# BaeHann/feature_level_style_transfer_for_TSC

Measured on AMD Instinct MI355X. Metric: train-step samples/sec (univariate TS, len=512, batch=256) at 1/2/4/8 MI355X, higher is better.
Workload: dtype bf16x3

## Files before the change

### feature_level_style_transfer_for_tsc_amd/_lib.py

```python
from __future__ import annotations

import ctypes
import os
from ctypes import POINTER, Structure, c_char_p, c_float, c_int, c_int32, c_int64, c_void_p
from typing import Optional

import torch

ABI_VERSION = 26
_LIB_NAME = "libfst_hip.so"
_HERE = os.path.dirname(os.path.abspath(__file__))
LIB_PATH = os.environ.get("FST_HIP_LIB", os.path.join(_HERE, _LIB_NAME))


class FstLibraryError(RuntimeError):
    pass


class WSrc(Structure):
    _fields_ = [("w", c_void_p), ("off0", c_int64), ("sm", c_int64), ("sc", c_int64), ("st", c_int64)]


_P = c_void_p
_I32P = c_void_p
_SIGNATURES = {
    "fst_version": (c_int, []),
    "fst_last_error": (c_char_p, []),
    "fst_pack_weights": (c_int, [_I32P, _I32P, c_int, POINTER(WSrc), POINTER(WSrc), c_int, c_int, c_int, c_int, _P, c_void_p]),
    "fst_pack_weights_bf16x3": (c_int, [_I32P, _I32P, c_int, POINTER(WSrc), POINTER(WSrc), c_int, c_int, c_int, c_int, _P, c_void_p]),
    "fst_unpack_weights": (c_int, [_I32P, _I32P, c_int, _P, c_int, _P, c_int64, c_int64, c_int64, c_int64,
                                   _P, c_int64, c_int64, c_int64, c_int64, c_int, c_void_p]),
    "fst_mask_taps": (c_int, [_P, _I32P, _I32P, c_int, c_int, c_int, c_void_p]),
    "fst_conv_gemm": (c_int, [_P, c_int64, _P, c_int64, _P, _I32P, _I32P, c_int, _P, _P, c_int64, _P, c_int64,
                              _P, c_int64, c_int, c_int, c_int, c_int, c_int, c_int, c_int, c_int, c_void_p]),
    "fst_conv_wgrad": (c_int, [_P, c_int64, _P, c_int64, _P, c_int64, _P, c_int64, c_int, _P, _I32P, _I32P, c_int,
                               c_int, c_int, c_int, c_int, c_int, c_int64, c_void_p]),
    "fst_conv_last_route": (c_int, [POINTER(c_int32)]),
    "fst_row_sum": (c_int, [_P, c_int64, c_int, c_int, c_int, _P, c_void_p]),
    "fst_bn_stats": (c_int, [_P, c_int, c_int, c_int, _P, c_int64, c_void_p]),
    "fst_bn_finalize": (c_int, [_P, c_int, _P, _P, _P, _P, c_int, c_int, c_float, c_float, _P, c_void_p]),
    "fst_bn_apply": (c_int, [_P, _P, _P, _P, _P, c_int, c_int, c_int, c_int, c_int64, c_void_p]),
    "fst_bn_bwd_reduce": (c_int, [_P, _P, _P, _P, c_int, c_int, c_int, c_int, _P, c_int64, c_void_p]),
    "fst_bn_bwd_apply": (c_int, [_P, _P, _P, _P, _P, c_int, _P, _P, _P, c_int, c_int, c_int, c_int, c_int, c_int, c_int64, c_void_p]),
    "fst_bn_bwd_reduce_join": (c_int, [_P, _P, _P, _P, _P, c_int, c_int, c_int, _P, _P, c_int64, c_void_p]),
    "fst_bn_bwd_apply_join": (c_int, [_P, _P, _P, _P, _P, _P, _P, c_int, _P, _P, _P, _P, _P, _P, c_int, c_int, c_int, c_int, c_int,
                                      c_int64, c_void_p]),
    "fst_gate_fwd": (c_int, [_P, _P, c_int, c_int, c_int, c_int64, c_void_p]),
    "fst_gate_bwd": (c_int, [_P, _P, _P, c_int, c_int, c_int, c_int64, c_void_p]),
    "fst_coupling_sum_slots": (c_int64, [c_int, c_int, c_int]),
    "fst_coupling_fwd": (c_int, [_P, _P, _P, c_int, c_int, c_int, c_int64, _P, c_void_p]),
    "fst_coupling_bwd": (c_int, [_P, _P, _P, _P, _P, _P, _P, _P, c_int, c_int, c_int, c_int64, c_void_p]),
    "fst_coupling_inv_fwd": (c_int, [_P, _P, _P, c_int, c_int, c_int, c_int64, c_void_p]),
    "fst_coupling_inv_bwd": (c_int, [_P, _P, _P, _P, _P, c_int, c_int, c_int, c_int64, c_void_p]),
    "fst_rmsprop_multi": (c_int, [_P, _P, _P, _P, _P, c_int, c_float, c_float, c_void_p]),
    "fst_adam_multi": (c_int, [_P, _P, _P, _P, _P, c_int, _P, c_float, c_float, c_float, c_float, c_void_p]),
    "fst_rmsprop_multi_dev": (c_int, [_P, _P, _P, _P, _P, c_int, c_float, c_float, c_void_p]),
    "fst_adam_multi_dev": (c_int, [_P, _P, _P, _P, _P, c_int, _P, _P, c_float, c_float, c_float, c_void_p]),
    "fst_nonfinite_slots": (c_int64, [c_int]),
    "fst_nonfinite_multi": (c_int, [_P, _P, _I32P, c_int, c_int32, _I32P, c_int64, _I32P, _I32P, _P, _I32P, c_void_p]),
    "fst_rmsprop_multi_guard": (c_int, [_P, _P, _P, _P, _P, _P, c_int, c_float, c_float, _I32P, c_void_p]),
    "fst_adam_multi_guard": (c_int, [_P, _P, _P, _P, _P, c_int, _P, c_float, _P, c_float, c_float, c_float, _I32P, c_void_p]),
    "fst_guard_copy_multi": (c_int, [_P, _P, _P, c_int, _I32P, c_int, c_void_p]),
    "fst_sumsq_slots": (c_int64, [c_int]),
    "fst_sumsq_multi": (c_int, [_P, _P, _I32P, c_int, _P, c_int64, _P, _P, _P, c_void_p]),
    "fst_scale_multi": (c_int, [_P, _P, _I32P, c_int, _P, c_void_p]),
    "fst_ema_multi": (c_int, [_P, _P, _P, _I32P, c_int, c_int32, _P, _P, c_void_p]),
    "fst_swap_multi": (c_int, [_P, _P, _P, c_int, c_void_p]),
    "fst_accum_multi": (c_int, [_P, _P, _P, c_int, _P, c_int, c_void_p]),
    "fst_feed_batch": (c_int, [_P, _P, _P, _P, _P, _P, c_int, _P, _P, c_int, _P, c_void_p]),
    "fst_eval_fold": (c_int, [_P, c_int64, _P, c_int64, c_int, _P, _P, _P, _P, _P, _P, c_int64, _P, c_void_p]),
    "fst_eval_finish": (c_int, [_P, _P, c_int64, _P, c_int, c_void_p]),
    "fst_wn_stack_fwd_ok": (c_int, [c_int, c_int, c_int, c_int]),
    "fst_wn_stack_fwd": (c_int, [_P, _P, _P, c_int64, _P, _P, _P, c_int64, _P, c_int, c_int, c_int, c_int, c_int, c_int64, c_void_p]),
    "fst_wn_stack_infer": (c_int, [_P, _P, _P, c_int64, _P, _P, c_int64, _P, c_int, c_int, c_int, c_int, c_int, c_int64, c_void_p]),
    "fst_wn_stack_bwd_ok": (c_int, [c_int, c_int, c_int, c_int]),
    "fst_wn_stack_bwd": (c_int, [_P, _P, _P, _P, _P, _P, _P, _P, _P, c_int64, c_int, c_int, c_int, c_int, c_int, c_int64, c_void_p]),
    "fst_wn_stack_bwd_proj": (c_int, [_P, _P, _P, _P, _P, _P, _P, _P, c_int, c_int64, _P, c_int64, c_int, c_int, c_int, c_int, c_int,
                                      c_int64, c_void_p]),
    "fst_wn_wgrad_ok": (c_int, [c_int, c_int, c_int, c_int, c_int, c_int]),
    "fst_wn_wgrad_workspace_floats": (c_int64, [c_int, c_int, c_int, c_int, c_int, c_int]),
    "fst_wn_wgrad_in": (c_int, [_P, _P, _P, c_int, c_int64, _P, _P, _P, c_int64, c_int, c_int, c_int, c_int, c_int, c_int, c_int64,
                                c_void_p]),
    "fst_wn_wgrad_rs": (c_int, [_P, _P, _P, c_int, _P, _P, c_int64, c_int, c_int, c_int, c_int, c_int64, c_void_p]),
    "fst_wn_wgrad_in_slabs": (c_int, [_P, _P, _P, c_int, c_int64, _P, c_int64, c_int, c_int, c_int, c_int, c_int, c_int, c_int64,
                                      c_void_p]),
    "fst_wn_wgrad_rs_slabs": (c_int, [_P, _P, _P, c_int, _P, c_int64, c_int, c_int, c_int, c_int, c_int64, c_void_p]),
    "fst_wn_wgrad_reduce_many": (c_int, [_I32P, _I32P, _I32P, _P, _P, _P, _P, c_int, c_int, c_int, c_int, c_int, c_void_p]),
    "fst_nt_gemm_workspace_floats": (c_int64, [c_int, c_int, c_int]),
    "fst_nt_gemm": (c_int, [_P, _P, _P, _P, c_int64, c_int, c_int, c_int, _P, _P, c_int, c_float, _P, c_void_p]),
    "fst_tap_wgrad_ok": (c_int, [c_int, c_int, c_int, c_int, c_int, c_int, c_int]),
    "fst_tap_wgrad_workspace_floats": (c_int64, [c_int, c_int, c_int, c_int, c_int]),
    "fst_tap_wgrad": (c_int, [_P, _P, _P, _P, c_int64, c_int, c_int, c_int, c_int, c_int, c_int, c_int, c_int, c_int64, c_int64, c_void_p]),
    "fst_dense_tap_wgrad_ok": (c_int, [c_int, c_int, c_int, c_int, c_int, c_int]),
    "fst_dense_tap_wgrad_workspace_floats": (c_int64, [c_int, c_int, c_int, c_int, c_int]),
    "fst_dense_tap_wgrad": (c_int, [_P, _P, _P, _P, c_int64, c_int, c_int, c_int, c_int, c_int, c_int, c_int64, c_int64, c_void_p]),
    "fst_wn_last_route": (c_int, [POINTER(c_int32)]),
    "fst_relu_bwd": (c_int, [_P, _P, _P, c_int64, c_void_p]),
    "fst_gemm_workspace_floats": (c_int64, [c_int, c_int, c_int]),
    "fst_gemm": (c_int, [_P, c_int64, c_int, _P, c_int64, c_int, _P, c_int64, c_int, c_int, c_int, _P, c_int, c_float, _P, c_int64,
                         c_void_p]),
    "fst_gemm_f32_workspace_floats": (c_int64, [c_int, c_int, c_int]),
    "fst_gemm_f32": (c_int, [_P, c_int64, c_int, _P, c_int64, c_int, _P, c_int64, c_int, c_int, c_int, _P, c_int, c_float, _P, c_int64,
                             c_void_p]),
    "fst_act_bwd": (c_int, [_P, _P, _P, c_int64, c_float, c_void_p]),
    "fst_batch_sum": (c_int, [_P, _P, _P, c_int, c_int64, c_int, c_void_p]),
    "fst_noise_transfer_fwd": (c_int, [_P, c_int, c_int, _P, _P, c_float, c_float, _P, _P, _P, _P, _P, _P, _P, c_int, c_int, c_void_p]),
    "fst_bcast_add": (c_int, [_P, _P, _P, c_int, c_int64, c_void_p]),
    "fst_noise_transfer_bwd": (c_int, [_P, c_int, _P, _P, _P, _P, c_int, c_int, c_void_p]),
    "fst_noise_transfer_dw": (c_int, [_P, _P, _P, _P, c_int, c_int, c_void_p]),
    "fst_noise_transfer_bwd_apply": (c_int, [_P, _P, _P, _P, c_float, c_float, c_int, _P, _P, c_int64, c_void_p]),
    "fst_wn_fold_fwd": (c_int, [_P, c_int, _P, _P, c_void_p]),
    "fst_wn_fold_bwd": (c_int, [_P, c_int, _P, _P, _P, c_void_p]),
    "fst_logdet_inv": (c_int, [_P, c_int, _P, _P, c_void_p]),
    "fst_wn_image_bytes": (c_int64, [c_int, c_int]),
    "fst_wn_pack": (c_int, [_P, _P, _P, _P, _P, _P, c_int, c_int, c_int, c_int, _P, c_int64, c_void_p]),
    "fst_wn_pack_stack": (c_int, [_P, _P, _P, _P, _P, _P, c_int, c_int, c_int, c_int, _P, c_int64, c_void_p]),
    "fst_wn_layer_fwd": (c_int, [_P, c_int64, _P, c_int64, _P, c_int64, _P, _P, _P, _P, c_int, c_int, c_int, c_int, c_int, c_int,
                                 c_int, c_int64, c_void_p]),
    "fst_wn_layer_infer": (c_int, [_P, c_int64, _P, c_int64, _P, c_int64, _P, _P, c_int, c_int, c_int, c_int, c_int, c_int, c_int,
                                   c_int64, c_void_p]),
    "fst_wn_bwd_image_bytes": (c_int64, [c_int, c_int]),
    "fst_wn_pack_bwd": (c_int, [_P, c_int, c_int, c_int, _P, c_int64, c_void_p]),
    "fst_wn_pack_bwd_stack": (c_int, [_P, c_int, c_int, c_int, _P, c_int64, c_void_p]),
    "fst_wn_bwd_proj_image_bytes": (c_int64, [c_int, c_int, c_int]),
    "fst_wn_pack_bwd_proj_stack": (c_int, [_P, _P, c_int, c_int, c_int, _P, c_int64, c_void_p]),
    "fst_wn_layer_bwd": (c_int, [_P, _P, _P, _P, c_int64, _P, _P, c_int64, c_int, c_int, c_int, c_int, c_int64, c_void_p]),
    "fst_wn_dgrad_image_bytes": (c_int64, [c_int]),
    "fst_wn_pack_dgrad": (c_int, [_P, _P, c_int, c_int, c_int, _P, c_int64, c_void_p]),
    "fst_wn_pack_dgrad_stack": (c_int, [_P, _P, c_int, c_int, c_int, c_int, _P, c_int64, c_void_p]),
    "fst_wn_dgrad_fits": (c_int, [c_int, c_int, c_int]),
    "fst_wn_layer_dgrad": (c_int, [_P, _P, c_int64, _P, _P, _P, _P, c_int64, c_int, c_int, c_int, c_int, c_int, c_int64, c_int64,
                                   c_void_p]),
    "fst_gru_fwd": (c_int, [_P, _P, _P, _P, _P, _I32P, c_int, c_int, c_int, c_int, c_int64, c_void_p]),
    "fst_gru_bwd": (c_int, [_P, _P, _P, _P, _I32P, c_int, _P, _P, c_int, c_int, c_int, c_int64, c_void_p]),
    "fst_lstm2_fwd": (c_int, [_P, _P, _P, _P, c_int, c_int, c_int64, c_void_p]),
    "fst_lstm2_bwd": (c_int, [_P, _P, _P, _P, _P, c_int, c_int, c_int64, c_void_p]),
    "fst_axpy": (c_int, [_P, _P, c_float, c_int64, c_void_p]),
    "fst_add_slices": (c_int, [_P, c_int64, _P, c_int64, _P, c_int64, c_int, c_int, c_int, c_void_p]),
    "fst_cpc_workspace_floats": (c_int64, [c_int, c_int, c_int, c_int]),
    "fst_cpc_nce_slots": (c_int64, [c_int, c_int, c_int, c_int]),
    "fst_cpc_nce_fwd": (c_int, [_P, c_int64, c_int64, c_int64, _I32P, _P, c_int, c_int, c_int, c_int, c_int, _P, _P, _P, c_void_p]),
    "fst_cpc_nce_bwd": (c_int, [_P, c_int64, c_int64, c_int64, _I32P, _P, _P, c_int, c_int, c_int, c_int, c_int, _P, _P, _P,
                                c_void_p]),
}
EXPORTED_SYMBOLS = tuple(_SIGNATURES)

_lib: Optional[ctypes.CDLL] = None


def load(path: Optional[str] = None) -> ctypes.CDLL:
    global _lib
    if _lib is not None and path is None:
        return _lib
    p = path or LIB_PATH
    if not os.path.exists(p):
        raise FstLibraryError(
            f"{p} not found — build it with `python -c 'import __graft_entry__ as g; g.build()'` "
            "(hipcc --offload-arch=gfx950).  There is no CPU fallback.")
    try:
        lib = ctypes.CDLL(p)
    except OSError as e:
        raise FstLibraryError(f"cannot load {p}: {e}") from e
    for name, (res, args) in _SIGNATURES.items():
        try:
            fn = getattr(lib, name)
        except AttributeError as e:
            raise FstLibraryError(f"{p} does not export {name}; rebuild the library") from e
        fn.restype, fn.argtypes = res, args
    if lib.fst_version() != ABI_VERSION:
        raise FstLibraryError(f"{p}: ABI version {lib.fst_version()} != expected {ABI_VERSION}; rebuild")
    if path is None:
        _lib = lib
    return lib


def check(rc: int, what: str) -> None:
    if rc != 0:
        msg = load().fst_last_error()
        raise RuntimeError(f"{what} failed (rc={rc}): {msg.decode() if msg else '?'}")


def stream_ptr() -> int:
    return torch.cuda.current_stream().cuda_stream


def ptr(t: Optional[torch.Tensor]) -> Optional[int]:
    return None if t is None else t.data_ptr()


def require_gpu_tensor(t: torch.Tensor, name: str) -> None:
    if not t.is_cuda:
        raise FstLibraryError(f"{name} lives on {t.device}; the fst ops run on an MI355X only (no CPU fallback)")
    if t.dtype != torch.float32:
        raise TypeError(f"{name} must be float32, got {t.dtype}")
```

### feature_level_style_transfer_for_tsc_amd/csrc/wn_wgrad.hip

```cpp
#include <stdlib.h>
#include <type_traits>

#include "fst_device.h"

#define WW_TT 32
#define WW_MROWS 256
#define WW_ND 3
#define WW_NX 2
#define WW_MAX_NX 5

__device__ __attribute__((aligned(16))) float ww_zero16[4] = {0.f, 0.f, 0.f, 0.f};

#define WW_MAX_SETS 3
struct WwOut { int rows, out, out_off, out_sc, out_sm; };
struct WwSeg {
  const float* ptr[WW_MAX_SETS];
  long long bs;
  long long mul_off;
  int shift;
  WwOut o;
};

struct WwParams {
  WwSeg dy[2];
  WwSeg x[4];
  int n_dy, n_x, M, K, K_main, n_extra;
  int xr;
  int mul;
  int n_groups, ksplit, B, L, tiles_per_seq, n_tiles;
  const float* epi_p;
  const float* epi_r1;
  float* epi_raw;
  int epi_ncls;
  float epi_scale;
  int n_sets;
  int RX;
  int misaligned;
  int Kcols;
  float* slab;
  float* slab_extra;
  float* w[2];
};

__device__ __forceinline__ unsigned ww_lds_addr(const char* p) {
  return (unsigned)(uintptr_t)((__attribute__((address_space(3))) const char*)p);
}
template <int OFF = 0>
__device__ __forceinline__ f32x4 ww_lds_read16(unsigned addr) {
  f32x4 v;
  asm volatile("ds_read_b128 %0, %1 offset:%2" : "=v"(v) : "v"(addr), "n"(OFF) : "memory");
  return v;
}
template <int OFF = 0>
__device__ __forceinline__ float ww_lds_read4(unsigned addr) {
  float v;
  asm volatile("ds_read_b32 %0, %1 offset:%2" : "=v"(v) : "v"(addr), "n"(OFF) : "memory");
  return v;
}
template <int OFF = 0>
__device__ __forceinline__ void ww_lds_write16(unsigned addr, const u32x4& v) {
  asm volatile("ds_write_b128 %0, %1 offset:%2" ::"v"(addr), "v"(v), "n"(OFF) : "memory");
}
template <int OFF = 0>
__device__ __forceinline__ void ww_lds_zero4(unsigned addr) {
  asm volatile("ds_write_b32 %0, %1 offset:%2" ::"v"(addr), "v"(0.0f), "n"(OFF) : "memory");
}
__device__ __forceinline__ void ww_dma16(const char* gsrc, unsigned lds_addr) {
  unsigned saved_m0;
  asm volatile("s_mov_b32 %0, m0\n\ts_mov_b32 m0, %2\n\ts_nop 0\n\tglobal_load_lds_dwordx4 %1, off\n\ts_mov_b32 m0, %0"
               : "=&s"(saved_m0) : "v"(gsrc), "s"(lds_addr) : "memory");
}
__device__ __forceinline__ void ww_lds_wait() {
  asm volatile("s_waitcnt lgkmcnt(0)" ::: "memory");
  __builtin_amdgcn_sched_barrier(0);
}

template <class V4>
__device__ __forceinline__ void ww_split8u(const V4& v0, const V4& v1, u32x4& h, u32x4& l) {
  const float v[8] = {v0.x, v0.y, v0.z, v0.w, v1.x, v1.y, v1.z, v1.w};
  bf16x8 hi, lo;
  split_bf16x8(v, hi, lo);
  h = __builtin_bit_cast(u32x4, hi);
  l = __builtin_bit_cast(u32x4, lo);
}

__device__ __forceinline__ int ww_dma_row(int i, int lane) { return 8 * i + ((lane >> 3) ^ (i & 1)); }
__device__ __forceinline__ int ww_lds_off(int r, int q) { return ((r ^ ((r >> 3) & 1)) << 7) + (((q ^ r) & 7) << 4); }


struct WwDmaLane { int r, q; };
__device__ __forceinline__ WwDmaLane ww_dma_lane(int i, int lane) {
  const int r = ww_dma_row(i, lane);
  return {r, (lane ^ r) & 7};
}

struct WwFragLane { int row, piece[2][2]; };
__device__ __forceinline__ WwFragLane ww_frag_lane(int l31, int half) {
  WwFragLane f;
  f.row = (l31 ^ ((l31 >> 3) & 1)) << 7;
  const int sw = l31 & 7;
#pragma unroll
  for (int ks = 0; ks < 2; ++ks)
#pragma unroll
    for (int j = 0; j < 2; ++j) f.piece[ks][j] = (((4 * ks + 2 * half + j) ^ sw) & 7) << 4;
  return f;
}

__device__ __forceinline__ void ww_tile_range(int wg, int n_wgs, int n_tiles, int& begin, int& end) {
  begin = (int)(((long long)wg * n_tiles) / n_wgs);
  end = (int)(((long long)(wg + 1) * n_tiles) / n_wgs);
}

__device__ __forceinline__ void ww_store_tile(float* dst, int ld, const f32x16& acc) {
#pragma unroll
  for (int r = 0; r < 16; ++r) dst[(long long)((r & 3) + 8 * (r >> 2)) * ld] = acc[r];
}


__device__ __forceinline__ const WwOut& ww_out(const WwSeg& s) { return s.o; }
__device__ __forceinline__ const WwOut& ww_out(const WwOut& o) { return o; }
struct WwRow { int si, c; };
template <class S>
__device__ __forceinline__ WwRow ww_k_row(const S (&x)[4], int n_x, int kk) {
  WwRow r = {0, kk};
#pragma unroll
  for (int j = 0; j < 3; ++j)
    if (r.si == j && j + 1 < n_x && r.c >= ww_out(x[j]).rows) { r.c -= ww_out(x[j]).rows; ++r.si; }
  return r;
}
template <class S, class F>
__device__ __forceinline__ auto ww_pick(const S (&x)[4], int si, F f) {
  auto v = f(x[0]);
  if (si == 1) v = f(x[1]);
  if (si == 2) v = f(x[2]);
  if (si == 3) v = f(x[3]);
  return v;
}

struct WwSrc { const float* p; int bs, t; };

struct WwDyStage {
  WwSrc src[4];

  __device__ __forceinline__ void build(const WwParams& p, int set, int wave_s, int lane) {
    const float* const d0 = p.dy[0].ptr[set];
    const float* const d1 = p.dy[1].ptr[set];
#pragma unroll
    for (int k = 0; k < 4; ++k) {
      const WwDmaLane m = ww_dma_lane(wave_s + 8 * k, lane);
      const int r = m.r, q = m.q;
      src[k].p = nullptr; src[k].bs = 0; src[k].t = 4 * q;
      if (r < p.M) {
        if (p.n_dy > 1 && r >= p.dy[0].o.rows) {
          src[k].p = d1 + ((long long)(r - p.dy[0].o.rows) * p.L + 4 * q); src[k].bs = (int)p.dy[1].bs;
        } else {
          src[k].p = d0 + ((long long)r * p.L + 4 * q); src[k].bs = (int)p.dy[0].bs;
        }
      }
    }
  }
  __device__ __forceinline__ void issue1(int k, int b, int t0, int L, char* slot, int wave_s, const char* zero16) const {
    const bool ok = src[k].p != nullptr && t0 + src[k].t < L;
    const char* s = ok ? reinterpret_cast<const char*>(src[k].p + ((long long)b * src[k].bs + t0)) : zero16;
    ww_dma16(s, ww_lds_addr(slot + (wave_s + 8 * k) * 1024));
  }
};

struct WwXStage {
  WwSrc src[WW_MAX_NX];
  int my_nx;

  __device__ __forceinline__ void build(const WwParams& p, int set, int g, int wave_s, int lane) {
    const int NXI = p.RX >> 3;
    my_nx = (NXI - wave_s + 7) >> 3;
    const float* const xp[4] = {p.x[0].ptr[set], p.x[1].ptr[set], p.x[2].ptr[set], p.x[3].ptr[set]};
#pragma unroll
    for (int k = 0; k < WW_MAX_NX; ++k) {
      src[k].p = nullptr; src[k].bs = 0; src[k].t = 0;
      if (k >= my_nx) continue;
      const WwDmaLane m = ww_dma_lane(wave_s + 8 * k, lane);
      const int rr = m.r, q = m.q;
      int kk = -1;
      bool partner = false;
      if (rr < p.xr) kk = g * p.xr + rr;
      else if (p.mul && rr < 2 * p.xr) { kk = g * p.xr + rr - p.xr; partner = true; }
      else {
        const int e = rr - p.xr * (1 + p.mul);
        if (g == 0 && e < p.n_extra) kk = p.K_main + e;
      }
      if (kk >= 0 && kk < p.K && (kk < p.K_main || rr >= p.xr * (1 + p.mul))) {
        const WwRow row = ww_k_row(p.x, p.n_x, kk);
        const float* sp = ww_pick(xp, row.si, [](const float* x) { return x; });
        const long long sbs = ww_pick(p.x, row.si, [](const WwSeg& x) { return x.bs; });
        const long long smo = ww_pick(p.x, row.si, [](const WwSeg& x) { return x.mul_off; });
        const int ssh = ww_pick(p.x, row.si, [](const WwSeg& x) { return x.shift; });
        src[k].p = sp + ((long long)row.c * p.L + ssh + 4 * q) + (partner ? smo : 0);
        src[k].bs = (int)sbs;
        src[k].t = ssh + 4 * q;
      }
    }
  }
  __device__ __forceinline__ void issue1(int k, int b, int t0, int L, char* slot, int wave_s, const char* zero16) const {
    if (k >= my_nx) return;
    const int t = t0 + src[k].t;
    const bool ok = src[k].p != nullptr && t > -4 && t < L;
    const char* s = ok ? reinterpret_cast<const char*>(src[k].p + ((long long)b * src[k].bs + t0)) : zero16;
    ww_dma16(s, ww_lds_addr(slot + (wave_s + 8 * k) * 1024));
  }
};

__device__ __forceinline__ int ww_patch_shift(const WwParams& p, int g, int tid) {
  if (!(p.misaligned && tid < p.xr)) return 0;
  const int kk = g * p.xr + tid;
  const int sh = ww_pick(p.x, ww_k_row(p.x, p.n_x, kk).si, [](const WwSeg& x) { return x.shift; });
  return (kk < p.K_main && (sh & 3) != 0 && sh > -4 && sh < 4) ? sh : 0;
}

__device__ __forceinline__ void ww_patch_edges(char* xslot, int tid, int patch_sh, int t0, int L) {
  const bool at_start = t0 == 0, at_end = t0 + WW_TT >= L;
  if (at_start || at_end) {
    if (patch_sh != 0) {
      char* rowp = xslot + ((tid ^ ((tid >> 3) & 1)) << 7);
      if (at_start && patch_sh < 0)
        for (int j = 0; j < -patch_sh; ++j) ww_lds_zero4(ww_lds_addr(rowp + (((0 ^ tid) & 7) << 4) + 4 * j));
      if (at_end && patch_sh > 0)
        for (int j = 4 - patch_sh; j < 4; ++j) ww_lds_zero4(ww_lds_addr(rowp + (((7 ^ tid) & 7) << 4) + 4 * j));
    }
    asm volatile("s_waitcnt lgkmcnt(0)" ::: "memory");
    __builtin_amdgcn_s_barrier();
  }
}

template <bool MUL, int NE>
static __device__ void ww_split_pass(char* dw, char* xw, int tid, int xr, int e_off, float (&ev)[2]) {
  const int u = tid & 3, r0 = tid >> 2;
  f32x4 e0, e1;
  if constexpr (NE > 0) {
    e0 = ww_lds_read16(ww_lds_addr(xw + e_off + ((2 * u) << 4)));
    e1 = ww_lds_read16(ww_lds_addr(xw + e_off + ((2 * u + 1) << 4)));
  }
  f32x4 d[2][2], xq[2][2], xm[2][2];
  char* da[2][2]; char* xa[2][2];
  const int nxu = (xr * 4 > 512 + tid) ? 2 : 1;
#pragma unroll
  for (int i = 0; i < 2; ++i) {
    const int r = r0 + 128 * i;
    da[i][0] = dw + ww_lds_off(r, 2 * u); da[i][1] = dw + ww_lds_off(r, 2 * u + 1);
    d[i][0] = ww_lds_read16(ww_lds_addr(da[i][0])); d[i][1] = ww_lds_read16(ww_lds_addr(da[i][1]));
    xa[i][0] = xw + ww_lds_off(r, 2 * u); xa[i][1] = xw + ww_lds_off(r, 2 * u + 1);
    if (i < nxu && r < xr) {
      xq[i][0] = ww_lds_read16(ww_lds_addr(xa[i][0])); xq[i][1] = ww_lds_read16(ww_lds_addr(xa[i][1]));
      if constexpr (MUL) {
        xm[i][0] = ww_lds_read16(ww_lds_addr(xa[i][0] + (xr << 7))); xm[i][1] = ww_lds_read16(ww_lds_addr(xa[i][1] + (xr << 7)));
      }
    }
  }
  ww_lds_wait();
#pragma unroll
  for (int i = 0; i < 2; ++i) {
    const int r = r0 + 128 * i;
    if constexpr (NE > 0)
      ev[i] += (d[i][0].x * e0.x + d[i][0].y * e0.y) + (d[i][0].z * e0.z + d[i][0].w * e0.w) +
               (d[i][1].x * e1.x + d[i][1].y * e1.y) + (d[i][1].z * e1.z + d[i][1].w * e1.w);
    u32x4 h4, l4;
    ww_split8u(d[i][0], d[i][1], h4, l4);
    ww_lds_write16(ww_lds_addr(da[i][0]), h4); ww_lds_write16(ww_lds_addr(da[i][1]), l4);
    if (i < nxu && r < xr) {
      if constexpr (MUL) { xq[i][0] *= xm[i][0]; xq[i][1] *= xm[i][1]; }
      ww_split8u(xq[i][0], xq[i][1], h4, l4);
      ww_lds_write16(ww_lds_addr(xa[i][0]), h4); ww_lds_write16(ww_lds_addr(xa[i][1]), l4);
    }
  }
  asm volatile("s_waitcnt lgkmcnt(0)" ::: "memory");
}

template <int MT, int KT, bool FULL, class Issue>
__device__ __forceinline__ void ww_k_step(f32x16 (&acc)[MT][KT], const char* ap, const char* bp, const int (&piece)[2], int m_live,
                                          int k_live, Issue issue) {
  f32x4 araw[MT][2], braw[KT][2];
#pragma unroll
  for (int i = 0; i < MT; ++i) {
    araw[i][0] = ww_lds_read16(ww_lds_addr(ap + ((i * 32) << 7) + piece[0]));
    araw[i][1] = ww_lds_read16(ww_lds_addr(ap + ((i * 32) << 7) + piece[1]));
  }
#pragma unroll
  for (int j = 0; j < KT; ++j) {
    braw[j][0] = ww_lds_read16(ww_lds_addr(bp + ((j * 32) << 7) + piece[0]));
    braw[j][1] = ww_lds_read16(ww_lds_addr(bp + ((j * 32) << 7) + piece[1]));
  }
  ww_lds_wait();
  issue(0);
#pragma unroll
  for (int j = 0; j < KT; ++j) {
    if (FULL || j < k_live) {
      const bf16x8 bh = __builtin_bit_cast(bf16x8, braw[j][0]), bl = __builtin_bit_cast(bf16x8, braw[j][1]);
#pragma unroll
      for (int i = 0; i < MT; ++i) {
        if (!FULL && i >= m_live) break;
        const bf16x8 ah = __builtin_bit_cast(bf16x8, araw[i][0]), al = __builtin_bit_cast(bf16x8, araw[i][1]);
        mfma_bf3(acc[i][j], ah, al, bh, bl);
      }
    }
    issue(1 + j);
  }
  if constexpr (KT < 3) issue(3);
  issue(4);
}

template <int MT, int KT, bool FULL, bool MUL, int NE>
__global__ __launch_bounds__(512, 2) void wn_wgrad_kernel(WwParams p) {
  extern __shared__ __attribute__((aligned(16))) char ww_lds[];
  const int tid = threadIdx.x, lane = tid & 63, half = lane >> 5, l31 = lane & 31;
  const int wave_s = __builtin_amdgcn_readfirstlane(tid >> 6);
  const int wm = wave_s >> 1, wk = wave_s & 1;
  const int g = blockIdx.y, L = p.L;
  const int set = blockIdx.x % p.n_sets;
  const int dslot_bytes = WW_MROWS * 128, xslot_bytes = p.RX * 128;
  char* const xring = ww_lds + WW_ND * dslot_bytes;
  const char* const zero16 = reinterpret_cast<const char*>(ww_zero16);

  WwDyStage dys;
  dys.build(p, set, wave_s, lane);
  WwXStage xs;
  xs.build(p, set, g, wave_s, lane);
  const int patch_sh = ww_patch_shift(p, g, tid);
  __builtin_amdgcn_s_waitcnt(0x0F70);

  auto tile_bt = [&](int tile, int& b, int& t0) {
    b = tile / p.tiles_per_seq;
    t0 = (tile - b * p.tiles_per_seq) * WW_TT;
  };
  auto issue_dy = [&](int tile, int slot) {
    int b, t0;
    tile_bt(tile, b, t0);
#pragma unroll
    for (int k = 0; k < 4; ++k) dys.issue1(k, b, t0, L, ww_lds + slot * dslot_bytes, wave_s, zero16);
  };
  auto issue_x = [&](int tile, int slot) {
    int b, t0;
    tile_bt(tile, b, t0);
#pragma unroll
    for (int k = 0; k < WW_MAX_NX; ++k) xs.issue1(k, b, t0, L, xring + slot * xslot_bytes, wave_s, zero16);
  };

  f32x16 acc[MT][KT];
  zero_acc(acc);
  float ev[2] = {0.f, 0.f};

  const int wg_in_set = blockIdx.x / p.n_sets, wgs_of_set = (p.ksplit - set + p.n_sets - 1) / p.n_sets;
  int tile_begin, tile_end;
  ww_tile_range(wg_in_set, wgs_of_set, p.n_tiles, tile_begin, tile_end);
  const int m_blocks = (p.M + 31) >> 5;
  const int k_blocks_here = min(2 * KT, ((p.K_main + 31) >> 5) - g * 2 * KT);
  const int m_live = m_blocks - wm * MT, k_live = k_blocks_here - wk * KT;
  const bool do_extra = NE > 0 && g == 0;

  const WwFragLane fl = ww_frag_lane(l31, half);
  const int a_off = ((wm * MT * 32) << 7) + fl.row;
  const int x_off = ((wk * KT * 32) << 7) + fl.row;
  const int e_off = (p.xr * (1 + p.mul)) << 7;

  const int n_st = tile_end - tile_begin;
  if (n_st > 0) { issue_dy(tile_begin, 0); issue_x(tile_begin, 0); }
  if (n_st > 1) issue_dy(tile_begin + 1, 1);
  int dslot = 0, xslot = 0;
  for (int c = 0; c < n_st; ++c) {
    if (c + 1 < n_st) wait_vmcnt<4>(); else wait_vmcnt<0>();
    __builtin_amdgcn_s_barrier();
    const bool have_x = c + 1 < n_st, have_dy = c + 2 < n_st;
    int nb = 0, nt0 = 0, db = 0, dt0 = 0;
    if (have_x) tile_bt(tile_begin + c + 1, nb, nt0);
    if (have_dy) tile_bt(tile_begin + c + 2, db, dt0);
    const int x_next = xslot ^ 1, d_next = dslot >= 1 ? dslot - 1 : 2;
    auto issue_pos = [&](int pos) {
      if (pos < WW_MAX_NX) { if (have_x) xs.issue1(pos, nb, nt0, L, xring + x_next * xslot_bytes, wave_s, zero16); }
      else if (pos < WW_MAX_NX + 4) { if (have_dy) dys.issue1(pos - WW_MAX_NX, db, dt0, L, ww_lds + d_next * dslot_bytes, wave_s, zero16); }
    };
    char* const dsl = ww_lds + dslot * dslot_bytes;
    char* const xsl = xring + xslot * xslot_bytes;
    if (p.misaligned) {
      int bq, t0;
      tile_bt(tile_begin + c, bq, t0);
      ww_patch_edges(xsl, tid, patch_sh, t0, L);
    }
    ww_split_pass<MUL, NE>(dsl, xsl, tid, p.xr, e_off, ev);
    __builtin_amdgcn_s_barrier();
#pragma unroll
    for (int ks = 0; ks < 2; ++ks)
      ww_k_step<MT, KT, FULL>(acc, dsl + a_off, xsl + x_off, fl.piece[ks], m_live, k_live, [&](int pos) { issue_pos(5 * ks + pos); });
    dslot = dslot == WW_ND - 1 ? 0 : dslot + 1;
    xslot ^= 1;
  }

  float* const slab = p.slab + (long long)blockIdx.x * WW_MROWS * p.Kcols;
#pragma unroll
  for (int i = 0; i < MT; ++i) {
    if (i >= m_live) break;
#pragma unroll
    for (int j = 0; j < KT; ++j) {
      if (j >= k_live) break;
      ww_store_tile(slab + (long long)((wm * MT + i) * 32 + 4 * half) * p.Kcols + g * p.xr + (wk * KT + j) * 32 + l31, p.Kcols, acc[i][j]);
    }
  }
  if (do_extra) {
#pragma unroll
    for (int i = 0; i < 2; ++i) {
      float sv = ev[i];
      sv += __shfl_xor(sv, 1, 64);
      sv += __shfl_xor(sv, 2, 64);
      if ((tid & 3) == 0) p.slab_extra[((long long)blockIdx.x * WW_MROWS + (tid >> 2) + 128 * i) * 2] = sv;
    }
  }
}


__device__ __forceinline__ void ww_dst(const WwParams& p, int si, int& out, int& off, int& sc, int& sm) {
  out = p.x[0].o.out; off = p.x[0].o.out_off; sc = p.x[0].o.out_sc; sm = p.x[0].o.out_sm;
  if (si == 1) { out = p.x[1].o.out; off = p.x[1].o.out_off; sc = p.x[1].o.out_sc; sm = p.x[1].o.out_sm; }
  if (si == 2) { out = p.x[2].o.out; off = p.x[2].o.out_off; sc = p.x[2].o.out_sc; sm = p.x[2].o.out_sm; }
  if (si == 3) { out = p.x[3].o.out; off = p.x[3].o.out_off; sc = p.x[3].o.out_sc; sm = p.x[3].o.out_sm; }
}
template <class P, class Epi>
__device__ __forceinline__ void ww_scatter(const P& p, int m, int kk, float v, Epi epi) {
  const WwRow r = ww_k_row(p.x, p.n_x, kk);
  int out, off, sc, sm;
  ww_dst(p, r.si, out, off, sc, sm);
  float* dst = out == 0 ? p.w[0] : p.w[1];
  const long long at = (long long)m * sm + (long long)r.c * sc + off;
  dst[at] = epi(v, at, r.c, sm);
}

template <class Store>
__device__ __forceinline__ void ww_quad_sum(const float* q, long long st, int ksplit, bool live, float4 (&part)[4][64], Store store) {
  const int cx = threadIdx.x & 63, sg = threadIdx.x >> 6;
  float4 s = make_float4(0.f, 0.f, 0.f, 0.f);
  if (live) {
    int sl = sg;
    for (; sl + 28 < ksplit; sl += 32) {
      float4 v[8];
#pragma unroll
      for (int u = 0; u < 8; ++u) v[u] = *reinterpret_cast<const float4*>(q + (sl + 4 * u) * st);
#pragma unroll
      for (int u = 0; u < 8; ++u) { s.x += v[u].x; s.y += v[u].y; s.z += v[u].z; s.w += v[u].w; }
    }
    for (; sl < ksplit; sl += 4) {
      const float4 v = *reinterpret_cast<const float4*>(q + sl * st);
      s.x += v.x; s.y += v.y; s.z += v.z; s.w += v.w;
    }
  }
  part[sg][cx] = s;
  __syncthreads();
  if (sg == 0 && live) {
    float4 t = part[0][cx];
#pragma unroll
    for (int g2 = 1; g2 < 4; ++g2) { const float4 o = part[g2][cx]; t.x += o.x; t.y += o.y; t.z += o.z; t.w += o.w; }
    const float tv[4] = {t.x, t.y, t.z, t.w};
    store(tv);
  }
}

__device__ __forceinline__ float ww_extra_sum(const float* q, int ksplit) {
  float s = 0.f;
  int sl = 0;
  for (; sl + 8 <= ksplit; sl += 8) {
    float v[8];
#pragma unroll
    for (int u = 0; u < 8; ++u) v[u] = q[(long long)(sl + u) * WW_MROWS * 2];
#pragma unroll
    for (int u = 0; u < 8; ++u) s += v[u];
  }
  for (; sl < ksplit; ++sl) s += q[(long long)sl * WW_MROWS * 2];
  return s;
}

__global__ __launch_bounds__(256) void wn_wgrad_reduce_kernel(WwParams p) {
  __shared__ float4 part[4][64];
  const int m = blockIdx.y, cx = threadIdx.x & 63, sg = threadIdx.x >> 6;
  const int kk0 = blockIdx.x * 256 + cx * 4;
  auto epi = [&](float v, long long at, int c, int sm) {
    if (p.epi_p) {
      float sd = 0.f;
      for (int j = 0; j < p.epi_ncls; ++j) sd += p.epi_p[m * p.epi_ncls + j] * p.epi_r1[(long long)j * sm + c];
      if (p.epi_raw) p.epi_raw[at] = v;
      v = v * p.epi_scale * sd;
    }
    return v;
  };
  ww_quad_sum(p.slab + (long long)m * p.Kcols + kk0, (long long)WW_MROWS * p.Kcols, p.ksplit, kk0 < p.Kcols, part, [&](const float (&tv)[4]) {
#pragma unroll
    for (int j = 0; j < 4; ++j)
      if (kk0 + j < p.K_main) ww_scatter(p, m, kk0 + j, tv[j], epi);
  });
  if (blockIdx.x == gridDim.x - 1 && sg == 1 && cx < p.n_extra && p.K_main < p.K)
    ww_scatter(p, m, p.K_main + cx, ww_extra_sum(p.slab_extra + (long long)m * 2 + cx, p.ksplit), epi);
}

#define WW_MAX_RED 16
struct WwRedEntry {
  const float* slab;
  const float* slab_extra;
  float* w[2];
  int ksplit, Kcols, K_main, K, n_extra, M, n_x;
  int quad_blocks;
  WwOut x[4];
};
struct WwRedParams { WwRedEntry e[WW_MAX_RED]; };
__device__ __forceinline__ void ww_dst(const WwRedEntry& e, int si, int& out, int& off, int& sc, int& sm) {
  auto field = [&](int WwOut::*f) { return ww_pick(e.x, si, [f](const WwOut& o) { return o.*f; }); };
  out = field(&WwOut::out); off = field(&WwOut::out_off); sc = field(&WwOut::out_sc); sm = field(&WwOut::out_sm);
}

__global__ __launch_bounds__(256) void wn_wgrad_reduce_many_kernel(WwRedParams p) {
  __shared__ float4 part[4][64];
  const WwRedEntry& e = p.e[blockIdx.z];
  const int bx = blockIdx.x;
  auto plain = [](float v, long long, int, int) { return v; };
  if (bx >= e.quad_blocks) {
    const int it = (bx - e.quad_blocks) * 256 + threadIdx.x;
    if (e.K_main < e.K && it < e.M * e.n_extra) {
      const int m = it / e.n_extra, j = it - m * e.n_extra;
      ww_scatter(e, m, e.K_main + j, ww_extra_sum(e.slab_extra + (long long)m * 2 + j, e.ksplit), plain);
    }
    return;
  }
  const int qpr = e.Kcols >> 2;
  const int quad = bx * 64 + (threadIdx.x & 63);
  ww_quad_sum(e.slab + (long long)quad * 4, (long long)WW_MROWS * e.Kcols, e.ksplit, quad < e.M * qpr, part, [&](const float (&tv)[4]) {
    const int m = quad / qpr, kk0 = (quad - m * qpr) * 4;
#pragma unroll
    for (int j = 0; j < 4; ++j)
      if (kk0 + j < e.K_main) ww_scatter(e, m, kk0 + j, tv[j], plain);
  });
}


static thread_local int32_t g_wn_route[FST_WN_ROUTE_LEN] = {0};

void fst_wn_set_route(int family, int t1, int t2, int t3, int t4, int gx, int gy, int gz, int a8, int a9, int a10, int lds) {
  const int32_t r[FST_WN_ROUTE_LEN] = {family, t1, t2, t3, t4, gx, gy, gz, a8, a9, a10, lds};
  for (int i = 0; i < FST_WN_ROUTE_LEN; ++i) g_wn_route[i] = r[i];
}

extern "C" int fst_wn_last_route(int32_t out[FST_WN_ROUTE_LEN]) {
  FST_REQUIRE(out != nullptr, "fst_wn_last_route: null output");
  for (int i = 0; i < FST_WN_ROUTE_LEN; ++i) out[i] = g_wn_route[i];
  return g_wn_route[0] != 0 ? 0 : -1;
}

static int ww_ksplit(int n_groups, int clamp, int floor) {
  int ks = fst_cu_count_or(256) / n_groups;
  if (ks > clamp) ks = clamp;
  if (ks < floor) ks = floor;
  return ks;
}

static void ww_tiles_and_split(WwParams* p, int B, int L, int n_sets) {
  p->RX = p->xr * (1 + p->mul) + (p->n_extra ? 8 : 0);
  p->Kcols = p->n_groups * p->xr;
  p->B = B; p->L = L;
  p->tiles_per_seq = L / WW_TT;
  p->n_tiles = B * p->tiles_per_seq;
  p->ksplit = ww_ksplit(p->n_groups, p->n_tiles * n_sets, n_sets);
  p->n_sets = n_sets;
}

static int64_t ww_slab_floats(const WwParams& p) { return (int64_t)p.ksplit * WW_MROWS * (p.Kcols + 2); }

static int ww_bind_workspace(WwParams& p, float* workspace, int64_t workspace_floats, const char* who) {
  FST_REQUIRE(workspace_floats >= ww_slab_floats(p), "%s: workspace of %lld floats is too small", who, (long long)workspace_floats);
  p.slab = workspace;
  p.slab_extra = workspace + (long long)p.ksplit * WW_MROWS * p.Kcols;
  return 0;
}

static int ww_geometry(int kind, int B, int L, int n, int h, int last, int n_sets, WwParams* p) {
  const int KT = kind == 0 ? 3 : 2;
  p->M = kind == 0 ? 2 * n : (last ? n : 2 * n);
  p->K = kind == 0 ? 3 * n + h : n;
  const int rem = p->K & 31;
  p->n_extra = (kind == 0 && rem == 1) ? 1 : 0;
  p->K_main = p->n_extra ? p->K - rem : p->K;
  p->xr = 32 * 2 * KT;
  const int kb = (p->K_main + 31) / 32;
  p->n_groups = (kb + 2 * KT - 1) / (2 * KT);
  p->mul = kind == 1;
  ww_tiles_and_split(p, B, L, n_sets);
  return KT;
}

extern "C" int fst_wn_wgrad_ok(int kind, int B, int L, int n, int h, int dil) {
  if (!(B > 0 && L > 0 && L % WW_TT == 0 && n > 0 && n < 128)) return 0;
  if (kind == 0) {
    if (!(h > 0 && h <= 32 && dil > 0 && (3 * n + h + 31) / 32 <= 18)) return 0;
    return dil % 4 == 0 ? 1 : (dil < 4 ? 2 : 0);
  }
  return kind == 1;
}

extern "C" int64_t fst_wn_wgrad_workspace_floats(int kind, int B, int L, int n, int h, int last) {
  if (!fst_wn_wgrad_ok(kind, B, L, n, h, 4)) return -1;
  WwParams p;
  ww_geometry(kind, B, L, n, h, last, WW_MAX_SETS, &p);
  return ww_slab_floats(p);
}

static int ww_launch(WwParams& p, int KT, void* stream, bool reduce = true) {
  const size_t lds = (size_t)WW_ND * WW_MROWS * 128 + (size_t)WW_NX * p.RX * 128;
  FST_REQUIRE(lds <= 160 * 1024 && (p.RX >> 3) <= 8 * WW_MAX_NX, "fst_wn_wgrad: %d staged k-rows per stage do not fit (LDS %zu B)", p.RX, lds);
  const bool full = (p.M + 31) / 32 == 8 && ((p.K_main + 31) / 32) % (2 * KT) == 0;
  void (*fn)(WwParams);
  if (KT == 3) {
    if (p.n_extra) fn = full ? wn_wgrad_kernel<2, 3, true, false, 1> : wn_wgrad_kernel<2, 3, false, false, 1>;
    else fn = full ? wn_wgrad_kernel<2, 3, true, false, 0> : wn_wgrad_kernel<2, 3, false, false, 0>;
  } else if (p.mul) {
    fn = full ? wn_wgrad_kernel<2, 2, true, true, 0> : wn_wgrad_kernel<2, 2, false, true, 0>;
  } else {
    fn = full ? wn_wgrad_kernel<2, 2, true, false, 0> : wn_wgrad_kernel<2, 2, false, false, 0>;
  }
  if (int rc = fst_allow_full_lds((const void*)fn, "fst_wn_wgrad")) return rc;
  fst_wn_set_route(FST_WN_ROUTE_WGRAD, KT, (int)full, p.mul, p.n_extra, p.ksplit, p.n_groups, 1, p.n_sets, p.misaligned, (int)reduce, (int)lds);
  hipLaunchKernelGGL(fn, dim3((unsigned)p.ksplit, (unsigned)p.n_groups), dim3(512), lds, (hipStream_t)stream, p);
  FST_LAUNCH_CHECK();
  if (!reduce) return 0;
  hipLaunchKernelGGL(wn_wgrad_reduce_kernel, dim3((unsigned)((p.Kcols + 255) / 256), (unsigned)p.M), dim3(256), 0, (hipStream_t)stream, p);
  FST_LAUNCH_CHECK();
  return 0;
}

static void ww_in_segments(WwParams& p, int n, int h, int L, int dil, long long u0_bs) {
  p.n_dy = 1;
  p.dy[0] = {{}, (long long)2 * n * L, 0, 0, {2 * n, 0, 0, 0, 0}};
  p.n_x = 4;
  for (int tap = 0; tap < 3; ++tap) p.x[tap] = {{}, (long long)n * L, 0, (tap - 1) * dil, {n, 0, tap, 3, 3 * n}};
  p.x[3] = {{}, u0_bs, 0, 0, {h, 1, 0, 1, h}};
}

static void ww_rs_segments(WwParams& p, int n, int L, int last) {
  p.n_dy = last ? 1 : 2;
  p.dy[0] = {{}, (long long)n * L, 0, 0, {n, 0, 0, 0, 0}};
  p.dy[1] = {{}, (long long)n * L, 0, 0, {n, 0, 0, 0, 0}};
  p.n_x = 1;
  p.x[0] = {{}, (long long)2 * n * L, (long long)n * L, 0, {n, 0, 0, 1, n}};
}

static int ww_prologue(const char* who, int kind, const float* const* const* ops, int n_ops, int n_sets, float* workspace,
                       int64_t workspace_floats, int B, int L, int n, int h, int last, WwParams& p, int& KT) {
  FST_REQUIRE(n_sets >= 1 && n_sets <= WW_MAX_SETS, "%s: %d operand sets (1..%d)", who, n_sets, WW_MAX_SETS);
  FST_REQUIRE(fst_aligned16(workspace), "%s: operands must be 16-byte aligned", who);
  KT = ww_geometry(kind, B, L, n, h, last, n_sets, &p);
  if (int rc = ww_bind_workspace(p, workspace, workspace_floats, who)) return rc;
  for (int s = 0; s < n_sets; ++s)
    for (int k = 0; k < n_ops; ++k) {
      FST_REQUIRE(ops[k][s], "%s: null operand in set %d", who, s);
      FST_REQUIRE(fst_aligned16(ops[k][s]), "%s: operands must be 16-byte aligned", who);
    }
  return 0;
}

static int ww_in(const float* const* dg, const float* const* a, const float* const* u0, int n_sets, int64_t u0_bs, float* dw_in,
                 float* dw_cond, float* workspace, int64_t workspace_floats, int B, int L, int n, int h, int dil, int a_slack,
                 int64_t numel_a, void* stream, bool reduce) {
  fst_wn_clear_route();
  FST_REQUIRE(dg && a && u0 && workspace && (!reduce || (dw_in && dw_cond)), "fst_wn_wgrad_in: null operand");
  const int served = fst_wn_wgrad_ok(0, B, L, n, h, dil);
  FST_REQUIRE(served == 1 || (served == 2 && a_slack), "fst_wn_wgrad_in: unsupported shape B=%d L=%d n=%d h=%d dil=%d (needs L %% 32 == 0, "
              "n < 128, h <= 32, and dil %% 4 == 0 or — with 16 readable bytes either side of a — dil < 4)", B, L, n, h, dil);
  FST_REQUIRE((long long)B * n * L == (long long)numel_a, "fst_wn_wgrad_in: B*n*L does not match the element count %lld of a", (long long)numel_a);
  FST_REQUIRE(B == 1 || u0_bs >= (int64_t)h * L, "fst_wn_wgrad_in: u0 batch stride %lld < h*L", (long long)u0_bs);
  FST_REQUIRE(u0_bs % 4 == 0, "fst_wn_wgrad_in: operands must be 16-byte aligned");
  WwParams p = {};
  int KT;
  const float* const* const ops[3] = {dg, a, u0};
  if (int rc = ww_prologue("fst_wn_wgrad_in", 0, ops, 3, n_sets, workspace, workspace_floats, B, L, n, h, 0, p, KT)) return rc;
  ww_in_segments(p, n, h, L, dil, (long long)u0_bs);
  for (int s = 0; s < n_sets; ++s) {
    p.dy[0].ptr[s] = dg[s];
    for (int tap = 0; tap < 3; ++tap) p.x[tap].ptr[s] = a[s];
    p.x[3].ptr[s] = u0[s];
  }
  p.misaligned = dil % 4 != 0;
  p.w[0] = dw_in; p.w[1] = dw_cond;
  return ww_launch(p, KT, stream, reduce);
}

extern "C" int fst_wn_wgrad_in(const float* const* dg, const float* const* a, const float* const* u0, int n_sets, int64_t u0_bs,
                               float* dw_in, float* dw_cond, float* workspace, int64_t workspace_floats, int B, int L, int n, int h,
                               int dil, int a_slack, int64_t numel_a, void* stream) {
  return ww_in(dg, a, u0, n_sets, u0_bs, dw_in, dw_cond, workspace, workspace_floats, B, L, n, h, dil, a_slack, numel_a, stream, true);
}

extern "C" int fst_wn_wgrad_in_slabs(const float* const* dg, const float* const* a, const float* const* u0, int n_sets, int64_t u0_bs,
                                     float* workspace, int64_t workspace_floats, int B, int L, int n, int h, int dil, int a_slack,
                                     int64_t numel_a, void* stream) {
  return ww_in(dg, a, u0, n_sets, u0_bs, nullptr, nullptr, workspace, workspace_floats, B, L, n, h, dil, a_slack, numel_a, stream, false);
}

static int ww_rs(const float* const* d_a, const float* const* d_out, const float* const* ts, int n_sets, float* dw_rs, float* workspace,
                 int64_t workspace_floats, int last, int B, int L, int n, int64_t numel_a, void* stream, bool reduce) {
  fst_wn_clear_route();
  FST_REQUIRE(d_out && ts && (dw_rs || !reduce) && workspace && (last || d_a), "fst_wn_wgrad_rs: null operand");
  FST_REQUIRE(fst_wn_wgrad_ok(1, B, L, n, 0, 4), "fst_wn_wgrad_rs: unsupported shape B=%d L=%d n=%d (needs L %% 32 == 0, n < 128)", B, L, n);
  FST_REQUIRE((long long)B * n * L == (long long)numel_a, "fst_wn_wgrad_rs: B*n*L does not match the element count %lld", (long long)numel_a);
  WwParams p = {};
  int KT;
  const float* const* const ops[3] = {d_out, ts, d_a};
  if (int rc = ww_prologue("fst_wn_wgrad_rs", 1, ops, last ? 2 : 3, n_sets, workspace, workspace_floats, B, L, n, 0, last, p, KT)) return rc;
  ww_rs_segments(p, n, L, last);
  for (int s = 0; s < n_sets; ++s) {
    if (last) p.dy[0].ptr[s] = d_out[s];
    else { p.dy[0].ptr[s] = d_a[s]; p.dy[1].ptr[s] = d_out[s]; }
    p.x[0].ptr[s] = ts[s];
  }
  p.w[0] = dw_rs; p.w[1] = nullptr;
  return ww_launch(p, KT, stream, reduce);
}

extern "C" int fst_wn_wgrad_rs(const float* const* d_a, const float* const* d_out, const float* const* ts, int n_sets, float* dw_rs,
                               float* workspace, int64_t workspace_floats, int last, int B, int L, int n, int64_t numel_a,
                               void* stream) {
  return ww_rs(d_a, d_out, ts, n_sets, dw_rs, workspace, workspace_floats, last, B, L, n, numel_a, stream, true);
}

extern "C" int fst_wn_wgrad_rs_slabs(const float* const* d_a, const float* const* d_out, const float* const* ts, int n_sets,
                                     float* workspace, int64_t workspace_floats, int last, int B, int L, int n, int64_t numel_a,
                                     void* stream) {
  return ww_rs(d_a, d_out, ts, n_sets, nullptr, workspace, workspace_floats, last, B, L, n, numel_a, stream, false);
}

static WwRedEntry ww_red_entry(const WwParams& p) {
  WwRedEntry e = {p.slab, p.slab_extra, {p.w[0], p.w[1]}, p.ksplit, p.Kcols, p.K_main, p.K, p.n_extra, p.M, p.n_x,
                  (p.M * (p.Kcols / 4) + 63) / 64, {}};
  for (int i = 0; i < p.n_x; ++i) e.x[i] = p.x[i].o;
  return e;
}

extern "C" int fst_wn_wgrad_reduce_many(const int32_t* kind, const int32_t* last, const int32_t* n_sets, float* const* workspace,
                                        const int64_t* workspace_floats, float* const* dw0, float* const* dw1, int n_entries, int B,
                                        int L, int n, int h, void* stream) {
  fst_wn_clear_route();
  FST_REQUIRE(kind && last && n_sets && workspace && workspace_floats && dw0 && dw1, "fst_wn_wgrad_reduce_many: null table");
  FST_REQUIRE(n_entries >= 1 && n_entries <= WW_MAX_RED, "fst_wn_wgrad_reduce_many: %d entries (1..%d)", n_entries, WW_MAX_RED);
  WwRedParams rp = {};
  unsigned gx = 1;
  for (int j = 0; j < n_entries; ++j) {
    FST_REQUIRE(kind[j] == 0 || kind[j] == 1, "fst_wn_wgrad_reduce_many: entry %d has kind %d (0 or 1)", j, (int)kind[j]);
    FST_REQUIRE(fst_wn_wgrad_ok(kind[j], B, L, n, h, 4), "fst_wn_wgrad_reduce_many: unsupported shape B=%d L=%d n=%d h=%d", B, L, n, h);
    FST_REQUIRE(n_sets[j] >= 1 && n_sets[j] <= WW_MAX_SETS, "fst_wn_wgrad_reduce_many: entry %d has %d operand sets (1..%d)", j,
                (int)n_sets[j], WW_MAX_SETS);
    FST_REQUIRE(workspace[j] && dw0[j] && (kind[j] == 1 || dw1[j]), "fst_wn_wgrad_reduce_many: null operand in entry %d", j);
    FST_REQUIRE(fst_aligned16(workspace[j]), "fst_wn_wgrad_reduce_many: workspaces must be 16-byte aligned");
    WwParams p = {};
    const int lastj = kind[j] == 1 && last[j];
    ww_geometry(kind[j], B, L, n, h, lastj, n_sets[j], &p);
    char who[48];
    snprintf(who, sizeof who, "fst_wn_wgrad_reduce_many: entry %d", j);
    if (int rc = ww_bind_workspace(p, workspace[j], workspace_floats[j], who)) return rc;
    if (kind[j] == 0) ww_in_segments(p, n, h, L, 4, 0);
    else ww_rs_segments(p, n, L, lastj);
    p.w[0] = dw0[j]; p.w[1] = kind[j] == 0 ? dw1[j] : nullptr;
    const WwRedEntry& e = rp.e[j] = ww_red_entry(p);
    const unsigned blocks = (unsigned)e.quad_blocks + (unsigned)((p.K_main < p.K ? p.M * p.n_extra : 0) + 255) / 256;
    if (blocks > gx) gx = blocks;
  }
  hipLaunchKernelGGL(wn_wgrad_reduce_many_kernel, dim3(gx, 1, (unsigned)n_entries), dim3(256), 0, (hipStream_t)stream, rp);
  FST_LAUNCH_CHECK();
  return 0;
}

static void nt_geometry(int M, int N, int K, WwParams* p) {
  p->M = M; p->K = N; p->K_main = N; p->n_extra = 0;
  p->xr = 128;
  p->n_groups = ((N + 31) / 32 + 3) / 4;
  p->mul = 0;
  ww_tiles_and_split(p, 1, K, 1);
}

extern "C" int64_t fst_nt_gemm_workspace_floats(int M, int N, int K) {
  if (!(M > 0 && M <= WW_MROWS && N > 0 && K > 0 && K % WW_TT == 0)) return -1;
  WwParams p = {};
  nt_geometry(M, N, K, &p);
  return ww_slab_floats(p);
}

extern "C" int fst_nt_gemm(const float* A, const float* Bm, float* C, float* workspace, int64_t workspace_floats, int M, int N, int K,
                           const float* epi_p, const float* epi_r1, int epi_ncls, float epi_scale, float* epi_raw, void* stream) {
  fst_wn_clear_route();
  FST_REQUIRE(A && Bm && C && workspace, "fst_nt_gemm: null operand");
  FST_REQUIRE(M > 0 && M <= WW_MROWS && N > 0 && K > 0 && K % WW_TT == 0, "fst_nt_gemm: M=%d N=%d K=%d (needs M <= 256, K %% 32 == 0)", M, N, K);
  FST_REQUIRE((long long)N * K < (1LL << 31) * 4 && (long long)M * N < (1LL << 31), "fst_nt_gemm: operand too large");
  FST_REQUIRE(fst_aligned16(A) && fst_aligned16(Bm) && fst_aligned16(workspace), "fst_nt_gemm: operands must be 16-byte aligned");
  FST_REQUIRE((epi_p == nullptr) == (epi_r1 == nullptr) && (epi_p == nullptr || epi_ncls > 0) && (epi_p != nullptr || epi_raw == nullptr),
              "fst_nt_gemm: the epilogue takes p [M][ncls] and r1 [ncls][N] together (and the raw product only with them)");
  WwParams p = {};
  nt_geometry(M, N, K, &p);
  if (int rc = ww_bind_workspace(p, workspace, workspace_floats, "fst_nt_gemm")) return rc;
  p.n_dy = 1;
  p.dy[0] = {{A, nullptr, nullptr}, 0, 0, 0, {M, 0, 0, 0, 0}};
  p.n_x = 1;
  p.x[0] = {{Bm, nullptr, nullptr}, 0, 0, 0, {N, 0, 0, 1, N}};
  p.w[0] = C; p.w[1] = nullptr;
  p.epi_p = epi_p; p.epi_r1 = epi_r1; p.epi_ncls = epi_ncls; p.epi_scale = epi_scale; p.epi_raw = epi_raw;
  const bool direct = p.ksplit == 1 && M == WW_MROWS && p.Kcols == N && !epi_p;
  if (direct) p.slab = C;
  return ww_launch(p, 2, stream, !direct);
}

extern "C" int fst_tap_wgrad_ok(int B, int L, int M, int C, int ntaps, int dil, int pad_left) {
  if (!(B > 0 && L > 0 && L % WW_TT == 0 && M > 0 && M <= WW_MROWS && C > 0 && ntaps >= 1 && ntaps <= 4 && dil > 0)) return 0;
  if (((long long)ntaps * C + 31) / 32 > 18) return 0;
  int need_slack = 0;
  for (int tap = 0; tap < ntaps; ++tap) {
    const int sh = tap * dil - pad_left;
    if (sh % 4 != 0) {
      if (sh <= -4 || sh >= 4) return 0;
      need_slack = 1;
    }
  }
  return need_slack ? 2 : 1;
}

static void tap_geometry(int B, int L, int M, int C, int ntaps, WwParams* p) {
  p->M = M; p->K = ntaps * C; p->K_main = p->K; p->n_extra = 0;
  p->xr = 192;
  p->n_groups = ((p->K + 31) / 32 + 5) / 6;
  p->mul = 0;
  ww_tiles_and_split(p, B, L, 1);
}

extern "C" int64_t fst_tap_wgrad_workspace_floats(int B, int L, int M, int C, int ntaps) {
  if (!fst_tap_wgrad_ok(B, L, M, C, ntaps, 4, 0)) return -1;
  WwParams p = {};
  tap_geometry(B, L, M, C, ntaps, &p);
  return ww_slab_floats(p);
}

extern "C" int fst_tap_wgrad(const float* dy, const float* x, float* dw, float* workspace, int64_t workspace_floats, int B, int L, int M,
                             int C, int ntaps, int dil, int pad_left, int x_slack, int64_t numel_dy, int64_t numel_x, void* stream) {
  fst_wn_clear_route();
  FST_REQUIRE(dy && x && dw && workspace, "fst_tap_wgrad: null operand");
  const int served = fst_tap_wgrad_ok(B, L, M, C, ntaps, dil, pad_left);
  FST_REQUIRE(served == 1 || (served == 2 && x_slack), "fst_tap_wgrad: unsupported shape B=%d L=%d M=%d C=%d ntaps=%d dil=%d pad_left=%d "
              "(needs L %% 32 == 0, M <= 256, at most 4 taps, tap shifts multiples of 4 or — with 16 readable bytes either side of x — "
              "within 3 samples)", B, L, M, C, ntaps, dil, pad_left);
  FST_REQUIRE((long long)B * M * L == (long long)numel_dy && (long long)B * C * L == (long long)numel_x,
              "fst_tap_wgrad: B*M*L / B*C*L do not match the element counts %lld / %lld", (long long)numel_dy, (long long)numel_x);
  FST_REQUIRE(fst_aligned16(dy) && fst_aligned16(x) && fst_aligned16(workspace), "fst_tap_wgrad: operands must be 16-byte aligned");
  WwParams p = {};
  tap_geometry(B, L, M, C, ntaps, &p);
  if (int rc = ww_bind_workspace(p, workspace, workspace_floats, "fst_tap_wgrad")) return rc;
  p.n_dy = 1;
  p.dy[0] = {{dy, nullptr, nullptr}, (long long)M * L, 0, 0, {M, 0, 0, 0, 0}};
  p.n_x = ntaps;
  p.misaligned = 0;
  for (int tap = 0; tap < ntaps; ++tap) {
    const int sh = tap * dil - pad_left;
    p.x[tap] = {{x, nullptr, nullptr}, (long long)C * L, 0, sh, {C, 0, tap, ntaps, C * ntaps}};
    if (sh % 4 != 0) p.misaligned = 1;
  }
  p.w[0] = dw; p.w[1] = nullptr;
  return ww_launch(p, 3, stream);
}

#define TZ_CPB 288
#define TZ_XRAW 1024
#define TZ_ND 4

struct TzParams {
  const float* dy;
  const float* x;
  float* slab;
  float* dw;
  int B, L, M, C, K, P4;
  int off0;
  int n_groups, ksplit, tiles_per_seq, n_tiles, Kcols;
  int m_halves;
};

#ifdef FST_STAMPS
__device__ unsigned long long tz_stamps[12];
extern "C" int fst_debug_tz_stamps(unsigned long long* out_host, int reset) { return fst_read_stamps(tz_stamps, out_host, reset); }
#endif


template <int MP, bool FULL>
__global__ __launch_bounds__(512, 2) void tz_wgrad_kernel(TzParams p) {
  constexpr int CW = 8 / MP;
  constexpr int NDW = MP == 2 ? 2 : 1;
  constexpr int DSLOT = (MP == 2 ? 128 : 64) * 128;
  constexpr int XSLOT = CW * TZ_XRAW;
  constexpr int LO = CW * 8 * TZ_CPB, COPIES = 2 * LO;
  constexpr int X0 = TZ_ND * DSLOT, C0 = X0 + TZ_ND * XSLOT;
  constexpr int XU = (128 * CW) / 512;
  extern __shared__ __attribute__((aligned(16))) char tz_lds[];
  const unsigned lds0 = ww_lds_addr(tz_lds);
  const int tid = threadIdx.x, lane = tid & 63, half = lane >> 5, l31 = lane & 31;
  const int wave_s = __builtin_amdgcn_readfirstlane(tid >> 6);
  const int wm = wave_s / CW, wk = wave_s % CW;
  const int g = blockIdx.y, L = p.L;
  const char* const zero16 = reinterpret_cast<const char*>(ww_zero16);

  const int m_base = blockIdx.z * 128;
  const int M_here = p.m_halves > 1 ? min(128, p.M - m_base) : p.M;
  const float* dsrc[NDW];
#pragma unroll
  for (int k = 0; k < NDW; ++k) {
    const WwDmaLane m = ww_dma_lane(wave_s + 8 * k, lane);
    dsrc[k] = p.dy + ((long long)(m_base + (m.r < M_here ? m.r : 0)) * L + 4 * m.q);
  }
  const bool has_x = wave_s < CW;
  const int my_ch = CW * g + wave_s;
  const bool x_lane = has_x && my_ch < p.C && lane < 40;
  const float* const xrow = p.x + ((long long)(x_lane ? my_ch : 0) * L + 4 * lane - p.P4);
  const int xt = 4 * lane - p.P4;
  const long long dy_bs = (long long)p.M * L, x_bs = (long long)p.C * L;
  __builtin_amdgcn_s_waitcnt(0x0F70);

  struct Pos { int t0; long long doff, xoff; };
  auto advance = [&](Pos& q) {
    q.t0 += WW_TT; q.doff += WW_TT; q.xoff += WW_TT;
    if (q.t0 == L) { q.t0 = 0; q.doff += dy_bs - L; q.xoff += x_bs - L; }
  };
  auto issue_stage = [&](const Pos& q, int slot) {
#pragma unroll
    for (int k = 0; k < NDW; ++k)
      ww_dma16(reinterpret_cast<const char*>(dsrc[k] + q.doff), lds0 + slot * DSLOT + (wave_s + 8 * k) * 1024);
    if (has_x) {
      const int t = q.t0 + xt;
      const char* src = (x_lane && t >= 0 && t < L) ? reinterpret_cast<const char*>(xrow + q.xoff) : zero16;
      ww_dma16(src, lds0 + X0 + slot * XSLOT + wave_s * TZ_XRAW);
    }
  };
  auto wait_keep_one = [&]() {
    if (has_x) wait_vmcnt<NDW + 1>(); else wait_vmcnt<NDW>();
  };

  f32x16 acc[2][3];
  zero_acc(acc);

  int tile_begin, tile_end;
  ww_tile_range(blockIdx.x, p.ksplit, p.n_tiles, tile_begin, tile_end);
  const int m_blocks = (M_here + 31) >> 5;
  const int k_blocks = (p.K + 31) >> 5;
  const bool ch_live = CW * g + wk < p.C;

  const WwFragLane fl = ww_frag_lane(l31, half);
  unsigned a_lane[2][2];
#pragma unroll
  for (int ks = 0; ks < 2; ++ks)
#pragma unroll
    for (int j = 0; j < 2; ++j) a_lane[ks][j] = ((wm * 2 * 32) << 7) + fl.row + fl.piece[ks][j];
  const int o0 = p.off0 + l31 + 8 * half;
  const unsigned b_lane = wk * (8 * TZ_CPB) + (o0 & 7) * TZ_CPB + ((o0 >> 3) << 4);
  const int su = tid & 3, sr = tid >> 2;
  const bool dy_thread = MP == 2 || wave_s < 4;
  const unsigned sd_lane0 = ww_lds_off(sr, 2 * su), sd_lane1 = ww_lds_off(sr, 2 * su + 1);
  unsigned sx_src[XU], sx_dst[XU];
#pragma unroll
  for (int j = 0; j < XU; ++j) {
    const int id = tid + 512 * j, xc = id >> 7, xr = (id >> 4) & 7, xq = id & 15;
    sx_src[j] = xc * TZ_XRAW + (8 * xq + xr) * 4;
    sx_dst[j] = xc * (8 * TZ_CPB) + xr * TZ_CPB + (xq << 4);
  }

  const int n_st = tile_end - tile_begin;
  f32x4 sd0, sd1;
  float sxv[XU][8];
  auto split_load = [&](unsigned d_slot, unsigned x_slot) {
    if (dy_thread) { sd0 = ww_lds_read16<0>(d_slot + sd_lane0); sd1 = ww_lds_read16<0>(d_slot + sd_lane1); }
#pragma unroll
    for (int j = 0; j < XU; ++j) {
      const unsigned a = x_slot + sx_src[j];
      sxv[j][0] = ww_lds_read4<0>(a); sxv[j][1] = ww_lds_read4<4>(a); sxv[j][2] = ww_lds_read4<8>(a); sxv[j][3] = ww_lds_read4<12>(a);
      sxv[j][4] = ww_lds_read4<16>(a); sxv[j][5] = ww_lds_read4<20>(a); sxv[j][6] = ww_lds_read4<24>(a); sxv[j][7] = ww_lds_read4<28>(a);
    }
  };
  auto split_dy_store = [&](unsigned d_slot) {
    if (!dy_thread) return;
    u32x4 h4, l4;
    ww_split8u(sd0, sd1, h4, l4);
    ww_lds_write16<0>(d_slot + sd_lane0, h4); ww_lds_write16<0>(d_slot + sd_lane1, l4);
  };
  auto split_x_store = [&](unsigned cbuf) {
#pragma unroll
    for (int j = 0; j < XU; ++j) {
      bf16x8 hi, lo;
      split_bf16x8(sxv[j], hi, lo);
      ww_lds_write16<0>(cbuf + sx_dst[j], __builtin_bit_cast(u32x4, hi));
      ww_lds_write16<LO>(cbuf + sx_dst[j], __builtin_bit_cast(u32x4, lo));
    }
  };

  Pos pos;
  {
    const int b = tile_begin / p.tiles_per_seq;
    pos.t0 = (tile_begin - b * p.tiles_per_seq) * WW_TT;
    pos.doff = (long long)b * dy_bs + pos.t0;
    pos.xoff = (long long)b * x_bs + pos.t0;
  }
  int issued = 0;
  auto issue_next = [&](int slot) {
    issue_stage(pos, slot);
    ++issued;
    if (issued < n_st) advance(pos);
  };
  f32x4 araw[2][2][2], braw[2][3][2];
  auto frag_reads = [&](auto ks_c, unsigned d_slot, unsigned cbuf) {
    constexpr int ks = decltype(ks_c)::value;
    araw[ks][0][0] = ww_lds_read16<0>(d_slot + a_lane[ks][0]);    araw[ks][0][1] = ww_lds_read16<0>(d_slot + a_lane[ks][1]);
    araw[ks][1][0] = ww_lds_read16<4096>(d_slot + a_lane[ks][0]); araw[ks][1][1] = ww_lds_read16<4096>(d_slot + a_lane[ks][1]);
    const unsigned bb = cbuf + b_lane;
    braw[ks][0][0] = ww_lds_read16<((2 * ks) << 4)>(bb);      braw[ks][0][1] = ww_lds_read16<((2 * ks) << 4) + LO>(bb);
    braw[ks][1][0] = ww_lds_read16<((2 * ks + 4) << 4)>(bb);  braw[ks][1][1] = ww_lds_read16<((2 * ks + 4) << 4) + LO>(bb);
    braw[ks][2][0] = ww_lds_read16<((2 * ks + 8) << 4)>(bb);  braw[ks][2][1] = ww_lds_read16<((2 * ks + 8) << 4) + LO>(bb);
  };
  auto mfma_group = [&](int ks, int sb) {
    if (FULL || (sb < k_blocks && ch_live)) {
      const bf16x8 bh = __builtin_bit_cast(bf16x8, braw[ks][sb][0]), bl = __builtin_bit_cast(bf16x8, braw[ks][sb][1]);
#pragma unroll
      for (int i = 0; i < 2; ++i) {
        if (!FULL && wm * 2 + i >= m_blocks) break;
        const bf16x8 ah = __builtin_bit_cast(bf16x8, araw[ks][i][0]), al = __builtin_bit_cast(bf16x8, araw[ks][i][1]);
        mfma_bf3(acc[i][sb], ah, al, bh, bl);
      }
    }
    __builtin_amdgcn_sched_barrier(0);
  };
  FST_SUMS(12);
  FST_T(tz_begin);
  if (n_st > 0) {
// ... 149 lines not shown
```

### feature_level_style_transfer_for_tsc_amd/ops.py

```python
from __future__ import annotations

import ctypes
import math
import os
from typing import Callable, Dict, List, NamedTuple, Optional, Sequence, Tuple

import torch

from . import _lib
from . import dist as _dist
from ._lib import WSrc, check, ptr, stream_ptr
from .plan import Plan, Segment, build_plan, pick_mb

EPI_RELU, EPI_ACC2, EPI_ATOMIC, EPI_ACC1 = 1, 2, 4, 8
GEMM_BF16X3 = 16
WGRAD_SLABS = 32
MATH = os.environ.get("FST_MATH", "bf16x3")
LDS_BUDGET = 96 * 1024
LDS_MULTI_CHUNK = 44 * 1024
PIPE_C = 16

_PARTIAL_BACKWARD = False


class KernelTimer:

    def __init__(self, detail: bool = False):
        self.detail = detail
        self.records = {}

    def begin(self):
        ev = torch.cuda.Event(enable_timing=True)
        ev.record()
        return ev

    def end(self, key: str, start, flops: float, nbytes: float = 0.0):
        ev = torch.cuda.Event(enable_timing=True)
        ev.record()
        self.records.setdefault(key, []).append((start, ev, flops, nbytes))

    def summary(self):
        torch.cuda.synchronize()
        out = {}
        for key, recs in self.records.items():
            ms = sum(r[0].elapsed_time(r[1]) for r in recs)
            out[key] = {"launches": len(recs), "total_ms": ms, "avg_us": 1e3 * ms / len(recs),
                        "flops": sum(r[2] for r in recs), "bytes": sum(r[3] for r in recs)}
        return out


KERNEL_TIMER: Optional[KernelTimer] = None


ROUTE_GEMM, ROUTE_PIPE, ROUTE_BF3, ROUTE_WIN_BF3, ROUTE_WIN_ROWS, ROUTE_WGRAD = 1, 2, 3, 4, 5, 6
ROUTE_EPI_PLAIN, ROUTE_EPI_ADD, ROUTE_EPI_ATOMIC, ROUTE_EPI_VEC, ROUTE_EPI_VEC_ADD = 0, 1, 2, 3, 4
_ROUTE_NAMES = {ROUTE_GEMM: "conv_gemm_kernel", ROUTE_PIPE: "conv_gemm_pipe_kernel", ROUTE_BF3: "conv_gemm_bf3_kernel",
                ROUTE_WIN_BF3: "conv_win_bf3_kernel", ROUTE_WIN_ROWS: "conv_win_rows_kernel", ROUTE_WGRAD: "conv_wgrad_kernel"}
_ROUTE_NARGS = {ROUTE_GEMM: 2, ROUTE_PIPE: 3, ROUTE_BF3: 2, ROUTE_WIN_BF3: 2, ROUTE_WIN_ROWS: 0, ROUTE_WGRAD: 5}
_ROUTE_BOOLS = {(ROUTE_PIPE, 2), (ROUTE_WGRAD, 2), (ROUTE_WGRAD, 4)}


def last_route() -> Tuple[int, ...]:
    out = (ctypes.c_int32 * 8)()
    _lib.load().fst_conv_last_route(out)
    return tuple(out)


WN_ROUTE_WGRAD, WN_ROUTE_TZ, WN_ROUTE_LAYER_FWD, WN_ROUTE_STACK_FWD, WN_ROUTE_LAYER_BWD, WN_ROUTE_LAYER_DGRAD, WN_ROUTE_STACK_BWD = \
    1, 2, 3, 4, 5, 6, 7
WN_ROUTE_LAYER_INFER, WN_ROUTE_STACK_INFER = 8, 9
WN_ROUTE_LEN = 12
_WN_ROUTE_NAMES = {WN_ROUTE_WGRAD: "wn_wgrad_kernel", WN_ROUTE_TZ: "tz_wgrad_kernel", WN_ROUTE_LAYER_FWD: "wn_layer_fwd_kernel",
                   WN_ROUTE_STACK_FWD: "wn_stack_fwd_kernel", WN_ROUTE_LAYER_BWD: "wn_layer_bwd_kernel",
                   WN_ROUTE_LAYER_DGRAD: "wn_layer_dgrad_kernel", WN_ROUTE_STACK_BWD: "wn_stack_bwd_kernel",
                   WN_ROUTE_LAYER_INFER: "wn_layer_infer_kernel", WN_ROUTE_STACK_INFER: "wn_stack_infer_kernel"}


def wn_last_route() -> Tuple[int, ...]:
    out = (ctypes.c_int32 * WN_ROUTE_LEN)()
    _lib.load().fst_wn_last_route(out)
    return tuple(out)


def wn_route_kernel_name(route: Sequence[int]) -> str:
    fam, tf = route[0], ("false", "true")
    if fam == WN_ROUTE_WGRAD:
        return f"wn_wgrad_kernel<2, {route[1]}, {tf[route[2]]}, {tf[route[3]]}, {route[4]}>"
    if fam == WN_ROUTE_TZ:
        return f"tz_wgrad_kernel<{route[1]}, {tf[route[2]]}>"
    if fam == WN_ROUTE_LAYER_FWD:
        return f"wn_layer_fwd_kernel<{route[1]}>"
    if fam == WN_ROUTE_LAYER_INFER:
        return f"wn_layer_infer_kernel<{route[1]}>"
    return _WN_ROUTE_NAMES[fam]


def route_kernel_name(route: Sequence[int]) -> str:
    fam = route[0]
    args = [("true" if route[1 + i] else "false") if (fam, i) in _ROUTE_BOOLS else str(route[1 + i])
            for i in range(_ROUTE_NARGS[fam])]
    return _ROUTE_NAMES[fam] + (f"<{', '.join(args)}>" if args else "")


def bf3_ok(plan: Plan, L: int) -> bool:
    if MATH != "bf16x3":
        return False
    return (plan.pipeable and L % 4 == 0) or plan.windowed16


def _plan_macs_per_step(plan: Plan, M: int) -> int:
    total = 0
    ch, en = plan.chunks(), plan.entries()
    rows_per_group = plan.MB * 32
    for g in range(plan.n_mgroups):
        rows = max(0, min(M, (g + 1) * rows_per_group) - g * rows_per_group)
        for q in range(plan.n_chunks):
            lo, hi = int(en[g, q, 0]), int(en[g, q, 1])
            if hi > lo:
                total += rows * (hi - lo) * int(ch[q, 2])
    return total


class partial_backward:

    def __enter__(self):
        global _PARTIAL_BACKWARD
        self._prev, _PARTIAL_BACKWARD = _PARTIAL_BACKWARD, True
        return self

    def __exit__(self, *exc):
        global _PARTIAL_BACKWARD
        _PARTIAL_BACKWARD = self._prev
        return False


def _want_weight_grad(spec=None) -> bool:
    return (not _PARTIAL_BACKWARD) or bool(getattr(spec, "always_weight_grad", False))

Tensor = torch.Tensor


def _ncl(t: Tensor, name: str) -> Tuple[int, int]:
    _lib.require_gpu_tensor(t, name)
    if t.dim() != 3 or t.stride(2) != 1 or (t.size(1) > 1 and t.stride(1) != t.size(2)):
        raise ValueError(f"{name}: expected NCL view with channel stride L, got shape {tuple(t.shape)} strides {t.stride()}")
    return t.stride(0), t.size(2)


def _same_numel(*tensors: Optional[Tensor]) -> int:
    ts = [t for t in tensors if t is not None]
    n = ts[0].numel()
    for t in ts:
        if t.numel() != n or not t.is_contiguous():
            raise ValueError(f"pointwise launch over tensors of different extents / non-contiguous: {[tuple(x.shape) for x in ts]}")
    return n


def _gate_numel(acts: Tensor, *pairs: Tensor) -> int:
    n = _same_numel(acts)
    for t in pairs:
        if t.numel() != 2 * n or not t.is_contiguous():
            raise ValueError(f"gate launch: {tuple(t.shape)} is not the contiguous [B, 2n, L] partner of {tuple(acts.shape)}")
    return n


def _wsrc(t: Optional[Tensor], off0: int, sm: int, sc: int, st: int) -> WSrc:
    if t is not None:
        _lib.require_gpu_tensor(t, "weight")
    return WSrc(ptr(t) if t is not None else None, off0, sm, sc, st)


_PACK_CACHE: Optional[dict] = None


class pack_cache:

    def __enter__(self):
        global _PACK_CACHE
        self._prev, _PACK_CACHE = _PACK_CACHE, {}
        return self

    def __exit__(self, *exc):
        global _PACK_CACHE
        _PACK_CACHE = self._prev
        return False


def pack_weights(plan: Plan, M: int, w0: Tensor, s0: Tuple[int, int, int, int], w1: Optional[Tensor] = None,
                 s1: Tuple[int, int, int, int] = (0, 0, 0, 0), parts=None, bf3: bool = False) -> Tensor:
    if _PACK_CACHE is not None:
        key = (id(plan), bf3, M, w0.data_ptr(), w0._version, s0, None if w1 is None else (w1.data_ptr(), w1._version), s1,
               None if parts is None else tuple((p[0], p[1], p[2], p[3], p[4].data_ptr(), p[4]._version, p[5]) for p in parts))
        hit = _PACK_CACHE.get(key)
        if hit is not None:
            return hit[0]
        a = _pack_weights(plan, M, w0, s0, w1, s1, parts, bf3)
        _PACK_CACHE[key] = (a, w0, w1, plan, parts)
        return a
    return _pack_weights(plan, M, w0, s0, w1, s1, parts, bf3)


def _pack_weights(plan: Plan, M: int, w0: Tensor, s0, w1: Optional[Tensor], s1, parts=None, bf3: bool = False) -> Tensor:
    lib = _lib.load()
    a = torch.empty(plan.packed_floats_bf3 if bf3 else plan.packed_floats, device=w0.device, dtype=torch.float32)
    fn, who = (lib.fst_pack_weights_bf16x3, "fst_pack_weights_bf16x3") if bf3 else (lib.fst_pack_weights, "fst_pack_weights")
    second = (w1, s1)
    if parts is None:
        parts = [(0, -1, 0, M, w0, s0)]
    else:
        second = (None, (0, 0, 0, 0))
    for (g0, g1, row_base, row_end, w, sw) in parts:
        src0 = _wsrc(w, *sw)
        src1 = _wsrc(second[0], *second[1]) if second[0] is not None else None
        check(fn(ptr(plan.dev(w0.device)), plan.host_ptr(), plan.length, ctypes.byref(src0),
                 ctypes.byref(src1) if src1 is not None else None, row_end, g0, g1, row_base, ptr(a), stream_ptr()), who)
    return a


def unpack_weights(plan: Plan, M: int, a: Tensor, dw0: Tensor, s0, dw1: Optional[Tensor] = None, s1=(0, 0, 0, 0)) -> None:
    lib = _lib.load()
    n_slabs = a.size(0) if a.dim() == 2 else 1
    check(lib.fst_unpack_weights(ptr(plan.dev(a.device)), plan.host_ptr(), plan.length, ptr(a), M, ptr(dw0), *s0,
                                 ptr(dw1), *s1, n_slabs, stream_ptr()), "fst_unpack_weights")


def conv_gemm(plan: Plan, a: Tensor, x0: Tensor, x1: Optional[Tensor], bias: Optional[Tensor], B: int, L: int, M: int,
              y: Optional[Tensor], res: Optional[Tensor] = None, y2: Optional[Tensor] = None, msplit: Optional[int] = None,
              nb: int = 1, ksplit: int = 1, flags: int = 0, m2_start: Optional[int] = None, bf3: bool = False) -> None:
    lib = _lib.load()
    if bf3:
        flags |= GEMM_BF16X3
    msplit = M if msplit is None else msplit
    m2_start = msplit if m2_start is None else m2_start
    x0_bs, _ = _ncl(x0, "x0")
    x1_bs = _ncl(x1, "x1")[0] if x1 is not None else 0
    y_bs = _ncl(y, "y")[0] if y is not None else 0
    res_bs = _ncl(res, "res")[0] if res is not None else 0
    y2_bs = _ncl(y2, "y2")[0] if y2 is not None else 0
    t0 = KERNEL_TIMER.begin() if KERNEL_TIMER is not None else None
    check(lib.fst_conv_gemm(ptr(x0), x0_bs, ptr(x1), x1_bs, ptr(a), ptr(plan.dev(x0.device)), plan.host_ptr(),
                            plan.length, ptr(bias), ptr(y), y_bs, ptr(res), res_bs, ptr(y2), y2_bs, msplit, m2_start, B, L,
                            M, nb, ksplit, flags, stream_ptr()), "fst_conv_gemm")
    if t0 is not None:
        key = route_kernel_name(last_route())
        if KERNEL_TIMER.detail:
            key += f" M={M} rec={plan.total_records} dil={plan.dil}"
        rows_in = x0.size(1) + (x1.size(1) if x1 is not None else 0) + (res.size(1) if res is not None else 0)
        rows_out = (msplit if y is not None else 0) + ((M - m2_start) if y2 is not None else 0)
        if y2 is not None and flags & EPI_ACC2:
            rows_in += M - m2_start
        if flags & EPI_ACC1 and y is not None:
            rows_in += msplit
        KERNEL_TIMER.end(key, t0, 2.0 * B * L * _plan_macs_per_step(plan, M), 4.0 * B * L * (rows_in + rows_out))


def conv_wgrad(plan: Plan, x0: Tensor, x1: Optional[Tensor], dy: Tensor, dy2: Optional[Tensor], msplit: int, B: int,
               L: int, M: int, ksplit: int, x0_mul_off: int = 0) -> Tensor:
    lib = _lib.load()
    n_slabs = max(1, min(ksplit, B * ((L + 31) // 32)))
    da = torch.empty(n_slabs, plan.packed_floats, device=x0.device, dtype=torch.float32)
    x0_bs, _ = _ncl(x0, "x0")
    x1_bs = _ncl(x1, "x1")[0] if x1 is not None else 0
    dy_bs, _ = _ncl(dy, "dy")
    dy2_bs = _ncl(dy2, "dy2")[0] if dy2 is not None else 0
    t0 = KERNEL_TIMER.begin() if KERNEL_TIMER is not None else None
    bf3 = MATH == "bf16x3"
    check(lib.fst_conv_wgrad(ptr(x0), x0_bs, ptr(x1), x1_bs, ptr(dy), dy_bs, ptr(dy2), dy2_bs, msplit, ptr(da),
                             ptr(plan.dev(x0.device)), plan.host_ptr(), plan.length, B, L, M, ksplit,
                             (GEMM_BF16X3 if bf3 else 0) | WGRAD_SLABS, x0_mul_off, stream_ptr()),
          "fst_conv_wgrad")
    if t0 is not None:
        key = route_kernel_name(last_route())
        if KERNEL_TIMER.detail:
            key += f" M={M} rec={plan.total_records} ksplit={ksplit}"
        rows_in = x0.size(1) + (x1.size(1) if x1 is not None else 0) + M
        KERNEL_TIMER.end(key, t0, 2.0 * B * L * _plan_macs_per_step(plan, M), 4.0 * B * L * rows_in + 8.0 * plan.packed_floats)
    return da


def row_sum(x: Tensor, out: Optional[Tensor] = None) -> Tensor:
    lib = _lib.load()
    bs, L = _ncl(x, "x")
    B, C = x.size(0), x.size(1)
    if out is None:
        out = torch.empty(C, device=x.device, dtype=torch.float32)
    check(lib.fst_row_sum(ptr(x), bs, B, C, L, ptr(out), stream_ptr()), "fst_row_sum")
    return out


def wgrad_ksplit(B: int, L: int, n_wg_per_slice: int) -> int:
    tiles = B * ((L + 31) // 32)
    target = 384 if n_wg_per_slice == 1 else 512
    k = max(1, target // max(1, n_wg_per_slice))
    if k >= 16:
        k -= k % 8
    return max(1, min(tiles, k))


class ConvSpec:

    def __init__(self, M: int, C0: int, ntaps: int = 1, dil: int = 1, pad_left: int = 0, C1: int = 0,
                 row_live: Optional[Sequence[Tuple[int, int]]] = None, dense_dw: bool = True):
        self.M, self.C0, self.ntaps, self.dil, self.pad_left, self.C1 = M, C0, ntaps, dil, pad_left, C1
        self.row_live = list(row_live) if row_live is not None else None
        self.dense_dw = dense_dw
        self.dense_if_fast = False
        if C1:
            if pad_left % dil or not (0 <= pad_left // dil < ntaps):
                raise ValueError("the 1x1 side input needs a tap with zero offset")
        self.x1_tap = pad_left // dil if C1 else 0
        self._plans: Dict[Tuple[str, int], Plan] = {}
        self.mb = 1 if self.row_live is not None and ntaps > 2 else pick_mb(M)

    def dense_tap_wgrad_ok(self, B: int, L: int, x0: Tensor, dy: Tensor) -> bool:
        if self.C1 or MATH != "bf16x3" or not (self.dense_dw or self.row_live is None or self.dense_if_fast) or self.dil != 1:
            return False
        if not (x0.is_contiguous() and dy.is_contiguous()):
            return False
        if x0.data_ptr() % 16 or dy.data_ptr() % 16 or dy.size(1) != self.M or x0.size(1) != self.C0:
            return False
        return bool(_lib.load().fst_dense_tap_wgrad_ok(B, L, self.M, self.C0, self.ntaps, self.pad_left))

    def tap_wgrad_ok(self, B: int, L: int, x0: Tensor, dy: Tensor) -> bool:
        if self.C1 or MATH != "bf16x3" or not (self.dense_dw or self.row_live is None) or self.ntaps < 2 or self.C0 < 64:
            return False
        if os.environ.get("FST_TAP_WGRAD", "0") != "1" or not (x0.is_contiguous() and dy.is_contiguous()):
            return False
        if x0.data_ptr() % 16 or dy.data_ptr() % 16:
            return False
        served = _lib.load().fst_tap_wgrad_ok(B, L, self.M, self.C0, self.ntaps, self.dil, self.pad_left)
        return served == 1 or (served == 2 and has_slack(x0))

    def _halo(self) -> int:
        return (self.ntaps - 1) * self.dil

    def nb_for(self, B: int, L: int, mb: int, windowed_c: int, halo: int) -> int:
        tiles128 = (L + 127) // 128
        win_bf3 = windowed_c >= 8 and MATH == "bf16x3"
        if win_bf3:
            windowed_c, mb = min(windowed_c, PIPE_C), min(mb, 2)
        best = 1
        for nb in ((4, 2, 1) if windowed_c else (2, 1)):
            if mb * nb > (4 if win_bf3 else 8) or nb > max(1, tiles128):
                continue
            if windowed_c and windowed_c <= 64 and ((windowed_c + 1) & ~1) * (128 * nb + halo) * 4 > LDS_BUDGET:
                continue
            if windowed_c > 64 and nb > 2:
                continue
            best = nb
            if B * ((L + 128 * nb - 1) // (128 * nb)) >= 512:
                break
        return best

    def _fwd_segments(self) -> List[Segment]:
        segs = [Segment(0, self.C0, 0, self.ntaps)]
        if self.C1:
            segs.append(Segment(1, self.C1, self.x1_tap, self.x1_tap + 1))
        return segs

    def _windowed(self, channels: int) -> bool:
        return self.dil == 1 and self.ntaps > 3

    def _chunking(self, channels: int, nb: int, ntaps: int) -> Tuple[int, bool]:
        if not self._windowed(channels):
            return PIPE_C, True
        if MATH == "bf16x3" and channels >= 8:
            return PIPE_C, False
        halo = (ntaps - 1) * self.dil
        cap = (LDS_BUDGET // (4 * (128 * nb + halo))) & ~1
        if channels <= cap:
            return (channels + 1) & ~1, False
        cap = (LDS_MULTI_CHUNK // (4 * (128 * nb + halo))) & ~1
        n = (channels + cap - 1) // cap
        return ((channels + n - 1) // n + 1) & ~1, False

    def fwd_plan(self, nb: int) -> Plan:
        key = ("fwd", nb)
        if key not in self._plans:
            chunk_c, split = self._chunking(max(self.C0, self.C1), nb, self.ntaps)
            mb = min(self.mb, 2) if (chunk_c == PIPE_C and not split) else self.mb
            self._plans[key] = build_plan(self.M, self._fwd_segments(), self.ntaps, self.dil, self.pad_left, MB=mb,
                                          chunk_c=chunk_c, split_taps=split, row_live=self.row_live)
        return self._plans[key]

    def dx0_plan(self, nb: int) -> Plan:
        key = ("dx0", nb)
        if key not in self._plans:
            col_live = None
            if self.row_live is not None:
                col_live = [(self.ntaps - hi, self.ntaps - lo) for lo, hi in self.row_live]
# ... 226 lines not shown


def gemm(A: Tensor, ta: bool, B: Tensor, tb: bool, bias: Optional[Tensor] = None, act: int = ACT_NONE, slope: float = 0.0) -> Tensor:
    if not gemm_ok(A, B):
        raise ValueError(f"gemm: operands {tuple(A.shape)} / {tuple(B.shape)} must be fp32 matrices with unit column stride on the GPU "
                         f"(split-bf16 mode; FST_MATH={MATH})")
    return _gemm_launch("gemm", "gemm_bf3_kernel bf3", A, ta, B, tb, bias, act, slope)


def gemm_f32_ok(*ts: Tensor) -> bool:
    return all(t.is_cuda and t.dtype == torch.float32 and t.dim() == 2 and t.numel() > 0 and t.stride(1) == 1
               and t.stride(0) >= t.size(1) for t in ts)


def gemm_f32(A: Tensor, ta: bool, B: Tensor, tb: bool, bias: Optional[Tensor] = None, act: int = ACT_NONE, slope: float = 0.0) -> Tensor:
    if not gemm_f32_ok(A, B):
        raise ValueError(f"gemm_f32: operands {tuple(A.shape)} / {tuple(B.shape)} must be fp32 matrices with unit column stride on the GPU")
    return _gemm_launch("gemm_f32", "gemm_f32_kernel f32", A, ta, B, tb, bias, act, slope)


def _gemm_rows(t: Tensor) -> Tensor:
    if t.stride(1) == 1 and t.stride(0) >= t.size(1):
        return t
    return torch.empty(t.shape, device=t.device, dtype=t.dtype).copy_(t)


def act_bwd(dy: Tensor, y: Tensor, slope: float) -> Tensor:
    dy = _aligned16(dy)
    out = torch.empty_like(dy)
    check(_lib.load().fst_act_bwd(ptr(dy), ptr(y), ptr(out), _same_numel(dy, y), float(slope), stream_ptr()), "fst_act_bwd")
    return out


class LinearActFn(torch.autograd.Function):

    @staticmethod
    def forward(ctx, x: Tensor, W: Tensor, b: Optional[Tensor], act: int, slope: float):
        x2 = x.reshape(-1, x.size(-1))
        if x2.stride(1) != 1 or x2.stride(0) < x2.size(1):
            x2 = _gemm_rows(x2.contiguous())
        y = gemm(x2, False, W, False, b, act, slope)
        ctx.save_for_backward(x2, W, y if act != ACT_NONE else None)
        ctx.lead, ctx.act, ctx.slope, ctx.has_bias = x.shape[:-1], act, slope, b is not None
        return y.view(*ctx.lead, W.size(0))

    @staticmethod
    def backward(ctx, dy):
        x2, W, y = ctx.saved_tensors
        g = dy.reshape(-1, W.size(0))
        g = act_bwd(g, y, ctx.slope if ctx.act == ACT_LEAKY else 0.0) if ctx.act != ACT_NONE else g.contiguous()
        g = _gemm_rows(g)
        dx = gemm(g, False, W, True).view(*ctx.lead, W.size(1)) if ctx.needs_input_grad[0] else None
        dW = gemm(g, True, x2, True) if ctx.needs_input_grad[1] and _want_weight_grad() else None
        db = g.sum(dim=0) if ctx.has_bias and ctx.needs_input_grad[2] and _want_weight_grad() else None
        return dx, dW, db, None, None


def linear_act(x: Tensor, lin: "torch.nn.Linear", act: int = ACT_NONE, slope: float = 0.0) -> Tensor:
    if x.is_cuda and x.dtype == torch.float32 and MATH == "bf16x3" and x.numel() > 0 and lin.weight.numel() > 0:
        return LinearActFn.apply(x, lin.weight, lin.bias, act, slope)
    h = torch.nn.functional.linear(x, lin.weight, lin.bias)
    if act == ACT_RELU:
        return torch.nn.functional.relu(h)
    if act == ACT_LEAKY:
        return torch.nn.functional.leaky_relu(h, slope)
    return h


def mask_taps_(w: Tensor, lo: Tensor, hi: Tensor) -> None:
    lib = _lib.load()
    M, C, K = w.shape
    check(lib.fst_mask_taps(ptr(w), ptr(lo), ptr(hi), M, C, K, stream_ptr()), "fst_mask_taps")


BN_SLOTS = 16


class _RowSums:

    @staticmethod
    def attach(dx: Tensor, rs: Tensor) -> None:
        dx._fst_row_sums = (rs, dx._version)

    @staticmethod
    def take(dy: Tensor) -> Optional[Tensor]:
        tag = getattr(dy, "_fst_row_sums", None)
        if tag is None or dy.dim() != 3:
            return None
        rs, version = tag
        if version != dy._version or tuple(rs.shape) != tuple(dy.shape[:2]) or not dy.is_contiguous():
            return None
        return rs


_ROW_SUMS = _RowSums()


def _bn_stats(y: Tensor, gamma: Tensor, beta: Tensor, rmean: Tensor, rvar: Tensor, training: bool, eps: float,
              momentum: float) -> Tensor:
    lib = _lib.load()
    B, C, L = y.shape
    stats = torch.empty(4 * C, device=y.device, dtype=torch.float32)
    part, n_slots = None, 0
    if training:
        part = torch.empty(C, BN_SLOTS, 4, device=y.device, dtype=torch.float32)
        check(lib.fst_bn_stats(ptr(y), B, C, L, ptr(part), y.numel(), stream_ptr()), "fst_bn_stats")
        part = _dist.gather_slots(part)
        n_slots = part.size(1)
    check(lib.fst_bn_finalize(ptr(part), n_slots, ptr(gamma), ptr(beta), ptr(rmean), ptr(rvar), int(training), C, eps,
                              momentum, ptr(stats), stream_ptr()), "fst_bn_finalize")
    return stats


def _bn_slot_sum(part: Tensor) -> Tensor:
    red = part[..., 0].clone()
    for s in range(1, part.size(-1)):
        red += part[..., s]
    return red


def _bn_backward(dy: Tensor, y: Tensor, out: Optional[Tensor], stats: Tensor, relu: bool, training: bool,
                 need_dx: bool = True):
    lib = _lib.load()
    B, C, L = y.shape
    part = torch.empty(2, C, BN_SLOTS, device=y.device, dtype=torch.float32)
    check(lib.fst_bn_bwd_reduce(ptr(dy), ptr(y), ptr(out), ptr(stats), B, C, L, int(relu), ptr(part), _same_numel(dy, y, out),
                                stream_ptr()),
          "fst_bn_bwd_reduce")
    if not need_dx:
        red = _bn_slot_sum(part).view(2 * C)
        return None, red[C:], red[:C]
    dx = torch.empty_like(y)
    rs = torch.empty(B, C, device=y.device, dtype=torch.float32)
    if training and _dist.global_batch_active():
        red = part.sum(dim=2).view(2 * C)
        red_g = red.clone()
        B_total = _dist.sum_over_ranks_(red_g) * B
        check(lib.fst_bn_bwd_apply(ptr(dy), ptr(y), ptr(out), ptr(stats), ptr(red_g), 1, None, ptr(dx), ptr(rs), B, C, L, int(relu),
                                   int(training), B_total, _same_numel(dy, y, out, dx), stream_ptr()), "fst_bn_bwd_apply")
    else:
        red = torch.empty(2 * C, device=y.device, dtype=torch.float32)
        check(lib.fst_bn_bwd_apply(ptr(dy), ptr(y), ptr(out), ptr(stats), ptr(part), BN_SLOTS, ptr(red), ptr(dx), ptr(rs), B, C, L,
                                   int(relu), int(training), B, _same_numel(dy, y, out, dx), stream_ptr()), "fst_bn_bwd_apply")
    _ROW_SUMS.attach(dx, rs)
    return dx, red[C:], red[:C]


def _bn_backward_join(dy: Tensor, ya: Tensor, yb: Tensor, sa: Tensor, sb: Tensor, training: bool, need_dxa: bool,
                      need_dxb: bool):
    lib = _lib.load()
    B, C, L = ya.shape
    dev = ya.device
    parts = torch.empty(2, 2, C, BN_SLOTS, device=dev, dtype=torch.float32)
    check(lib.fst_bn_bwd_reduce_join(ptr(dy), ptr(ya), ptr(yb), ptr(sa), ptr(sb), B, C, L, ptr(parts[0]), ptr(parts[1]),
                                     _same_numel(dy, ya, yb), stream_ptr()), "fst_bn_bwd_reduce_join")
    need = (need_dxa, need_dxb)
    dx = [torch.empty_like(y) if n else None for y, n in zip((ya, yb), need)]
    rs = [torch.empty(B, C, device=dev, dtype=torch.float32) if n else None for n in need]
    red = [None, None]
    if any(need):
        if training and _dist.global_batch_active():
            local = parts.sum(dim=3).view(2, 2 * C)
            red_g = local.clone()
            B_total = _dist.sum_over_ranks_(red_g) * B
            check(lib.fst_bn_bwd_apply_join(ptr(dy), ptr(ya), ptr(yb), ptr(sa), ptr(sb), ptr(red_g[0]), ptr(red_g[1]), 1, None, None,
                                            ptr(dx[0]), ptr(dx[1]), ptr(rs[0]), ptr(rs[1]), B, C, L, int(training), B_total,
                                            _same_numel(dy, ya, yb, *dx), stream_ptr()), "fst_bn_bwd_apply_join")
            red = [local[i] if need[i] else None for i in range(2)]
        else:
            sums = torch.empty(2, 2 * C, device=dev, dtype=torch.float32)
            check(lib.fst_bn_bwd_apply_join(ptr(dy), ptr(ya), ptr(yb), ptr(sa), ptr(sb), ptr(parts[0]), ptr(parts[1]), BN_SLOTS,
                                            ptr(sums[0]) if need[0] else None, ptr(sums[1]) if need[1] else None,
                                            ptr(dx[0]), ptr(dx[1]), ptr(rs[0]), ptr(rs[1]), B, C, L, int(training), B,
                                            _same_numel(dy, ya, yb, *dx), stream_ptr()), "fst_bn_bwd_apply_join")
            red = [sums[i] if need[i] else None for i in range(2)]
    res = []
    for i in range(2):
        if need[i]:
            _ROW_SUMS.attach(dx[i], rs[i])
        else:
            red[i] = _bn_slot_sum(parts[i]).view(2 * C)
        res.append((dx[i], red[i][C:], red[i][:C]))
    return res


class BNActFn(torch.autograd.Function):

    @staticmethod
    def forward(ctx, y, gamma, beta, rmean, rvar, training: bool, relu: bool, eps: float, momentum: float):
        lib = _lib.load()
        y = y.contiguous()
        B, C, L = y.shape
        stats = _bn_stats(y, gamma, beta, rmean, rvar, training, eps, momentum)
        out = torch.empty_like(y)
        check(lib.fst_bn_apply(ptr(y), ptr(stats), None, None, ptr(out), B, C, L, int(relu), _same_numel(y, out), stream_ptr()),
              "fst_bn_apply")
        ctx.save_for_backward(y, stats)
        ctx.relu, ctx.training = relu, training
        return out

    @staticmethod
    def backward(ctx, dout):
        y, stats = ctx.saved_tensors
        dx, dg, db = _bn_backward(dout.contiguous(), y, None, stats, ctx.relu, ctx.training, ctx.needs_input_grad[0])
        return dx, dg, db, None, None, None, None, None, None


class BNAddBNReluFn(torch.autograd.Function):

    @staticmethod
    def forward(ctx, ya, ga, ba, rma, rva, yb, gb, bb, rmb, rvb, training: bool, eps: float, momentum: float):
        lib = _lib.load()
        ya, yb = ya.contiguous(), yb.contiguous()
        B, C, L = ya.shape
        sa = _bn_stats(ya, ga, ba, rma, rva, training, eps, momentum)
        sb = _bn_stats(yb, gb, bb, rmb, rvb, training, eps, momentum)
        out = torch.empty_like(ya)
        check(lib.fst_bn_apply(ptr(ya), ptr(sa), ptr(yb), ptr(sb), ptr(out), B, C, L, 1, _same_numel(ya, yb, out), stream_ptr()),
              "fst_bn_apply")
        ctx.save_for_backward(ya, yb, sa, sb)
        ctx.training = training
        return out

    @staticmethod
    def backward(ctx, dout):
        ya, yb, sa, sb = ctx.saved_tensors
        (dxa, dga, dba), (dxb, dgb, dbb) = _bn_backward_join(dout.contiguous(), ya, yb, sa, sb, ctx.training,
                                                             ctx.needs_input_grad[0], ctx.needs_input_grad[5])
        return dxa, dga, dba, None, None, dxb, dgb, dbb, None, None, None, None, None


class WNSpecs:

    def __init__(self, h: int, n: int, n_layers: int = 8, kernel: int = 3):
        self.h, self.n, self.n_layers, self.kernel = h, n, n_layers, kernel
        self.start = ConvSpec(n, h)
        self.ins = [ConvSpec(2 * n, n, kernel, 2 ** i, int((kernel * 2 ** i - 2 ** i) / 2), C1=h) for i in range(n_layers)]
        self.rs = [ConvSpec(2 * n if i < n_layers - 1 else n, n) for i in range(n_layers)]
        self.end = ConvSpec(2 * h, n)
        self.rs_T = build_plan(n, [Segment(0, n, 0, 1), Segment(1, n, 0, 1)], 1, 1, 0, chunk_c=PIPE_C)
        self.rs_T_last = build_plan(n, [Segment(0, n, 0, 1)], 1, 1, 0, chunk_c=PIPE_C)
        nl = n_layers
        self.shapes = ([(n, h, 1), (n,), (2 * n * nl, h, 1), (2 * n * nl,), (2 * h, n, 1), (2 * h,)]
                       + [(2 * n, n, kernel)] * nl + [(2 * n,)] * nl
                       + [(2 * n if i < nl - 1 else n, n, 1) for i in range(nl)] + [(2 * n if i < nl - 1 else n,) for i in range(nl)])
        self.offsets = [0]
        for sh in self.shapes:
            self.offsets.append(self.offsets[-1] + int(math.prod(sh)))
        self.flat_numel = self.offsets[-1]

    def flatten(self, weights: Sequence[Tensor]) -> Tensor:
        assert len(weights) == len(self.shapes) and all(tuple(w.shape) == sh for w, sh in zip(weights, self.shapes))
        return torch.cat([w.reshape(-1) for w in weights])

    def unflatten(self, flat: Tensor) -> List[Tensor]:
        assert flat.numel() == self.flat_numel and flat.is_contiguous()
        return [flat[self.offsets[i]: self.offsets[i + 1]].view(sh) for i, sh in enumerate(self.shapes)]


def wn_wgrad_ok(kind: int, B: int, L: int, n: int, h: int, dil: int, a: Optional[Tensor] = None) -> bool:
    if MATH != "bf16x3" or os.environ.get("FST_WN_WGRAD", "1") == "0":
        return False
    served = _lib.load().fst_wn_wgrad_ok(kind, B, L, n, h, dil)
    return served == 1 or (served == 2 and a is not None and has_slack(a))


def empty_with_slack(B: int, C: int, L: int, device) -> Tensor:
    buf = torch.empty(B * C * L + 8, device=device, dtype=torch.float32)
    return buf[4: 4 + B * C * L].view(B, C, L)


def has_slack(t: Tensor) -> bool:
    off = t.storage_offset()
    return t.is_contiguous() and off >= 4 and t.untyped_storage().nbytes() >= (off + t.numel() + 4) * 4


WN_WGRAD_MAX_SETS = 3


def _sets(x) -> list:
    return list(x) if isinstance(x, (list, tuple)) else [x]


def _wgrad_sets(who: str, *operands) -> List[list]:
    sets = [_sets(o) for o in operands]
    if not (1 <= len(sets[0]) <= WN_WGRAD_MAX_SETS and all(len(s) == len(sets[0]) for s in sets)):
        raise ValueError(f"{who}: {'/'.join(str(len(s)) for s in sets)} operand sets (1..{WN_WGRAD_MAX_SETS}, equally many)")
    return sets


def _wn_wgrad_launch(kind: int, last: bool, ns: int, B: int, L: int, n: int, h: int, device, targets: tuple, slabs: Optional[list],
                     launch, timer: tuple) -> None:
    lib = _lib.load()
    ws_n = lib.fst_wn_wgrad_workspace_floats(kind, B, L, n, h, int(last))
    ws = torch.empty(ws_n, device=device, dtype=torch.float32)
    t0 = KERNEL_TIMER.begin() if KERNEL_TIMER is not None else None
    launch(lib, ptr(ws), ws_n, slabs is not None)
    if slabs is not None:
        slabs.append((kind, bool(last), ns, ws) + targets)
    if t0 is not None:
        KERNEL_TIMER.end(timer[0], t0, timer[1], timer[2])


def wn_wgrad_in(dg, a, u0, dw_in: Tensor, dw_cond: Tensor, n: int, h: int, dil: int, slabs: Optional[list] = None) -> None:
    dgs, as_, u0s = _wgrad_sets("wn_wgrad_in", dg, a, u0)
    B, _, L = dgs[0].shape
    u0_bs, _ = _ncl(u0s[0], "u0")
    numel = _same_numel(*as_)
    slack = True
    for dg_s, a_s, u0_s in zip(dgs, as_, u0s):
        if dg_s.numel() != 2 * numel or not dg_s.is_contiguous() or tuple(a_s.shape) != (B, n, L) or tuple(u0_s.shape) != (B, h, L):
            raise ValueError("wn_wgrad_in: dg must be contiguous [B, 2n, L], a [B, n, L], u0 [B, h, L]")
        if _ncl(u0_s, "u0")[0] != u0_bs:
            raise ValueError("wn_wgrad_in: the operand sets' u0 tensors must share one batch stride")
        slack = slack and has_slack(a_s)
    for t, sh in ((dw_in, (2 * n, n, 3)), (dw_cond, (2 * n, h, 1))):
        if tuple(t.shape) != sh or not t.is_contiguous() or t.dtype != torch.float32:
            raise ValueError(f"wn_wgrad_in: gradient target of shape {tuple(t.shape)}, expected contiguous {sh}")
    ns = len(dgs)

    def launch(lib, ws, ws_n, keep_slabs):
        sets = (_ptr_sets(dgs), _ptr_sets(as_), _ptr_sets(u0s), ns, u0_bs)
        shape = (B, L, n, h, dil, int(slack), numel, stream_ptr())
        if keep_slabs:
            check(lib.fst_wn_wgrad_in_slabs(*sets, ws, ws_n, *shape), "fst_wn_wgrad_in_slabs")
        else:
            check(lib.fst_wn_wgrad_in(*sets, ptr(dw_in), ptr(dw_cond), ws, ws_n, *shape), "fst_wn_wgrad_in")

    _wn_wgrad_launch(0, False, ns, B, L, n, h, dgs[0].device, (dw_in, dw_cond), slabs, launch,
                     ("wn_wgrad_kernel<2, 3> bf3", 2.0 * ns * B * L * 2 * n * (3 * n + h), 4.0 * ns * B * L * (2 * n + n + h)))


def wn_wgrad_rs(d_a, d_out, ts, dw_rs: Tensor, last: bool, n: int, slabs: Optional[list] = None) -> None:
    d_as, d_outs, tss = _wgrad_sets("wn_wgrad_rs", [None] * len(_sets(d_out)) if d_a is None else d_a, d_out, ts)
    B, _, L = d_outs[0].shape
    numel = _same_numel(*d_outs, *[t for t in d_as if t is not None])
    M = n if last else 2 * n
    for da_s, ts_s in zip(d_as, tss):
        if ts_s.numel() != 2 * numel or not ts_s.is_contiguous() or (da_s is None) != bool(last):
            raise ValueError("wn_wgrad_rs: ts must be contiguous [B, 2n, L]; d_a is None exactly on the last layer")
    if tuple(dw_rs.shape) != (M, n, 1) or not dw_rs.is_contiguous() or dw_rs.dtype != torch.float32:
        raise ValueError(f"wn_wgrad_rs: gradient target of shape {tuple(dw_rs.shape)}, expected contiguous {(M, n, 1)}")
    ns = len(d_outs)

    def launch(lib, ws, ws_n, keep_slabs):
        sets = (None if last else _ptr_sets(d_as), _ptr_sets(d_outs), _ptr_sets(tss), ns)
        shape = (int(last), B, L, n, numel, stream_ptr())
        if keep_slabs:
            check(lib.fst_wn_wgrad_rs_slabs(*sets, ws, ws_n, *shape), "fst_wn_wgrad_rs_slabs")
        else:
            check(lib.fst_wn_wgrad_rs(*sets, ptr(dw_rs), ws, ws_n, *shape), "fst_wn_wgrad_rs")

    _wn_wgrad_launch(1, last, ns, B, L, n, 0, d_outs[0].device, (dw_rs, None), slabs, launch,
                     ("wn_wgrad_kernel<2, 2> bf3", 2.0 * ns * B * L * M * n, 4.0 * ns * B * L * (M + 2 * n)))


WN_WGRAD_MAX_REDUCE = 16


def wn_wgrad_reduce_many(slabs: list, B: int, L: int, n: int, h: int) -> None:
    lib = _lib.load()
    for c0 in range(0, len(slabs), WN_WGRAD_MAX_REDUCE):
        chunk = slabs[c0: c0 + WN_WGRAD_MAX_REDUCE]
        ne = len(chunk)
        ints = lambda vals: (ctypes.c_int32 * ne)(*[int(v) for v in vals])
        check(lib.fst_wn_wgrad_reduce_many(ints(e[0] for e in chunk), ints(e[1] for e in chunk), ints(e[2] for e in chunk),
                                           _ptr_table([e[3] for e in chunk]), (ctypes.c_int64 * ne)(*[e[3].numel() for e in chunk]),
                                           _ptr_table([e[4] for e in chunk]), _ptr_table([e[5] for e in chunk]), ne, B, L, n, h,
                                           stream_ptr()), "fst_wn_wgrad_reduce_many")
    del slabs[:]


def _tap_wgrad(who: str, taps_name: str, timer_key: str, dy: Tensor, x: Tensor, dw: Tensor, M: int, C: int, taps: int, *geometry) -> None:
    lib = _lib.load()
    B, _, L = dy.shape
    if tuple(dy.shape) != (B, M, L) or tuple(x.shape) != (B, C, L) or not (dy.is_contiguous() and x.is_contiguous()):
        raise ValueError(f"{who}: dy {tuple(dy.shape)} / x {tuple(x.shape)} must be contiguous [B, {M}, L] / [B, {C}, L]")
    if tuple(dw.shape) != (M, C, taps) or not dw.is_contiguous() or dw.dtype != torch.float32:
        raise ValueError(f"{who}: gradient target of shape {tuple(dw.shape)}, expected contiguous {(M, C, taps)}")
    ws_n = getattr(lib, f"fst_{who}_workspace_floats")(B, L, M, C, taps)
    if ws_n <= 0:
        raise ValueError(f"{who}: unsupported shape B={B} L={L} M={M} C={C} {taps_name}={taps}")
    ws = torch.empty(ws_n, device=dy.device, dtype=torch.float32)
    t0 = KERNEL_TIMER.begin() if KERNEL_TIMER is not None else None
    check(getattr(lib, f"fst_{who}")(ptr(dy), ptr(x), ptr(dw), ptr(ws), ws_n, B, L, M, C, taps, *geometry, dy.numel(), x.numel(),
                                     stream_ptr()), f"fst_{who}")
    if t0 is not None:
        KERNEL_TIMER.end(timer_key, t0, 2.0 * B * L * M * C * taps, 4.0 * B * L * (M + C))


def dense_tap_wgrad(dy: Tensor, x: Tensor, dw: Tensor, M: int, C: int, K: int, pad_left: int) -> None:
    _tap_wgrad("dense_tap_wgrad", "K", f"tz_wgrad_kernel M={M} C={C} bf3", dy, x, dw, M, C, K, pad_left)


def tap_wgrad(dy: Tensor, x: Tensor, dw: Tensor, M: int, C: int, ntaps: int, dil: int, pad_left: int) -> None:
    _tap_wgrad("tap_wgrad", "ntaps", "tap_wgrad (wn_wgrad_kernel<2, 3>) bf3", dy, x, dw, M, C, ntaps, dil, pad_left, int(has_slack(x)))


def _ptr_sets(ts: Sequence[Tensor]):
    arr = (ctypes.c_void_p * len(ts))()
    for i, t in enumerate(ts):
        if t.dtype != torch.float32 or not t.is_cuda:
            raise ValueError("operand sets must be fp32 device tensors")
        arr[i] = t.data_ptr()
    return arr


class WNGradPool:

    def __init__(self):
        self.pending: dict = {}
        self.task = None

    def add(self, key, operands) -> None:
        task = torch._C._current_graph_task_id()
        if task != self.task:
            self.pending, self.task = {}, task
        self.pending.setdefault(key, []).append(operands)

    def take(self) -> dict:
        pending, self.pending = self.pending, {}
        return pending if self.task == torch._C._current_graph_task_id() else {}


class WGradJoinFn(torch.autograd.Function):

    @staticmethod
    def forward(ctx, pool: WNGradPool, specs: "WNSpecs", flat: Tensor):
        ctx.pool, ctx.specs = pool, specs
        return flat.view_as(flat)

    @staticmethod
    def backward(ctx, g):
        S, pool = ctx.specs, ctx.pool
        pending = pool.take()
        if not pending:
            return None, None, g
        g = g.contiguous()
        nl, n, h = S.n_layers, S.n, S.h
        dw = S.unflatten(g)
        g_cond_w, g_in_w, g_rs_w = dw[2], dw[6: 6 + nl], dw[6 + 2 * nl: 6 + 3 * nl]
        slabs, later = {}, []
        for (kind, i), sets in pending.items():
            groups = {}
            for s in sets:
                lead = s[0] if kind == 0 else s[1]
                shape = (lead.size(0), lead.size(2)) + ((s[2].stride(0),) if kind == 0 else ())
                groups.setdefault(shape, []).append(s)
            own = True
            for shape, members in groups.items():
                for c0 in range(0, len(members), WN_WGRAD_MAX_SETS):
                    chunk = members[c0: c0 + WN_WGRAD_MAX_SETS]
                    cols = [list(col) for col in zip(*chunk)]
                    to = None if c0 else slabs.setdefault(shape[:2], [])
                    if kind == 0:
                        t_in, t_cond = g_in_w[i], g_cond_w[2 * n * i: 2 * n * (i + 1)]
                        if not own:
                            t_in, t_cond = torch.empty_like(t_in), torch.empty_like(t_cond)
                            later += [(g_in_w[i], t_in), (g_cond_w[2 * n * i: 2 * n * (i + 1)], t_cond)]
                        wn_wgrad_in(cols[0], cols[1], cols[2], t_in, t_cond, n, h, 2 ** i, slabs=to)
                    else:
                        last = i == nl - 1
                        t_rs = g_rs_w[i]
                        if not own:
                            t_rs = torch.empty_like(t_rs)
                            later.append((g_rs_w[i], t_rs))
                        wn_wgrad_rs(None if last else cols[0], cols[1], cols[2], t_rs, last, n, slabs=to)
                    own = False
        for (B, L), entries in slabs.items():
            wn_wgrad_reduce_many(entries, B, L, n, h)
        for seg, t in later:
            seg.add_(t)
        return None, None, g


class WNFoldPlan:

    def __init__(self, specs: "WNSpecs", normed: Sequence[bool]):
        assert len(normed) == len(specs.shapes)
        self.specs, self.normed = specs, list(normed)
        self._key, self._table = None, None
        self.n_rows = sum(sh[0] if nm else 1 for sh, nm in zip(specs.shapes, normed))
        self.grad_offsets, off = [], 0
        for sh, nm in zip(specs.shapes, normed):
            numel = int(math.prod(sh))
            self.grad_offsets.append(off)
            off += numel
            if nm:
                self.grad_offsets.append(off)
                off += sh[0]
        self.grad_numel = off

    def n_inputs(self) -> int:
        return len(self.grad_offsets)

    def table(self, tensors: Sequence[Tensor]) -> Tensor:
        import numpy as np
        key = tuple(t.data_ptr() for t in tensors) + (str(tensors[0].device),)
        if key == self._key:
            return self._table
        rows, it, gi = [], iter(tensors), 0
        for i, (sh, nm) in enumerate(zip(self.specs.shapes, self.normed)):
            dst, numel = self.specs.offsets[i], int(math.prod(sh))
            if nm:
                v, g = next(it), next(it)
                M, rowlen = sh[0], numel // sh[0]
                assert v.is_contiguous() and g.is_contiguous() and tuple(v.shape) == tuple(sh) and g.numel() == M
                m = np.arange(M, dtype=np.int64)
                blk = np.stack([v.data_ptr() + 4 * rowlen * m, g.data_ptr() + 4 * m, dst + rowlen * m, np.full(M, rowlen, np.int64),
                                self.grad_offsets[gi] + rowlen * m, self.grad_offsets[gi + 1] + m], axis=1)
                gi += 2
            else:
                t = next(it)
                assert t.is_contiguous() and t.numel() == numel
                blk = np.array([[t.data_ptr(), 0, dst, numel, self.grad_offsets[gi], 0]], dtype=np.int64)
                gi += 1
            rows.append(blk)
        tab = np.concatenate(rows, axis=0)
        assert tab.shape == (self.n_rows, 6)
        self._table = torch.from_numpy(tab).to(tensors[0].device)
        self._key = key
        return self._table


class WNFoldFn(torch.autograd.Function):

    @staticmethod
    def forward(ctx, plan: WNFoldPlan, *tensors: Tensor):
        lib = _lib.load()
        assert len(tensors) == plan.n_inputs()
        for t in tensors:
            _lib.require_gpu_tensor(t, "WN parameter")
        tab = plan.table(tensors)
        dev = tensors[0].device
        flat = torch.empty(plan.specs.flat_numel, device=dev, dtype=torch.float32)
        norms = torch.empty(plan.n_rows, device=dev, dtype=torch.float32)
        check(lib.fst_wn_fold_fwd(ptr(tab), plan.n_rows, ptr(flat), ptr(norms), stream_ptr()), "fst_wn_fold_fwd")
        ctx.plan, ctx.tab = plan, tab
        ctx.shapes = [tuple(t.shape) for t in tensors]
        ctx.save_for_backward(norms)
        return flat

    @staticmethod
    def backward(ctx, d_flat):
        lib = _lib.load()
        (norms,) = ctx.saved_tensors
        plan: WNFoldPlan = ctx.plan
        d_flat = d_flat.contiguous()
        dpar = torch.empty(plan.grad_numel, device=d_flat.device, dtype=torch.float32)
        check(lib.fst_wn_fold_bwd(ptr(ctx.tab), plan.n_rows, ptr(d_flat), ptr(norms), ptr(dpar), stream_ptr()), "fst_wn_fold_bwd")
        grads = []
        for off, sh in zip(plan.grad_offsets, ctx.shapes):
            grads.append(dpar[off: off + int(math.prod(sh))].view(sh))
        return (None, *grads)


def wn_fused_ok(n: int, h: int, L: int, *tensors: Tensor, kernel: int = 3) -> bool:
    if MATH != "bf16x3" or kernel != 3 or not (0 < n < 128) or L % 4 != 0 or os.environ.get("FST_WN_FUSED", "1") == "0":
        return False
    return all(t.data_ptr() % 16 == 0 and t.stride(0) % 4 == 0 for t in tensors)


WN_PACK_MAX_LAYERS = 10


class _WnImages(NamedTuple):
    nl: int
    key: Callable
    nbytes: Callable
    sources: Callable
    one: Optional[Callable]
    stack: Callable


def _pack_one(f: _WnImages, i: int) -> Tensor:
    if _PACK_CACHE is not None:
        hit = _PACK_CACHE.get(f.key(i))
        if hit is not None:
            return hit[0]
    src = [t.contiguous() for t in f.sources(i)]
    img = torch.empty(f.nbytes(i) // 4, device=src[0].device, dtype=torch.float32)
    f.one(i, src, img)
    if _PACK_CACHE is not None:
        _PACK_CACHE[f.key(i)] = (img, *f.sources(i), src)
    return img


def _pack_stack(f: _WnImages) -> List[Tensor]:
    hits = [None if _PACK_CACHE is None else _PACK_CACHE.get(f.key(i)) for i in range(f.nl)]
    if _PACK_CACHE is not None and all(hit is not None for hit in hits):
        return [hit[0] for hit in hits]
    if f.one is not None and (f.nl > WN_PACK_MAX_LAYERS or any(hit is not None for hit in hits)):
        return [_pack_one(f, i) for i in range(f.nl)]
    srcs = [[t.contiguous() for t in f.sources(i)] for i in range(f.nl)]
    imgs = [torch.empty(f.nbytes(i) // 4, device=srcs[i][0].device, dtype=torch.float32) for i in range(f.nl)]
    f.stack(srcs, imgs)
    if _PACK_CACHE is not None:
        for i, img in enumerate(imgs):
            _PACK_CACHE[f.key(i)] = (img, *f.sources(i), srcs[i])
    return imgs


def _wn_fwd_images(who: str, layers: Sequence[Sequence[Tensor]], lasts: Sequence[bool], n: int, h: int) -> _WnImages:
    lib, nl = _lib.load(), len(layers)
    for in_w in (l[0] for l in layers):
        if in_w.dim() != 3 or in_w.size(0) != 2 * n or in_w.size(1) != n:
            raise ValueError(f"{who}: in_w must be [2n, n, taps], got {tuple(in_w.shape)} for n={n}")
    nbytes = lib.fst_wn_image_bytes(n, h)
    return _WnImages(
        nl, lambda i: ("wn", n, h, lasts[i]) + tuple((t.data_ptr(), t._version) for t in layers[i]), lambda i: nbytes,
        lambda i: layers[i],
        lambda i, src, img: check(lib.fst_wn_pack(*[ptr(t) for t in src], n, h, layers[i][0].size(2), int(lasts[i]), ptr(img), nbytes,
                                                  stream_ptr()), "fst_wn_pack"),
        lambda srcs, imgs: check(lib.fst_wn_pack_stack(*[_ptr_table([l[j] for l in srcs]) for j in range(6)], nl, n, h,
                                                       layers[0][0].size(2), _ptr_table(imgs), nbytes, stream_ptr()),
                                 "fst_wn_pack_stack"))


def wn_pack_layer(in_w: Tensor, cond_w: Tensor, in_b: Tensor, cond_b: Tensor, rs_w: Tensor, rs_b: Tensor, n: int, h: int,
                  last: bool) -> Tensor:
    return _pack_one(_wn_fwd_images("wn_pack_layer", [(in_w, cond_w, in_b, cond_b, rs_w, rs_b)], [last], n, h), 0)


def wn_pack_layers(layers: Sequence[Sequence[Tensor]], n: int, h: int) -> List[Tensor]:
    nl = len(layers)
    return _pack_stack(_wn_fwd_images("wn_pack_layers", layers, [i == nl - 1 for i in range(nl)], n, h))


def _wn_bwd_images(rs_ws: Sequence[Tensor], lasts: Sequence[bool], n: int, acc_order: bool) -> _WnImages:
    lib, nl = _lib.load(), len(rs_ws)
    nbytes = lambda i: lib.fst_wn_bwd_image_bytes(n, int(lasts[i]))
    return _WnImages(
        nl, lambda i: ("wn_bwd", n, lasts[i], acc_order, rs_ws[i].data_ptr(), rs_ws[i]._version), nbytes, lambda i: (rs_ws[i],),
        lambda i, src, img: check(lib.fst_wn_pack_bwd(ptr(src[0]), n, int(lasts[i]), int(acc_order), ptr(img), nbytes(i), stream_ptr()),
                                  "fst_wn_pack_bwd"),
        lambda srcs, imgs: check(lib.fst_wn_pack_bwd_stack(_ptr_table([s_[0] for s_ in srcs]), nl, n, int(acc_order), _ptr_table(imgs),
                                                           lib.fst_wn_bwd_image_bytes(n, 0), stream_ptr()), "fst_wn_pack_bwd_stack"))


def wn_pack_bwd(rs_w: Tensor, n: int, last: bool, acc_order: bool = False) -> Tensor:
    return _pack_one(_wn_bwd_images([rs_w], [last], n, acc_order), 0)


def wn_pack_bwd_layers(rs_ws: Sequence[Tensor], n: int, acc_order: bool = False) -> List[Tensor]:
    nl = len(rs_ws)
    return _pack_stack(_wn_bwd_images(rs_ws, [i == nl - 1 for i in range(nl)], n, acc_order))


def wn_pack_bwd_proj_layers(rs_ws: Sequence[Tensor], end_w: Tensor, n: int) -> List[Tensor]:
    lib, nl, h2 = _lib.load(), len(rs_ws), end_w.size(0)
    if nl > WN_PACK_MAX_LAYERS or tuple(end_w.shape) != (h2, n, 1) or h2 > 64:
        raise ValueError(f"wn_pack_bwd_proj_layers: {nl} layers, end_w {tuple(end_w.shape)} (at most {WN_PACK_MAX_LAYERS} layers, "
                         f"end_w [2h <= 64, n = {n}, 1])")
    return _pack_stack(_WnImages(
        nl, lambda i: ("wn_bwd_proj", n, h2, i == nl - 1, rs_ws[i].data_ptr(), rs_ws[i]._version, end_w.data_ptr(), end_w._version),
        lambda i: lib.fst_wn_bwd_proj_image_bytes(n, h2, int(i == nl - 1)), lambda i: (rs_ws[i], end_w), None,
        lambda srcs, imgs: check(lib.fst_wn_pack_bwd_proj_stack(_ptr_table([s_[0] for s_ in srcs]), ptr(srcs[0][1]), nl, n, h2,
                                                                _ptr_table(imgs), lib.fst_wn_bwd_proj_image_bytes(n, h2, 0),
                                                                stream_ptr()), "fst_wn_pack_bwd_proj_stack")))


def _wn_dgrad_images(in_ws: Sequence[Tensor], cond_ws: Sequence[Tensor], n: int, h: int) -> _WnImages:
    lib, nl = _lib.load(), len(in_ws)
    nbytes = lib.fst_wn_dgrad_image_bytes(n)
    return _WnImages(
        nl, lambda i: ("wn_dgrad", n, h, in_ws[i].data_ptr(), in_ws[i]._version, cond_ws[i].data_ptr(), cond_ws[i]._version),
        lambda i: nbytes, lambda i: (in_ws[i], cond_ws[i]),
        lambda i, src, img: check(lib.fst_wn_pack_dgrad(ptr(src[0]), ptr(src[1]), n, h, in_ws[i].size(2), ptr(img), nbytes, stream_ptr()),
                                  "fst_wn_pack_dgrad"),
        lambda srcs, imgs: check(lib.fst_wn_pack_dgrad_stack(_ptr_table([s_[0] for s_ in srcs]), _ptr_table([s_[1] for s_ in srcs]), nl, n,
                                                             h, in_ws[0].size(2), _ptr_table(imgs), nbytes, stream_ptr()),
                                 "fst_wn_pack_dgrad_stack"))


def wn_pack_dgrad(in_w: Tensor, cond_w: Tensor, n: int, h: int) -> Tensor:
    return _pack_one(_wn_dgrad_images([in_w], [cond_w], n, h), 0)


def wn_pack_dgrad_layers(in_ws: Sequence[Tensor], cond_ws: Sequence[Tensor], n: int, h: int) -> List[Tensor]:
    return _pack_stack(_wn_dgrad_images(in_ws, cond_ws, n, h))


def _wn_layer_forward(save: bool, a: Tensor, u0: Tensor, img: Tensor, ts: Optional[Tensor], acts: Optional[Tensor],
                      a_next: Optional[Tensor], out: Tensor, first: bool, last: bool, n: int, h: int, dil: int) -> None:
    lib = _lib.load()
    a_bs, L = _ncl(a, "a")
    u0_bs, _ = _ncl(u0, "u0")
    B = a.size(0)
    numel = _same_numel(a, out, acts, a_next)
    if save and (ts.numel() != 2 * numel or not ts.is_contiguous()):
        raise ValueError("wn_layer_fwd: ts must be the contiguous [B, 2n, L] partner of a")
    if save:
        fn, who, key, saved = lib.fst_wn_layer_fwd, "fst_wn_layer_fwd", "wn_layer_fwd_kernel", (ptr(ts), ptr(acts))
    else:
        fn, who, key, saved = lib.fst_wn_layer_infer, "fst_wn_layer_infer", "wn_layer_infer_kernel", ()
    t0 = KERNEL_TIMER.begin() if KERNEL_TIMER is not None else None
    check(fn(ptr(a), a_bs, ptr(u0), u0_bs, ptr(img), img.numel() * 4, *saved, ptr(a_next), ptr(out), int(first), int(last), B, L, n, h,
             dil, numel, stream_ptr()), who)
    if t0 is not None:
        rs_rows = n if last else 2 * n
        flops = 2.0 * B * L * (2 * n * (3 * n + h) + rs_rows * n)
        rows = n + h + (0 if first else n) + (0 if last else n) + n
        rows += (2 * n if save else 0) + (n if acts is not None else 0)
        KERNEL_TIMER.end(key, t0, flops, 4.0 * B * L * rows)


def wn_layer_fwd(a: Tensor, u0: Tensor, img: Tensor, ts: Tensor, acts: Optional[Tensor], a_next: Optional[Tensor], out: Tensor,
                 first: bool, last: bool, n: int, h: int, dil: int) -> None:
    _wn_layer_forward(True, a, u0, img, ts, acts, a_next, out, first, last, n, h, dil)


def wn_layer_infer(a: Tensor, u0: Tensor, img: Tensor, a_next: Optional[Tensor], out: Tensor, first: bool, last: bool, n: int, h: int,
                   dil: int) -> None:
    _wn_layer_forward(False, a, u0, img, None, None, a_next, out, first, last, n, h, dil)


def wn_bwd_partials(n_layers: int, B: int, L: int, device) -> Tensor:
    return torch.empty(n_layers, 256, B * ((L + 127) // 128), device=device, dtype=torch.float32)


def wn_layer_bwd(d_a: Optional[Tensor], d_out: Tensor, ts: Tensor, img: Tensor, dg: Tensor, last: bool, n: int,
                 want_row_sums: bool = False, sums_out: Optional[Tensor] = None, part: Optional[Tensor] = None) -> Optional[Tensor]:
    lib = _lib.load()
    B, _, L = d_out.shape
    deferred = part is not None
    if part is None and want_row_sums:
        part = torch.empty(256, B * ((L + 127) // 128), device=dg.device, dtype=torch.float32)
    numel = _same_numel(d_out, d_a)
    for t in (ts, dg):
        if t.numel() != 2 * numel or not t.is_contiguous():
            raise ValueError("wn_layer_bwd: ts / dg must be contiguous [B, 2n, L]")
    if part is not None and (part.shape != (256, B * ((L + 127) // 128)) or not part.is_contiguous()):
        raise ValueError(f"wn_layer_bwd: partial-sum slab of shape {tuple(part.shape)}")
    t0 = KERNEL_TIMER.begin() if KERNEL_TIMER is not None else None
    check(lib.fst_wn_layer_bwd(ptr(d_a), ptr(d_out), ptr(ts), ptr(img), img.numel() * 4, ptr(dg), ptr(part),
                               0 if part is None else part.size(1), int(last), B, L, n, numel, stream_ptr()), "fst_wn_layer_bwd")
    if t0 is not None:
        k = n if last else 2 * n
        KERNEL_TIMER.end("wn_layer_bwd_kernel", t0, 2.0 * B * L * n * k, 4.0 * B * L * (k + 4 * n))
    if part is None or deferred:
        return None
    if sums_out is not None:
        return torch.sum(part[: 2 * n], dim=1, out=sums_out)
    return part.sum(dim=1)[: 2 * n]


WN_DGRAD_TILE = 512


def wn_dgrad_ok(n: int, h: int, dil: int) -> bool:
    return bool(_lib.load().fst_wn_dgrad_fits(n, h, dil))


def wn_dgrad_partials(n_layers: int, B: int, L: int, device) -> Tensor:
    return torch.empty(n_layers, 128, B * ((L + WN_DGRAD_TILE - 1) // WN_DGRAD_TILE), device=device, dtype=torch.float32)


def wn_layer_dgrad(dg: Tensor, img: Tensor, d_a: Optional[Tensor], d_u0: Tensor, n: int, h: int, dil: int,
                   want_row_sums: bool = False, sums_out: Optional[Tensor] = None, part: Optional[Tensor] = None):
    lib = _lib.load()
    B, _, L = dg.shape
    deferred = part is not None
    if part is None and want_row_sums:
        part = torch.empty(128, B * ((L + WN_DGRAD_TILE - 1) // WN_DGRAD_TILE), device=dg.device, dtype=torch.float32)
    d_a_new = torch.empty(B, n, L, device=dg.device, dtype=torch.float32)
    numel = _same_numel(d_a_new, d_a)
    if dg.numel() != 2 * numel or not dg.is_contiguous():
        raise ValueError("wn_layer_dgrad: dg must be contiguous [B, 2n, L]")
    d_u0_bs, _ = _ncl(d_u0, "d_u0")
    if tuple(d_u0.shape) != (B, h, L):
        raise ValueError(f"wn_layer_dgrad: d_u0 must be [B, h, L] = {(B, h, L)}, got {tuple(d_u0.shape)}")
# ... 1027 lines not shown
```

### include/fst_hip.h

```cpp
#ifndef FST_HIP_H
#define FST_HIP_H

#include <stdint.h>

#ifdef __cplusplus
extern "C" {
#endif

#define FST_ABI_VERSION 26

int fst_version(void);
const char* fst_last_error(void);

#define FST_PLAN_HEADER 16

typedef struct {
  const float* w;
  int64_t off0, sm, sc, st;
} fst_wsrc;

int fst_pack_weights(const int32_t* plan_dev, const int32_t* plan_host, int plan_len,
                     const fst_wsrc* src0_host, const fst_wsrc* src1_host,
                     int M, int g_begin, int g_end , int row_base ,
                     float* a_packed, void* stream);

int fst_pack_weights_bf16x3(const int32_t* plan_dev, const int32_t* plan_host, int plan_len,
                            const fst_wsrc* src0_host, const fst_wsrc* src1_host,
                            int M, int g_begin, int g_end, int row_base, void* a_image, void* stream);

int fst_unpack_weights(const int32_t* plan_dev, const int32_t* plan_host, int plan_len,
                       const float* a_packed, int M,
                       float* dw0, int64_t off0_0, int64_t sm0, int64_t sc0, int64_t st0,
                       float* dw1, int64_t off0_1, int64_t sm1, int64_t sc1, int64_t st1,
                       int n_slabs ,
                       void* stream);

int fst_mask_taps(float* w, const int32_t* live_lo, const int32_t* live_hi, int M, int C, int K, void* stream);

#define FST_EPI_RELU    1
#define FST_EPI_ACC2    2
#define FST_EPI_ATOMIC  4
#define FST_EPI_ACC1    8
#define FST_GEMM_BF16X3 16
#define FST_WGRAD_SLABS 32
int fst_conv_gemm(const float* x0, int64_t x0_bs, const float* x1, int64_t x1_bs,
                  const float* a_packed, const int32_t* plan_dev, const int32_t* plan_host, int plan_len,
                  const float* bias,
                  float* y, int64_t y_bs, const float* res, int64_t res_bs,
                  float* y2, int64_t y2_bs, int msplit, int m2_start ,
                  int B, int L, int M, int nb_cfg, int ksplit, int flags, void* stream);

int fst_conv_wgrad(const float* x0, int64_t x0_bs, const float* x1, int64_t x1_bs,
                   const float* dy, int64_t dy_bs, const float* dy2, int64_t dy2_bs, int msplit,
                   float* da_packed, const int32_t* plan_dev, const int32_t* plan_host, int plan_len,
                   int B, int L, int M, int ksplit, int flags , int64_t x0_mul_off, void* stream);

#define FST_ROUTE_GEMM      1
#define FST_ROUTE_PIPE      2
#define FST_ROUTE_BF3       3
#define FST_ROUTE_WIN_BF3   4
#define FST_ROUTE_WIN_ROWS  5
#define FST_ROUTE_WGRAD     6
#define FST_ROUTE_EPI_PLAIN   0
#define FST_ROUTE_EPI_ADD     1
#define FST_ROUTE_EPI_ATOMIC  2
#define FST_ROUTE_EPI_VEC     3
#define FST_ROUTE_EPI_VEC_ADD 4
int fst_conv_last_route(int32_t out[8]);

int fst_row_sum(const float* x, int64_t x_bs, int B, int C, int L, float* out, void* stream);

#define FST_BN_SLOTS 16
int fst_bn_stats(const float* y, int B, int C, int L, float* part , int64_t numel, void* stream);
int fst_bn_finalize(const float* part, int n_slots, const float* gamma, const float* beta,
                    float* running_mean, float* running_var, int train, int C, float eps, float momentum,
                    float* stats, void* stream);
int fst_bn_apply(const float* y, const float* stats, const float* res, const float* res_stats,
                 float* out, int B, int C, int L, int relu, int64_t numel, void* stream);
int fst_bn_bwd_reduce(const float* dy, const float* y, const float* out, const float* stats,
                      int B, int C, int L, int relu, float* red , int64_t numel, void* stream);
int fst_bn_bwd_apply(const float* dy, const float* y, const float* out, const float* stats, const float* red, int n_slots,
                     float* red_out, float* dx, float* row_sums, int B, int C, int L, int relu, int train, int B_total,
                     int64_t numel, void* stream);
int fst_bn_bwd_reduce_join(const float* dy, const float* ya, const float* yb, const float* stats_a, const float* stats_b,
                           int B, int C, int L, float* red_a, float* red_b, int64_t numel, void* stream);
int fst_bn_bwd_apply_join(const float* dy, const float* ya, const float* yb, const float* stats_a, const float* stats_b,
                          const float* red_a, const float* red_b, int n_slots, float* red_out_a, float* red_out_b,
                          float* dxa, float* dxb, float* row_sums_a, float* row_sums_b, int B, int C, int L, int train,
                          int B_total, int64_t numel, void* stream);

int fst_gate_fwd(float* g_ts, float* acts, int B, int n, int L, int64_t numel_acts, void* stream);
int fst_gate_bwd(const float* ts, const float* dacts, float* dg, int B, int n, int L, int64_t numel_acts, void* stream);
int64_t fst_coupling_sum_slots(int B, int h, int L);
int fst_coupling_fwd(const float* u, const float* o, float* xn, int B, int h, int L, int64_t numel, float* sums, void* stream);
int fst_coupling_bwd(const float* u, const float* o, const float* dxn, const float* dlogs, const float* g_ls, const float* g_sq,
                     float* du, float* d_o, int B, int h, int L, int64_t numel, void* stream);
int fst_coupling_inv_fwd(const float* x, const float* o, float* xn, int B, int h, int L, int64_t numel, void* stream);
int fst_coupling_inv_bwd(const float* xn, const float* o, const float* dxn,
                         float* dx, float* d_o, int B, int h, int L, int64_t numel, void* stream);

int fst_wn_fold_fwd(const int64_t* table_dev, int n_rows, float* flat, float* norms , void* stream);
int fst_wn_fold_bwd(const int64_t* table_dev, int n_rows, const float* d_flat, const float* norms, float* dpar, void* stream);

int fst_logdet_inv(const float* W, int n, float* out , float* inv_t , void* stream);

int64_t fst_wn_image_bytes(int n, int h);
int fst_wn_pack(const float* in_w, const float* cond_w, const float* in_b, const float* cond_b,
                const float* rs_w, const float* rs_b, int n, int h, int ntaps , int last, void* image, int64_t image_bytes, void* stream);
int fst_wn_pack_stack(const float* const* in_w, const float* const* cond_w, const float* const* in_b, const float* const* cond_b,
                      const float* const* rs_w, const float* const* rs_b, int nl, int n, int h, int ntaps, void* const* images,
                      int64_t image_bytes, void* stream);
int fst_wn_pack_bwd_stack(const float* const* rs_w, int nl, int n, int acc_order, void* const* images, int64_t image_bytes,
                          void* stream);
int fst_wn_pack_dgrad_stack(const float* const* in_w, const float* const* cond_w, int nl, int n, int h, int ntaps,
                            void* const* images, int64_t image_bytes, void* stream);
int64_t fst_wn_bwd_proj_image_bytes(int n, int h2, int last);
int fst_wn_pack_bwd_proj_stack(const float* const* rs_w, const float* end_w, int nl, int n, int h2, void* const* images,
                               int64_t image_bytes, void* stream);
int fst_wn_layer_fwd(const float* a, int64_t a_bs, const float* u0, int64_t u0_bs, const void* image, int64_t image_bytes,
                     float* ts, float* acts, float* a_next, float* out, int first, int last,
                     int B, int L, int n, int h, int dil, int64_t numel_a, void* stream);

int64_t fst_wn_bwd_image_bytes(int n, int last);
int fst_wn_pack_bwd(const float* rs_w, int n, int last,
                    int acc_order ,
                    void* image, int64_t image_bytes, void* stream);
int fst_wn_layer_bwd(const float* d_a_next , const float* d_out, const float* ts, const void* image,
                     int64_t image_bytes, float* dg,
                     float* row_sums ,
                     int64_t row_sums_rows, int last, int B, int L, int n, int64_t numel_a, void* stream);

int64_t fst_wn_dgrad_image_bytes(int n);
int fst_wn_pack_dgrad(const float* in_w, const float* cond_w, int n, int h, int ntaps , void* image,
                      int64_t image_bytes, void* stream);
int fst_wn_dgrad_fits(int n, int h, int dil);
int fst_wn_layer_dgrad(const float* dg, const void* image, int64_t image_bytes, const float* d_a, float* d_a_new, float* d_u0,
                       float* row_sums , int64_t row_sums_rows,
                       int B, int L, int n, int h, int dil, int64_t numel_a, int64_t d_u0_bs, void* stream);

int fst_wn_stack_fwd_ok(int n, int h, int L, int nl);
int fst_wn_stack_fwd(const float* const* a_in, const int64_t* a_bs, const void* const* images, int64_t image_bytes, float* const* ts,
                     float* const* a_next, const float* u0, int64_t u0_bs, float* out, int nl, int B, int L, int n, int h,
                     int64_t numel_a, void* stream);

int fst_wn_layer_infer(const float* a, int64_t a_bs, const float* u0, int64_t u0_bs, const void* image, int64_t image_bytes,
                       float* a_next, float* out, int first, int last, int B, int L, int n, int h, int dil, int64_t numel_a,
                       void* stream);
int fst_wn_stack_infer(const float* const* a_in, const int64_t* a_bs, const void* const* images, int64_t image_bytes,
                       float* const* a_next, const float* u0, int64_t u0_bs, float* out, int nl, int B, int L, int n, int h,
                       int64_t numel_a, void* stream);

int fst_wn_stack_bwd_ok(int n, int h, int L, int nl);
int fst_wn_stack_bwd(const float* const* ts, const void* const* img_b, const void* const* img_d, float* const* dg,
                     float* const* da_out, float* const* rs_b , float* const* rs_d ,
                     const float* d_out, float* d_u0, int64_t d_u0_bs, int nl, int B, int L, int n, int h, int64_t numel_a,
                     void* stream);
int fst_wn_stack_bwd_proj(const float* const* ts, const void* const* img_b, const void* const* img_d, float* const* dg,
                          float* const* da_out, float* const* rs_b , float* const* rs_d ,
                          const float* d_o, int h2, int64_t numel_o, float* d_u0, int64_t d_u0_bs, int nl, int B, int L, int n,
                          int h, int64_t numel_a, void* stream);

int fst_wn_wgrad_ok(int kind, int B, int L, int n, int h, int dil);
int64_t fst_wn_wgrad_workspace_floats(int kind, int B, int L, int n, int h, int last);
int fst_wn_wgrad_in(const float* const* dg, const float* const* a, const float* const* u0, int n_sets, int64_t u0_bs, float* dw_in,
                    float* dw_cond, float* workspace, int64_t workspace_floats, int B, int L, int n, int h, int dil, int a_slack,
                    int64_t numel_a, void* stream);
int fst_wn_wgrad_rs(const float* const* d_a , const float* const* d_out, const float* const* ts, int n_sets,
                    float* dw_rs, float* workspace, int64_t workspace_floats, int last, int B, int L, int n, int64_t numel_a,
                    void* stream);
int fst_wn_wgrad_in_slabs(const float* const* dg, const float* const* a, const float* const* u0, int n_sets, int64_t u0_bs,
                          float* workspace, int64_t workspace_floats, int B, int L, int n, int h, int dil, int a_slack,
                          int64_t numel_a, void* stream);
int fst_wn_wgrad_rs_slabs(const float* const* d_a , const float* const* d_out, const float* const* ts, int n_sets,
                          float* workspace, int64_t workspace_floats, int last, int B, int L, int n, int64_t numel_a, void* stream);
int fst_wn_wgrad_reduce_many(const int32_t* kind, const int32_t* last, const int32_t* n_sets, float* const* workspace,
                             const int64_t* workspace_floats, float* const* dw0, float* const* dw1, int n_entries, int B, int L,
                             int n, int h, void* stream);

int64_t fst_nt_gemm_workspace_floats(int M, int N, int K);
int fst_nt_gemm(const float* A, const float* Bm, float* C, float* workspace, int64_t workspace_floats, int M, int N, int K,
                const float* epi_p , const float* epi_r1 , int epi_ncls, float epi_scale,
                float* epi_raw , void* stream);

int fst_tap_wgrad_ok(int B, int L, int M, int C, int ntaps, int dil, int pad_left);
int64_t fst_tap_wgrad_workspace_floats(int B, int L, int M, int C, int ntaps);
int fst_tap_wgrad(const float* dy, const float* x, float* dw , float* workspace, int64_t workspace_floats,
                  int B, int L, int M, int C, int ntaps, int dil, int pad_left, int x_slack, int64_t numel_dy, int64_t numel_x,
                  void* stream);

int fst_dense_tap_wgrad_ok(int B, int L, int M, int C, int K, int pad_left);
int64_t fst_dense_tap_wgrad_workspace_floats(int B, int L, int M, int C, int K);
int fst_dense_tap_wgrad(const float* dy, const float* x, float* dw , float* workspace, int64_t workspace_floats,
                        int B, int L, int M, int C, int K, int pad_left, int64_t numel_dy, int64_t numel_x, void* stream);

#define FST_WN_ROUTE_LEN         12
#define FST_WN_ROUTE_WGRAD       1
#define FST_WN_ROUTE_TZ          2
#define FST_WN_ROUTE_LAYER_FWD   3
#define FST_WN_ROUTE_STACK_FWD   4
#define FST_WN_ROUTE_LAYER_BWD   5
#define FST_WN_ROUTE_LAYER_DGRAD 6
#define FST_WN_ROUTE_STACK_BWD   7
#define FST_WN_ROUTE_LAYER_INFER 8
#define FST_WN_ROUTE_STACK_INFER 9
int fst_wn_last_route(int32_t out[FST_WN_ROUTE_LEN]);

int fst_batch_sum(const float* x0, const float* x1, float* part, int B, int64_t N, int S, void* stream);
int fst_noise_transfer_fwd(const float* part, int S, int B, const float* r_t_dev, const float* r_s_dev, float r_t, float r_s,
                           float* avg_t, float* avg_s, const float* W, const float* bias, float* dist, float* pre, float* learned,
                           int C, int L, void* stream);
int fst_bcast_add(float* out, const float* x, const float* v, int B, int64_t N, void* stream);
int fst_noise_transfer_bwd(const float* part, int S, const float* pre, const float* W, float* dpre, float* dd, int C, int L,
                           void* stream);
int fst_noise_transfer_dw(const float* dpre, const float* dist, float* dW, float* dbias, int C, int L, void* stream);
int fst_noise_transfer_bwd_apply(const float* g, const float* dd, const float* r_t_dev, const float* r_s_dev, float r_t, float r_s,
                                 int B, float* dz_t, float* dz_s, int64_t N, void* stream);

int fst_relu_bwd(const float* dy, const float* y, float* out, int64_t n, void* stream);

#define FST_ACT_NONE  0
#define FST_ACT_RELU  1
#define FST_ACT_LEAKY 2
int64_t fst_gemm_workspace_floats(int M, int N, int K);
int fst_gemm(const float* A, int64_t lda, int ta, const float* B, int64_t ldb, int tb, float* C, int64_t ldc, int M, int N, int K,
             const float* bias, int act, float slope, float* workspace, int64_t workspace_floats, void* stream);
int64_t fst_gemm_f32_workspace_floats(int M, int N, int K);
int fst_gemm_f32(const float* A, int64_t lda, int ta, const float* B, int64_t ldb, int tb, float* C, int64_t ldc, int M, int N, int K,
                 const float* bias, int act, float slope, float* workspace, int64_t workspace_floats, void* stream);
int fst_act_bwd(const float* dy, const float* y, float* out, int64_t n, float slope, void* stream);
int fst_axpy(float* y, const float* x, float alpha, int64_t n, void* stream);
int fst_add_slices(float* dst, int64_t dst_bs, const float* a, int64_t a_bs, const float* b, int64_t b_bs,
                   int B, int C, int L, void* stream);

int64_t fst_cpc_workspace_floats(int T, int B, int C, int Bc);
int64_t fst_cpc_nce_slots(int T, int B, int C, int Bc);
int fst_cpc_nce_fwd(const float* enc, int64_t s_i, int64_t s_b, int64_t s_c, const int32_t* t0_dev ,
                    const float* pred , int T, int B, int C,
                    int Bc , int col_off ,
                    float* lse , float* nce_sum , float* workspace ,
                    void* stream);
int fst_cpc_nce_bwd(const float* enc, int64_t s_i, int64_t s_b, int64_t s_c, const int32_t* t0_dev ,
                    const float* pred, const float* lse, int T, int B, int C, int Bc, int col_off, const float* gout,
                    float* denc , float* dpred , void* stream);

int fst_gru_fwd(const float* xproj, const float* w_hh, const float* b_hh, float* h_all, float* gates,
                const int32_t* t_last_dev, int t_last, int B, int S, int H, int64_t numel_h, void* stream);
int fst_gru_bwd(const float* w_hh, const float* h_all, const float* gates, const float* dout,
                const int32_t* t_last_dev, int t_last, float* dxproj, float* dgh, int B, int S, int H,
                int64_t numel_h, void* stream);

int fst_lstm2_fwd(const float* xproj, const float* w_hh_t, float* h2, float* save, int B, int H, int64_t numel_xproj, void* stream);
int fst_lstm2_bwd(const float* w_hh, const float* save, const float* dh2, float* dxproj, float* dpre2, int B, int H,
                  int64_t numel_xproj, void* stream);

int fst_rmsprop_multi(float* const* p_host, const float* const* g_host, float* const* v_host, const int64_t* numel_host,
                      const float* lr_host, int n_tensors, float alpha, float eps, void* stream);
int fst_adam_multi(float* const* p_host, const float* const* g_host, float* const* m_host, float* const* v_host,
                   const int64_t* numel_host, int n_tensors, const float* step_dev, float lr, float beta1, float beta2, float eps,
                   void* stream);
int fst_rmsprop_multi_dev(float* const* p_host, const float* const* g_host, float* const* v_host, const int64_t* numel_host,
                          const float* const* lr_dev_host, int n_tensors, float alpha, float eps, void* stream);
int fst_adam_multi_dev(float* const* p_host, const float* const* g_host, float* const* m_host, float* const* v_host,
                       const int64_t* numel_host, int n_tensors, const float* step_dev, const float* lr_dev, float beta1, float beta2,
                       float eps, void* stream);

int64_t fst_nonfinite_slots(int n_tensors);
int fst_nonfinite_multi(const float* const* x_host, const int64_t* numel_host, const int32_t* group_host, int n_tensors,
                        int32_t verdict_mask, int32_t* slots_dev, int64_t slots_len, int32_t* counts_dev, int32_t* verdict_dev,
                        float* ok_dev, int32_t* skipped_dev, void* stream);
int fst_rmsprop_multi_guard(float* const* p_host, const float* const* g_host, float* const* v_host, const int64_t* numel_host,
                            const float* lr_host, const float* const* lr_dev_host, int n_tensors, float alpha, float eps,
                            const int32_t* verdict_dev, void* stream);
int fst_adam_multi_guard(float* const* p_host, const float* const* g_host, float* const* m_host, float* const* v_host,
                         const int64_t* numel_host, int n_tensors, const float* step_dev, float lr, const float* lr_dev, float beta1,
                         float beta2, float eps, const int32_t* verdict_dev, void* stream);
int fst_guard_copy_multi(void* const* dst_host, const void* const* src_host, const int64_t* words_host, int n_tensors,
                         const int32_t* verdict_dev, int when, void* stream);

int64_t fst_sumsq_slots(int n_tensors);
int fst_sumsq_multi(const float* const* x_host, const int64_t* numel_host, const int32_t* group_host, int n_tensors,
                    float* slots_dev, int64_t slots_len, const float* limits_dev, float* norms_dev, float* coef_dev, void* stream);
int fst_scale_multi(float* const* x_host, const int64_t* numel_host, const int32_t* group_host, int n_tensors,
                    const float* coef_dev, void* stream);

int fst_ema_multi(float* const* avg_host, const float* const* live_host, const int64_t* numel_host, const int32_t* group_host,
                  int n_tensors, int32_t active_mask, void* state_dev, const int32_t* verdict_dev, void* stream);
int fst_swap_multi(float* const* a_host, float* const* b_host, const int64_t* numel_host, int n_tensors, void* stream);

int fst_accum_multi(float* const* acc_host, float* const* g_host, const int64_t* numel_host, int n_tensors, void* state_dev,
                    int advance, void* stream);

int fst_feed_batch(const void* const* src_host, void* const* dst_host, const int32_t* const* index_host,
                   const int64_t* row_words_host, const int64_t* n_rows_host, const int64_t* batch_host, int n_streams,
                   const void* const* table_host, void* const* scalar_dst_host, int n_scalars, void* state_dev, void* stream);

int fst_eval_fold(const float* logits, int64_t ld, const int64_t* labels, int64_t B, int C, const void* valid_dev, void* state_dev,
                  void* loss_dev, void* confusion_dev, int64_t* pred_out, float* logits_out, int64_t capacity, void* scratch,
                  void* stream);
int fst_eval_finish(const void* state_dev, const void* loss_dev, int64_t expect_rows, void* best_dev, int mode, void* stream);

#ifdef __cplusplus
}
#endif
#endif
```

Baseline: 3635.

## Batch WaveNet res-skip weight-gradient products of several layers into one launch

Adds a multi-layer wgrad kernel that decodes each workgroup into (layer, slice, group) and runs the shared product body with per-layer operand pointers held in the kernel-argument segment. By default only the res_skip kind (excluding the last layer) is grouped this way when layers share shape and d_out. This replaces many small per-layer launches with one larger grid, aiming to cut launch overhead and fill the GPU better. The cost is a larger argument block, one workspace allocation per layer, and a more complex dispatch path.

```diff
diff --git a/feature_level_style_transfer_for_tsc_amd/_lib.py b/feature_level_style_transfer_for_tsc_amd/_lib.py
--- a/feature_level_style_transfer_for_tsc_amd/_lib.py
+++ b/feature_level_style_transfer_for_tsc_amd/_lib.py
@@ -7,7 +7,7 @@
 
 import torch
 
-ABI_VERSION = 26
+ABI_VERSION = 27
 _LIB_NAME = "libfst_hip.so"
 _HERE = os.path.dirname(os.path.abspath(__file__))
 LIB_PATH = os.environ.get("FST_HIP_LIB", os.path.join(_HERE, _LIB_NAME))
@@ -85,6 +85,9 @@
     "fst_wn_wgrad_in_slabs": (c_int, [_P, _P, _P, c_int, c_int64, _P, c_int64, c_int, c_int, c_int, c_int, c_int, c_int, c_int64,
                                       c_void_p]),
     "fst_wn_wgrad_rs_slabs": (c_int, [_P, _P, _P, c_int, _P, c_int64, c_int, c_int, c_int, c_int, c_int64, c_void_p]),
+    "fst_wn_wgrad_in_slabs_many": (c_int, [_P, _P, _P, _I32P, c_int64, _P, _P, _I32P, _I32P, c_int, c_int, c_int, c_int, c_int, c_int64,
+                                           c_void_p]),
+    "fst_wn_wgrad_rs_slabs_many": (c_int, [_P, _P, _P, _I32P, _P, _P, c_int, c_int, c_int, c_int, c_int64, c_void_p]),
     "fst_wn_wgrad_reduce_many": (c_int, [_I32P, _I32P, _I32P, _P, _P, _P, _P, c_int, c_int, c_int, c_int, c_int, c_void_p]),
     "fst_nt_gemm_workspace_floats": (c_int64, [c_int, c_int, c_int]),
     "fst_nt_gemm": (c_int, [_P, _P, _P, _P, c_int64, c_int, c_int, c_int, _P, _P, c_int, c_float, _P, c_void_p]),
diff --git a/feature_level_style_transfer_for_tsc_amd/csrc/wn_wgrad.hip b/feature_level_style_transfer_for_tsc_amd/csrc/wn_wgrad.hip
--- a/feature_level_style_transfer_for_tsc_amd/csrc/wn_wgrad.hip
+++ b/feature_level_style_transfer_for_tsc_amd/csrc/wn_wgrad.hip
@@ -2,6 +2,7 @@
 #include <type_traits>
 
 #include "fst_device.h"
+#include "ww_order.h"
 
 #define WW_TT 32
 #define WW_MROWS 256
@@ -137,14 +138,35 @@
   return v;
 }
 
+struct WwOperands {
+  const float* dy0; const float* dy1;
+  const float* x0; const float* x1; const float* x2; const float* x3;
+  int sh0, sh1, sh2, sh3;
+  int misaligned;
+  float* slab;
+  float* slab_extra;
+};
+__device__ __forceinline__ WwOperands ww_own_operands(const WwParams& p, int set) {
+  return {p.dy[0].ptr[set], p.dy[1].ptr[set], p.x[0].ptr[set], p.x[1].ptr[set], p.x[2].ptr[set], p.x[3].ptr[set],
+          p.x[0].shift, p.x[1].shift, p.x[2].shift, p.x[3].shift, p.misaligned, p.slab, p.slab_extra};
+}
+template <class T>
+__device__ __forceinline__ T ww_pick4(int si, T v0, T v1, T v2, T v3) {
+  T v = v0;
+  if (si == 1) v = v1;
+  if (si == 2) v = v2;
+  if (si == 3) v = v3;
+  return v;
+}
+
 struct WwSrc { const float* p; int bs, t; };
 
 struct WwDyStage {
   WwSrc src[4];
 
-  __device__ __forceinline__ void build(const WwParams& p, int set, int wave_s, int lane) {
-    const float* const d0 = p.dy[0].ptr[set];
-    const float* const d1 = p.dy[1].ptr[set];
+  __device__ __forceinline__ void build(const WwParams& p, const WwOperands& o, int wave_s, int lane) {
+    const float* const d0 = o.dy0;
+    const float* const d1 = o.dy1;
 #pragma unroll
     for (int k = 0; k < 4; ++k) {
       const WwDmaLane m = ww_dma_lane(wave_s + 8 * k, lane);
@@ -170,10 +192,11 @@
   WwSrc src[WW_MAX_NX];
   int my_nx;
 
-  __device__ __forceinline__ void build(const WwParams& p, int set, int g, int wave_s, int lane) {
+  __device__ __forceinline__ void build(const WwParams& p, const WwOperands& o, int g, int wave_s, int lane) {
     const int NXI = p.RX >> 3;
     my_nx = (NXI - wave_s + 7) >> 3;
-    const float* const xp[4] = {p.x[0].ptr[set], p.x[1].ptr[set], p.x[2].ptr[set], p.x[3].ptr[set]};
+    const float* const xp0 = o.x0; const float* const xp1 = o.x1; const float* const xp2 = o.x2; const float* const xp3 = o.x3;
+    const int sh0 = o.sh0, sh1 = o.sh1, sh2 = o.sh2, sh3 = o.sh3;
 #pragma unroll
     for (int k = 0; k < WW_MAX_NX; ++k) {
       src[k].p = nullptr; src[k].bs = 0; src[k].t = 0;
@@ -190,10 +213,10 @@
       }
       if (kk >= 0 && kk < p.K && (kk < p.K_main || rr >= p.xr * (1 + p.mul))) {
         const WwRow row = ww_k_row(p.x, p.n_x, kk);
-        const float* sp = ww_pick(xp, row.si, [](const float* x) { return x; });
+        const float* sp = ww_pick4(row.si, xp0, xp1, xp2, xp3);
         const long long sbs = ww_pick(p.x, row.si, [](const WwSeg& x) { return x.bs; });
         const long long smo = ww_pick(p.x, row.si, [](const WwSeg& x) { return x.mul_off; });
-        const int ssh = ww_pick(p.x, row.si, [](const WwSeg& x) { return x.shift; });
+        const int ssh = ww_pick4(row.si, sh0, sh1, sh2, sh3);
         src[k].p = sp + ((long long)row.c * p.L + ssh + 4 * q) + (partner ? smo : 0);
         src[k].bs = (int)sbs;
         src[k].t = ssh + 4 * q;
@@ -209,10 +232,11 @@
   }
 };
 
-__device__ __forceinline__ int ww_patch_shift(const WwParams& p, int g, int tid) {
-  if (!(p.misaligned && tid < p.xr)) return 0;
+__device__ __forceinline__ int ww_patch_shift(const WwParams& p, const WwOperands& o, int g, int tid) {
+  const int sh0 = o.sh0, sh1 = o.sh1, sh2 = o.sh2, sh3 = o.sh3;
+  if (!(o.misaligned && tid < p.xr)) return 0;
   const int kk = g * p.xr + tid;
-  const int sh = ww_pick(p.x, ww_k_row(p.x, p.n_x, kk).si, [](const WwSeg& x) { return x.shift; });
+  const int sh = ww_pick4(ww_k_row(p.x, p.n_x, kk).si, sh0, sh1, sh2, sh3);
   return (kk < p.K_main && (sh & 3) != 0 && sh > -4 && sh < 4) ? sh : 0;
 }
 
@@ -308,22 +332,22 @@
 }
 
 template <int MT, int KT, bool FULL, bool MUL, int NE>
-__global__ __launch_bounds__(512, 2) void wn_wgrad_kernel(WwParams p) {
+__device__ __forceinline__ void ww_product(const WwParams& p, const WwOperands o, int slice, int g) {
   extern __shared__ __attribute__((aligned(16))) char ww_lds[];
   const int tid = threadIdx.x, lane = tid & 63, half = lane >> 5, l31 = lane & 31;
   const int wave_s = __builtin_amdgcn_readfirstlane(tid >> 6);
   const int wm = wave_s >> 1, wk = wave_s & 1;
-  const int g = blockIdx.y, L = p.L;
-  const int set = blockIdx.x % p.n_sets;
+  const int L = p.L;
+  const int set = slice % p.n_sets;
   const int dslot_bytes = WW_MROWS * 128, xslot_bytes = p.RX * 128;
   char* const xring = ww_lds + WW_ND * dslot_bytes;
   const char* const zero16 = reinterpret_cast<const char*>(ww_zero16);
 
   WwDyStage dys;
-  dys.build(p, set, wave_s, lane);
+  dys.build(p, o, wave_s, lane);
   WwXStage xs;
-  xs.build(p, set, g, wave_s, lane);
-  const int patch_sh = ww_patch_shift(p, g, tid);
+  xs.build(p, o, g, wave_s, lane);
+  const int patch_sh = ww_patch_shift(p, o, g, tid);
   __builtin_amdgcn_s_waitcnt(0x0F70);
 
   auto tile_bt = [&](int tile, int& b, int& t0) {
@@ -347,7 +371,7 @@
   zero_acc(acc);
   float ev[2] = {0.f, 0.f};
 
-  const int wg_in_set = blockIdx.x / p.n_sets, wgs_of_set = (p.ksplit - set + p.n_sets - 1) / p.n_sets;
+  const int wg_in_set = slice / p.n_sets, wgs_of_set = (p.ksplit - set + p.n_sets - 1) / p.n_sets;
   int tile_begin, tile_end;
   ww_tile_range(wg_in_set, wgs_of_set, p.n_tiles, tile_begin, tile_end);
   const int m_blocks = (p.M + 31) >> 5;
@@ -378,7 +402,7 @@
     };
     char* const dsl = ww_lds + dslot * dslot_bytes;
     char* const xsl = xring + xslot * xslot_bytes;
-    if (p.misaligned) {
+    if (o.misaligned) {
       int bq, t0;
       tile_bt(tile_begin + c, bq, t0);
       ww_patch_edges(xsl, tid, patch_sh, t0, L);
@@ -392,7 +416,7 @@
     xslot ^= 1;
   }
 
-  float* const slab = p.slab + (long long)blockIdx.x * WW_MROWS * p.Kcols;
+  float* const slab = o.slab + (long long)slice * WW_MROWS * p.Kcols;
 #pragma unroll
   for (int i = 0; i < MT; ++i) {
     if (i >= m_live) break;
@@ -408,8 +432,49 @@
       float sv = ev[i];
       sv += __shfl_xor(sv, 1, 64);
       sv += __shfl_xor(sv, 2, 64);
-      if ((tid & 3) == 0) p.slab_extra[((long long)blockIdx.x * WW_MROWS + (tid >> 2) + 128 * i) * 2] = sv;
-    }
+      if ((tid & 3) == 0) o.slab_extra[((long long)slice * WW_MROWS + (tid >> 2) + 128 * i) * 2] = sv;
+    }
+  }
+}
+
+template <int MT, int KT, bool FULL, bool MUL, int NE>
+__global__ __launch_bounds__(512, 2) void wn_wgrad_kernel(WwParams p) {
+  ww_product<MT, KT, FULL, MUL, NE>(p, ww_own_operands(p, blockIdx.x % p.n_sets), blockIdx.x, blockIdx.y);
+}
+
+#define WW_MAX_MANY 8
+struct WwLayer {
+  const float* ptr[3][WW_MAX_SETS];
+  float* slab;
+  float* slab_extra;
+  int dil;
+  int misaligned;
+};
+struct WwManyParams {
+  WwParams c;
+  WwLayer layer[WW_MAX_MANY];
+  int n_layers;
+};
+static_assert(sizeof(WwManyParams) <= 4096, "wn_wgrad_many_kernel: the arguments must fit the kernel-argument segment");
+
+template <int MT, int KT, bool FULL, bool MUL, int NE>
+__global__ __launch_bounds__(512, 2) void wn_wgrad_many_kernel(WwManyParams a_by_value) {
+  typedef const __attribute__((address_space(4))) WwManyParams Args;
+  Args& a = *(Args*)__builtin_amdgcn_kernarg_segment_ptr();
+  const WwWork w = ww_many_decode((int)blockIdx.x, a.n_layers, a.c.ksplit, a.c.n_groups);
+  const __attribute__((address_space(4))) WwLayer& lay = a.layer[w.layer];
+  const int set = w.slice % a_by_value.c.n_sets;
+  auto of_set = [set](const float* v0, const float* v1, const float* v2) { return ww_pick4(set, v0, v1, v2, v2); };
+  const float* const o0 = of_set(lay.ptr[0][0], lay.ptr[0][1], lay.ptr[0][2]);
+  const float* const o1 = of_set(lay.ptr[1][0], lay.ptr[1][1], lay.ptr[1][2]);
+  if constexpr (MUL) {
+    const WwOperands o = {o0, a_by_value.c.dy[1].ptr[set], o1, o1, o1, o1, 0, 0, 0, 0, 0, lay.slab, lay.slab_extra};
+    ww_product<MT, KT, FULL, MUL, NE>(a_by_value.c, o, w.slice, w.group);
+  } else {
+    const float* const o2 = of_set(lay.ptr[2][0], lay.ptr[2][1], lay.ptr[2][2]);
+    const int dil = lay.dil;
+    const WwOperands o = {o0, o0, o1, o1, o1, o2, -dil, 0, dil, 0, lay.misaligned, lay.slab, lay.slab_extra};
+    ww_product<MT, KT, FULL, MUL, NE>(a_by_value.c, o, w.slice, w.group);
   }
 }
 
@@ -725,6 +790,106 @@
                                      float* workspace, int64_t workspace_floats, int last, int B, int L, int n, int64_t numel_a,
                                      void* stream) {
   return ww_rs(d_a, d_out, ts, n_sets, nullptr, workspace, workspace_floats, last, B, L, n, numel_a, stream, false);
+}
+
+
+static int ww_many_launch(WwManyParams& mp, int KT, void* stream) {
+  const WwParams& p = mp.c;
+  const size_t lds = (size_t)WW_ND * WW_MROWS * 128 + (size_t)WW_NX * p.RX * 128;
+  FST_REQUIRE(lds <= 160 * 1024 && (p.RX >> 3) <= 8 * WW_MAX_NX, "fst_wn_wgrad_many: %d staged k-rows per stage do not fit (LDS %zu B)", p.RX, lds);
+  const bool full = (p.M + 31) / 32 == 8 && ((p.K_main + 31) / 32) % (2 * KT) == 0;
+  void (*fn)(WwManyParams);
+  if (KT == 3) {
+    if (p.n_extra) fn = full ? wn_wgrad_many_kernel<2, 3, true, false, 1> : wn_wgrad_many_kernel<2, 3, false, false, 1>;
+    else fn = full ? wn_wgrad_many_kernel<2, 3, true, false, 0> : wn_wgrad_many_kernel<2, 3, false, false, 0>;
+  } else {
+    fn = full ? wn_wgrad_many_kernel<2, 2, true, true, 0> : wn_wgrad_many_kernel<2, 2, false, true, 0>;
+  }
+  if (int rc = fst_allow_full_lds((const void*)fn, "fst_wn_wgrad_many")) return rc;
+  int misaligned = 0;
+  for (int j = 0; j < mp.n_layers; ++j) misaligned |= mp.layer[j].misaligned;
+  fst_wn_set_route(FST_WN_ROUTE_WGRAD_MANY, KT, (int)full, p.mul, p.n_extra, p.ksplit, p.n_groups, mp.n_layers, p.n_sets, misaligned, 0, (int)lds);
+  hipLaunchKernelGGL(fn, dim3((unsigned)(mp.n_layers * p.ksplit * p.n_groups)), dim3(512), lds, (hipStream_t)stream, mp);
+  FST_LAUNCH_CHECK();
+  return 0;
+}
+
+static int ww_many_prologue(const char* who, int kind, const float* const* const* const* ops, int n_ops, int n_layers,
+                            const int32_t* n_sets, float* const* workspace, const int64_t* workspace_floats, int B, int L, int n, int h,
+                            WwManyParams& mp, int& KT) {
+  FST_REQUIRE(n_layers >= 1 && n_layers <= WW_MAX_MANY, "%s: %d layers (1..%d)", who, n_layers, WW_MAX_MANY);
+  FST_REQUIRE(n_sets && workspace && workspace_floats, "%s: null table", who);
+  const int ns = n_sets[0];
+  FST_REQUIRE(ns >= 1 && ns <= WW_MAX_SETS, "%s: %d operand sets (1..%d)", who, ns, WW_MAX_SETS);
+  for (int j = 0; j < n_layers; ++j) FST_REQUIRE(n_sets[j] == ns, "%s: layer %d has %d operand sets, layer 0 has %d", who, j, (int)n_sets[j], ns);
+  KT = ww_geometry(kind, B, L, n, h, 0, ns, &mp.c);
+  mp.n_layers = n_layers;
+  for (int j = 0; j < n_layers; ++j) {
+    FST_REQUIRE(workspace[j] && fst_aligned16(workspace[j]), "%s: the workspace of layer %d is null or not 16-byte aligned", who, j);
+    WwParams q = mp.c;
+    char whoj[64];
+    snprintf(whoj, sizeof whoj, "%s: layer %d", who, j);
+    if (int rc = ww_bind_workspace(q, workspace[j], workspace_floats[j], whoj)) return rc;
+    mp.layer[j].slab = q.slab;
+    mp.layer[j].slab_extra = q.slab_extra;
+    for (int k = 0; k < n_ops; ++k) {
+      FST_REQUIRE(ops[k][j], "%s: null operand table of layer %d", who, j);
+      for (int s = 0; s < ns; ++s) {
+        FST_REQUIRE(ops[k][j][s], "%s: null operand in layer %d, set %d", who, j, s);
+        FST_REQUIRE(fst_aligned16(ops[k][j][s]), "%s: operands must be 16-byte aligned", who);
+        mp.layer[j].ptr[k][s] = ops[k][j][s];
+      }
+    }
+  }
+  return 0;
+}
+
+extern "C" int fst_wn_wgrad_in_slabs_many(const float* const* const* dg, const float* const* const* a, const float* const* const* u0,
+                                          const int32_t* n_sets, int64_t u0_bs, float* const* workspace, const int64_t* workspace_floats,
+                                          const int32_t* dil, const int32_t* a_slack, int n_layers, int B, int L, int n, int h,
+                                          int64_t numel_a, void* stream) {
+  fst_wn_clear_route();
+  const char* const who = "fst_wn_wgrad_in_slabs_many";
+  FST_REQUIRE(dg && a && u0 && dil && a_slack, "%s: null table", who);
+  FST_REQUIRE(n_layers >= 1 && n_layers <= WW_MAX_MANY, "%s: %d layers (1..%d)", who, n_layers, WW_MAX_MANY);
+  for (int j = 0; j < n_layers; ++j) {
+    const int served = fst_wn_wgrad_ok(0, B, L, n, h, dil[j]);
+    FST_REQUIRE(served == 1 || (served == 2 && a_slack[j]), "%s: layer %d: unsupported shape B=%d L=%d n=%d h=%d dil=%d (needs L %% 32 == 0, "
+                "n < 128, h <= 32, and dil %% 4 == 0 or — with 16 readable bytes either side of a — dil < 4)", who, j, B, L, n, h, (int)dil[j]);
+  }
+  FST_REQUIRE((long long)B * n * L == (long long)numel_a, "%s: B*n*L does not match the element count %lld of a", who, (long long)numel_a);
+  FST_REQUIRE(B == 1 || u0_bs >= (int64_t)h * L, "%s: u0 batch stride %lld < h*L", who, (long long)u0_bs);
+  FST_REQUIRE(u0_bs % 4 == 0, "%s: operands must be 16-byte aligned", who);
+  WwManyParams mp = {};
+  int KT;
+  const float* const* const* const ops[3] = {dg, a, u0};
+  if (int rc = ww_many_prologue(who, 0, ops, 3, n_layers, n_sets, workspace, workspace_floats, B, L, n, h, mp, KT)) return rc;
+  ww_in_segments(mp.c, n, h, L, dil[0], (long long)u0_bs);
+  for (int j = 0; j < n_layers; ++j) {
+    mp.layer[j].dil = dil[j];
+    mp.layer[j].misaligned = dil[j] % 4 != 0;
+  }
+  return ww_many_launch(mp, KT, stream);
+}
+
+extern "C" int fst_wn_wgrad_rs_slabs_many(const float* const* const* d_a, const float* const* d_out, const float* const* const* ts,
+                                          const int32_t* n_sets, float* const* workspace, const int64_t* workspace_floats, int n_layers,
+                                          int B, int L, int n, int64_t numel_a, void* stream) {
+  fst_wn_clear_route();
+  const char* const who = "fst_wn_wgrad_rs_slabs_many";
+  FST_REQUIRE(d_a && d_out && ts, "%s: null table", who);
+  FST_REQUIRE(fst_wn_wgrad_ok(1, B, L, n, 0, 4), "%s: unsupported shape B=%d L=%d n=%d (needs L %% 32 == 0, n < 128)", who, B, L, n);
+  FST_REQUIRE((long long)B * n * L == (long long)numel_a, "%s: B*n*L does not match the element count %lld", who, (long long)numel_a);
+  WwManyParams mp = {};
+  int KT;
+  const float* const* const* const ops[2] = {d_a, ts};
+  if (int rc = ww_many_prologue(who, 1, ops, 2, n_layers, n_sets, workspace, workspace_floats, B, L, n, 0, mp, KT)) return rc;
+  ww_rs_segments(mp.c, n, L, 0);
+  for (int s = 0; s < mp.c.n_sets; ++s) {
+    FST_REQUIRE(d_out[s] && fst_aligned16(d_out[s]), "%s: d_out of set %d is null or not 16-byte aligned", who, s);
+    mp.c.dy[1].ptr[s] = d_out[s];
+  }
+  return ww_many_launch(mp, KT, stream);
 }
 
 static WwRedEntry ww_red_entry(const WwParams& p) {
diff --git a/feature_level_style_transfer_for_tsc_amd/csrc/ww_order.h b/feature_level_style_transfer_for_tsc_amd/csrc/ww_order.h
--- /dev/null
+++ b/feature_level_style_transfer_for_tsc_amd/csrc/ww_order.h
@@ -0,0 +1,27 @@
+#pragma once
+
+#if defined(__HIPCC__) || defined(__CUDACC__)
+#define WW_ORDER_FN __host__ __device__ inline
+#else
+#define WW_ORDER_FN inline
+#endif
+
+struct WwWork { int layer, slice, group; };
+
+WW_ORDER_FN WwWork ww_many_decode(int id, int n_layers, int ksplit, int n_groups) {
+  const int per = n_layers * n_groups;
+  int slice, inner;
+  if ((ksplit & 7) == 0) {
+    const int x = id & 7, k = id >> 3;
+    slice = (k / per) * 8 + x;
+    inner = k % per;
+  } else {
+    slice = id / per;
+    inner = id % per;
+  }
+  WwWork w;
+  w.layer = (ksplit & 7) == 0 ? inner / n_groups : inner % n_layers;
+  w.group = (ksplit & 7) == 0 ? inner % n_groups : inner / n_layers;
+  w.slice = slice;
+  return w;
+}
diff --git a/feature_level_style_transfer_for_tsc_amd/ops.py b/feature_level_style_transfer_for_tsc_amd/ops.py
--- a/feature_level_style_transfer_for_tsc_amd/ops.py
+++ b/feature_level_style_transfer_for_tsc_amd/ops.py
@@ -68,12 +68,13 @@
 
 WN_ROUTE_WGRAD, WN_ROUTE_TZ, WN_ROUTE_LAYER_FWD, WN_ROUTE_STACK_FWD, WN_ROUTE_LAYER_BWD, WN_ROUTE_LAYER_DGRAD, WN_ROUTE_STACK_BWD = \
     1, 2, 3, 4, 5, 6, 7
-WN_ROUTE_LAYER_INFER, WN_ROUTE_STACK_INFER = 8, 9
+WN_ROUTE_LAYER_INFER, WN_ROUTE_STACK_INFER, WN_ROUTE_WGRAD_MANY = 8, 9, 10
 WN_ROUTE_LEN = 12
 _WN_ROUTE_NAMES = {WN_ROUTE_WGRAD: "wn_wgrad_kernel", WN_ROUTE_TZ: "tz_wgrad_kernel", WN_ROUTE_LAYER_FWD: "wn_layer_fwd_kernel",
                    WN_ROUTE_STACK_FWD: "wn_stack_fwd_kernel", WN_ROUTE_LAYER_BWD: "wn_layer_bwd_kernel",
                    WN_ROUTE_LAYER_DGRAD: "wn_layer_dgrad_kernel", WN_ROUTE_STACK_BWD: "wn_stack_bwd_kernel",
-                   WN_ROUTE_LAYER_INFER: "wn_layer_infer_kernel", WN_ROUTE_STACK_INFER: "wn_stack_infer_kernel"}
+                   WN_ROUTE_LAYER_INFER: "wn_layer_infer_kernel", WN_ROUTE_STACK_INFER: "wn_stack_infer_kernel",
+                   WN_ROUTE_WGRAD_MANY: "wn_wgrad_many_kernel"}
 
 
 def wn_last_route() -> Tuple[int, ...]:
@@ -84,8 +85,8 @@
 
 def wn_route_kernel_name(route: Sequence[int]) -> str:
     fam, tf = route[0], ("false", "true")
-    if fam == WN_ROUTE_WGRAD:
-        return f"wn_wgrad_kernel<2, {route[1]}, {tf[route[2]]}, {tf[route[3]]}, {route[4]}>"
+    if fam in (WN_ROUTE_WGRAD, WN_ROUTE_WGRAD_MANY):
+        return f"{_WN_ROUTE_NAMES[fam]}<2, {route[1]}, {tf[route[2]]}, {tf[route[3]]}, {route[4]}>"
     if fam == WN_ROUTE_TZ:
         return f"tz_wgrad_kernel<{route[1]}, {tf[route[2]]}>"
     if fam == WN_ROUTE_LAYER_FWD:
@@ -918,7 +919,7 @@
         KERNEL_TIMER.end(timer[0], t0, timer[1], timer[2])
 
 
-def wn_wgrad_in(dg, a, u0, dw_in: Tensor, dw_cond: Tensor, n: int, h: int, dil: int, slabs: Optional[list] = None) -> None:
+def _wgrad_in_operands(dg, a, u0, dw_in: Tensor, dw_cond: Tensor, n: int, h: int):
     dgs, as_, u0s = _wgrad_sets("wn_wgrad_in", dg, a, u0)
     B, _, L = dgs[0].shape
     u0_bs, _ = _ncl(u0s[0], "u0")
@@ -933,21 +934,10 @@
     for t, sh in ((dw_in, (2 * n, n, 3)), (dw_cond, (2 * n, h, 1))):
         if tuple(t.shape) != sh or not t.is_contiguous() or t.dtype != torch.float32:
             raise ValueError(f"wn_wgrad_in: gradient target of shape {tuple(t.shape)}, expected contiguous {sh}")
-    ns = len(dgs)
-
-    def launch(lib, ws, ws_n, keep_slabs):
-        sets = (_ptr_sets(dgs), _ptr_sets(as_), _ptr_sets(u0s), ns, u0_bs)
-        shape = (B, L, n, h, dil, int(slack), numel, stream_ptr())
-        if keep_slabs:
-            check(lib.fst_wn_wgrad_in_slabs(*sets, ws, ws_n, *shape), "fst_wn_wgrad_in_slabs")
-        else:
-            check(lib.fst_wn_wgrad_in(*sets, ptr(dw_in), ptr(dw_cond), ws, ws_n, *shape), "fst_wn_wgrad_in")
-
-    _wn_wgrad_launch(0, False, ns, B, L, n, h, dgs[0].device, (dw_in, dw_cond), slabs, launch,
-                     ("wn_wgrad_kernel<2, 3> bf3", 2.0 * ns * B * L * 2 * n * (3 * n + h), 4.0 * ns * B * L * (2 * n + n + h)))
-
-
-def wn_wgrad_rs(d_a, d_out, ts, dw_rs: Tensor, last: bool, n: int, slabs: Optional[list] = None) -> None:
+    return dgs, as_, u0s, B, L, u0_bs, numel, slack
+
+
+def _wgrad_rs_operands(d_a, d_out, ts, dw_rs: Tensor, last: bool, n: int):
     d_as, d_outs, tss = _wgrad_sets("wn_wgrad_rs", [None] * len(_sets(d_out)) if d_a is None else d_a, d_out, ts)
     B, _, L = d_outs[0].shape
     numel = _same_numel(*d_outs, *[t for t in d_as if t is not None])
@@ -957,6 +947,27 @@
             raise ValueError("wn_wgrad_rs: ts must be contiguous [B, 2n, L]; d_a is None exactly on the last layer")
     if tuple(dw_rs.shape) != (M, n, 1) or not dw_rs.is_contiguous() or dw_rs.dtype != torch.float32:
         raise ValueError(f"wn_wgrad_rs: gradient target of shape {tuple(dw_rs.shape)}, expected contiguous {(M, n, 1)}")
+    return d_as, d_outs, tss, B, L, numel, M
+
+
+def wn_wgrad_in(dg, a, u0, dw_in: Tensor, dw_cond: Tensor, n: int, h: int, dil: int, slabs: Optional[list] = None) -> None:
+    dgs, as_, u0s, B, L, u0_bs, numel, slack = _wgrad_in_operands(dg, a, u0, dw_in, dw_cond, n, h)
+    ns = len(dgs)
+
+    def launch(lib, ws, ws_n, keep_slabs):
+        sets = (_ptr_sets(dgs), _ptr_sets(as_), _ptr_sets(u0s), ns, u0_bs)
+        shape = (B, L, n, h, dil, int(slack), numel, stream_ptr())
+        if keep_slabs:
+            check(lib.fst_wn_wgrad_in_slabs(*sets, ws, ws_n, *shape), "fst_wn_wgrad_in_slabs")
+        else:
+            check(lib.fst_wn_wgrad_in(*sets, ptr(dw_in), ptr(dw_cond), ws, ws_n, *shape), "fst_wn_wgrad_in")
+
+    _wn_wgrad_launch(0, False, ns, B, L, n, h, dgs[0].device, (dw_in, dw_cond), slabs, launch,
+                     ("wn_wgrad_kernel<2, 3> bf3", 2.0 * ns * B * L * 2 * n * (3 * n + h), 4.0 * ns * B * L * (2 * n + n + h)))
+
+
+def wn_wgrad_rs(d_a, d_out, ts, dw_rs: Tensor, last: bool, n: int, slabs: Optional[list] = None) -> None:
+    d_as, d_outs, tss, B, L, numel, M = _wgrad_rs_operands(d_a, d_out, ts, dw_rs, last, n)
     ns = len(d_outs)
 
     def launch(lib, ws, ws_n, keep_slabs):
@@ -969,6 +980,54 @@
 
     _wn_wgrad_launch(1, last, ns, B, L, n, 0, d_outs[0].device, (dw_rs, None), slabs, launch,
                      ("wn_wgrad_kernel<2, 2> bf3", 2.0 * ns * B * L * M * n, 4.0 * ns * B * L * (M + 2 * n)))
+
+
+WN_WGRAD_MAX_MANY = 8
+WN_WGRAD_MANY = os.environ.get("FST_WN_WGRAD_MANY", "1") != "0"
+WN_WGRAD_MANY_KINDS = (1,)
+
+
+def _ptr_set_table(layers: Sequence[Sequence[Tensor]]):
+    arrays = [_ptr_sets(ts) for ts in layers]
+    return (ctypes.c_void_p * len(arrays))(*[ctypes.addressof(a) for a in arrays]), arrays
+
+
+def wn_wgrad_slabs_many(kind: int, layers: list, n: int, h: int, slabs: list) -> None:
+    lib = _lib.load()
+    if kind == 0:
+        checked = [_wgrad_in_operands(l[0], l[1], l[2], l[3], l[4], n, h) for l in layers]
+        facts = {(len(c[0]),) + c[3:7] for c in checked}
+    else:
+        checked = [_wgrad_rs_operands(l[0], l[1], l[2], l[3], False, n) for l in layers]
+        facts = {(len(c[0]),) + c[3:6] for c in checked}
+    if not 1 <= len(layers) <= WN_WGRAD_MAX_MANY or len(facts) != 1:
+        raise ValueError(f"wn_wgrad_slabs_many: 1..{WN_WGRAD_MAX_MANY} layers of one shape and one operand-set count")
+    nl, lead = len(layers), layers[0][0 if kind == 0 else 1]
+    ns, (B, _, L), dev = len(lead), lead[0].shape, lead[0].device
+    if kind == 1 and any([t.data_ptr() for t in l[1]] != [t.data_ptr() for t in lead] for l in layers):
+        raise ValueError("wn_wgrad_slabs_many: the res_skip products of one launch share their d_out tensors")
+    ws_n = lib.fst_wn_wgrad_workspace_floats(kind, B, L, n, h, 0)
+    wss = [torch.empty(ws_n, device=dev, dtype=torch.float32) for _ in range(nl)]
+    i32 = lambda vals: (ctypes.c_int32 * nl)(*[int(v) for v in vals])
+    tail = (i32([ns] * nl), _ptr_table(wss), (ctypes.c_int64 * nl)(*[ws_n] * nl))
+    numel = B * n * L
+    t0 = KERNEL_TIMER.begin() if KERNEL_TIMER is not None else None
+    if kind == 0:
+        tabs = [_ptr_set_table([l[j] for l in layers]) for j in range(3)]
+        u0_bs = checked[0][5]
+        check(lib.fst_wn_wgrad_in_slabs_many(tabs[0][0], tabs[1][0], tabs[2][0], tail[0], u0_bs, tail[1], tail[2], i32(l[5] for l in layers),
+                                             i32(c[7] for c in checked), nl, B, L, n, h, numel, stream_ptr()),
+              "fst_wn_wgrad_in_slabs_many")
+        key, flops, nbytes = "wn_wgrad_kernel<2, 3> bf3", 2.0 * ns * B * L * 2 * n * (3 * n + h), 4.0 * ns * B * L * (2 * n + n + h)
+    else:
+        tabs = [_ptr_set_table([l[j] for l in layers]) for j in (0, 2)]
+        check(lib.fst_wn_wgrad_rs_slabs_many(tabs[0][0], _ptr_sets(lead), tabs[1][0], *tail, nl, B, L, n, numel, stream_ptr()),
+              "fst_wn_wgrad_rs_slabs_many")
+        key, flops, nbytes = "wn_wgrad_kernel<2, 2> bf3", 2.0 * ns * B * L * 2 * n * n, 4.0 * ns * B * L * (2 * n + 2 * n)
+    for l, ws in zip(layers, wss):
+        slabs.append((kind, False, ns, ws) + ((l[3], l[4]) if kind == 0 else (l[3], None)))
+    if t0 is not None:
+        KERNEL_TIMER.end(key, t0, nl * flops, nl * nbytes)
 
 
 WN_WGRAD_MAX_REDUCE = 16
@@ -1056,7 +1115,7 @@
         nl, n, h = S.n_layers, S.n, S.h
         dw = S.unflatten(g)
         g_cond_w, g_in_w, g_rs_w = dw[2], dw[6: 6 + nl], dw[6 + 2 * nl: 6 + 3 * nl]
-        slabs, later = {}, []
+        slabs, later, many = {}, [], {}
         for (kind, i), sets in pending.items():
             groups = {}
             for s in sets:
@@ -1069,20 +1128,39 @@
                     chunk = members[c0: c0 + WN_WGRAD_MAX_SETS]
                     cols = [list(col) for col in zip(*chunk)]
                     to = None if c0 else slabs.setdefault(shape[:2], [])
+                    batch = many.setdefault((kind, shape), []) if to is not None and WN_WGRAD_MANY and kind in WN_WGRAD_MANY_KINDS and not (kind == 1 and i == nl - 1) else None
                     if kind == 0:
                         t_in, t_cond = g_in_w[i], g_cond_w[2 * n * i: 2 * n * (i + 1)]
                         if not own:
                             t_in, t_cond = torch.empty_like(t_in), torch.empty_like(t_cond)
                             later += [(g_in_w[i], t_in), (g_cond_w[2 * n * i: 2 * n * (i + 1)], t_cond)]
-                        wn_wgrad_in(cols[0], cols[1], cols[2], t_in, t_cond, n, h, 2 ** i, slabs=to)
+                        if batch is not None:
+                            batch.append((cols[0], cols[1], cols[2], t_in, t_cond, 2 ** i))
+                        else:
+                            wn_wgrad_in(cols[0], cols[1], cols[2], t_in, t_cond, n, h, 2 ** i, slabs=to)
                     else:
                         last = i == nl - 1
                         t_rs = g_rs_w[i]
                         if not own:
                             t_rs = torch.empty_like(t_rs)
                             later.append((g_rs_w[i], t_rs))
-                        wn_wgrad_rs(None if last else cols[0], cols[1], cols[2], t_rs, last, n, slabs=to)
+                        if batch is not None:
+                            batch.append((cols[0], cols[1], cols[2], t_rs))
+                        else:
+                            wn_wgrad_rs(None if last else cols[0], cols[1], cols[2], t_rs, last, n, slabs=to)
                     own = False
+        for (kind, shape), layers in many.items():
+            to = slabs[shape[:2]]
+            same = len({len(l[0]) for l in layers}) == 1 and (kind == 0 or len({tuple(t.data_ptr() for t in l[1]) for l in layers}) == 1)
+            if len(layers) > 1 and same:
+                for c0 in range(0, len(layers), WN_WGRAD_MAX_MANY):
+                    wn_wgrad_slabs_many(kind, layers[c0: c0 + WN_WGRAD_MAX_MANY], n, h, to)
+            else:
+                for l in layers:
+                    if kind == 0:
+                        wn_wgrad_in(l[0], l[1], l[2], l[3], l[4], n, h, l[5], slabs=to)
+                    else:
+                        wn_wgrad_rs(l[0], l[1], l[2], l[3], False, n, slabs=to)
         for (B, L), entries in slabs.items():
             wn_wgrad_reduce_many(entries, B, L, n, h)
         for seg, t in later:
diff --git a/include/fst_hip.h b/include/fst_hip.h
--- a/include/fst_hip.h
+++ b/include/fst_hip.h
@@ -7,7 +7,7 @@
 extern "C" {
 #endif
 
-#define FST_ABI_VERSION 26
+#define FST_ABI_VERSION 27
 
 int fst_version(void);
 const char* fst_last_error(void);
@@ -176,6 +176,13 @@
 int fst_wn_wgrad_reduce_many(const int32_t* kind, const int32_t* last, const int32_t* n_sets, float* const* workspace,
                              const int64_t* workspace_floats, float* const* dw0, float* const* dw1, int n_entries, int B, int L,
                              int n, int h, void* stream);
+int fst_wn_wgrad_in_slabs_many(const float* const* const* dg, const float* const* const* a, const float* const* const* u0,
+                               const int32_t* n_sets, int64_t u0_bs, float* const* workspace, const int64_t* workspace_floats,
+                               const int32_t* dil, const int32_t* a_slack, int n_layers, int B, int L, int n, int h, int64_t numel_a,
+                               void* stream);
+int fst_wn_wgrad_rs_slabs_many(const float* const* const* d_a, const float* const* d_out, const float* const* const* ts,
+                               const int32_t* n_sets, float* const* workspace, const int64_t* workspace_floats, int n_layers, int B,
+                               int L, int n, int64_t numel_a, void* stream);
 
 int64_t fst_nt_gemm_workspace_floats(int M, int N, int K);
 int fst_nt_gemm(const float* A, const float* Bm, float* C, float* workspace, int64_t workspace_floats, int M, int N, int K,
@@ -203,6 +210,7 @@
 #define FST_WN_ROUTE_STACK_BWD   7
 #define FST_WN_ROUTE_LAYER_INFER 8
 #define FST_WN_ROUTE_STACK_INFER 9
+#define FST_WN_ROUTE_WGRAD_MANY  10
 int fst_wn_last_route(int32_t out[FST_WN_ROUTE_LEN]);
 
 int fst_batch_sum(const float* x0, const float* x1, float* part, int B, int64_t N, int S, void* stream);
```

New measurement: 3627 (median of 3 runs). No clear change (-0.2%).
